# hagabbar/GenNet

Measured on AMD Instinct MI355X. Metric: waveforms/sec (CNN+GAN step, 2048-sample BBH), higher is better.
Workload: dtype f32

## Files before the change

gennet_amd/_lib.py:

```python
import ctypes as C
import os

_HERE = os.path.dirname(os.path.abspath(__file__))
LIB_PATH = os.path.join(_HERE, 'lib', 'libgennet_hip.so')

_lib = None

vp, i32, i64, f32, f64, u64, sz = C.c_void_p, C.c_int, C.c_longlong, C.c_float, C.c_double, C.c_uint64, C.c_size_t

_SIGS = {
    'gn_conv1d_fwd': [vp, vp, vp, vp, i32, i32, i32, i32, i32, i32, i32, i32, i32, f32, vp],
    'gn_conv1d_fwd_bf16x3': [vp, vp, vp, vp, vp, sz, i32, i32, i32, i32, i32, i32, i32, i32, i32, f32, i32, vp],
    'gn_conv1d_fwd_wino': [vp, vp, vp, vp, vp, sz, i32, i32, i32, i32, i32, i32, i32, i32, i32, f32, vp],
    'gn_conv1d_fwd_stats': [vp, vp, vp, vp, vp, vp, sz, i32, i32, i32, i32, i32, i32, i32, i32, vp],
    'gn_conv1d_fwd_dropout': [vp, vp, vp, vp, vp, i32, i32, i32, i32, i32, i32, i32, i32, i32, f32, f32, vp],
    'gn_conv1d_fwd_any': [vp, vp, vp, vp, i32, i32, i32, i32, i32, i32, i32, i32, i32, f32, vp],
    'gn_conv1d_dgrad_any': [vp, vp, vp, i32, i32, i32, i32, i32, i32, i32, i32, vp],
    'gn_conv1d_wgrad_any': [vp, vp, vp, vp, vp, sz, i32, i32, i32, i32, i32, i32, i32, i32, vp],
    'gn_conv1d_transpose_w': [vp, vp, i32, i32, i32, vp],
    'gn_conv1d_dgrad': [vp, vp, vp, i32, i32, i32, i32, i32, i32, i32, i32, vp],
    'gn_conv1d_dgrad_fused': [vp, vp, vp, i32, i32, i32, i32, i32, i32, i32, i32, vp, vp, i32, f32, f32, vp],
    'gn_dense_bwd_fused': [vp, vp, vp, vp, vp, vp, i32, i32, i32, vp, i32, f32, f32, vp],
    'gn_conv1d_wgrad': [vp, vp, vp, vp, vp, sz, i32, i32, i32, i32, i32, i32, i32, i32, vp],
    'gn_conv2d_w2_fold': [vp, vp, vp, vp, i32, i32, i32, vp],
    'gn_conv2d_w2_unfold_grad': [vp, vp, vp, vp, i32, i32, i32, vp],
    'gn_conv1d_tapfold_x': [vp, vp, i32, i32, i32, i32, i32, vp],
    'gn_conv1d_tapunfold_dx': [vp, vp, i32, i32, i32, i32, i32, vp],
    'gn_conv1d_tapfold_w': [vp, vp, i32, i32, i32, vp],
    'gn_conv1d_tapunfold_dw': [vp, vp, i32, i32, i32, vp],
    'gn_conv1d_tap_groups': [i32, vp, vp],
    'gn_conv1d_up2_fold': [vp, vp, vp, vp, i32, i32, i32, vp],
    'gn_conv1d_up2_unfold_grad': [vp, vp, vp, vp, i32, i32, i32, vp],
    'gn_dense_fwd': [vp, vp, vp, vp, i32, i32, i32, i32, f32, vp],
    'gn_dense_bwd': [vp, vp, vp, vp, vp, vp, vp, sz, i32, i32, i32, vp],
    'gn_act_fwd': [vp, vp, sz, i32, f32, vp],
    'gn_act_bwd': [vp, vp, vp, sz, i32, f32, vp],
    'gn_act_dropout_bwd': [vp, vp, vp, vp, sz, i32, f32, f32, vp],
    'gn_set_conv_math': [i32, vp, sz],
    'gn_conv_fold_bn': [vp, vp, vp, vp, vp, vp, sz, i32, vp],
    'gn_bn_apply_dropgen': [vp, vp, vp, vp, vp, sz, i32, i32, f32, f32, u64, u64, vp],
    'gn_bias_act_dropout': [vp, vp, vp, sz, i32, i32, f32, f32, i32, u64, u64, vp],
    'gn_bias_grad': [vp, vp, vp, sz, sz, i32, vp],
    'gn_prelu_fwd': [vp, vp, vp, i32, sz, vp],
    'gn_prelu_bwd': [vp, vp, vp, vp, vp, i32, sz, vp],
    'gn_dropout_mask': [vp, sz, f32, u64, u64, vp],
    'gn_dropout_apply': [vp, vp, vp, sz, f32, vp],
    'gn_upsample2_fwd': [vp, vp, i32, i32, i32, vp],
    'gn_upsample2_bwd': [vp, vp, i32, i32, i32, vp],
    'gn_maxpool_h2_fwd': [vp, vp, i32, i32, i32, vp],
    'gn_maxpool_h2_bwd': [vp, vp, vp, i32, i32, i32, vp],
    'gn_subtract_stack_fwd': [vp, vp, vp, i32, i32, vp],
    'gn_subtract_stack_bwd': [vp, vp, i32, i32, vp],
    'gn_affine_stack_fwd': [vp, vp, vp, f32, f32, vp, i32, i32, vp],
    'gn_affine_stack_bwd': [vp, f32, f32, vp, i32, i32, vp],
    'gn_assemble_d_batch': [vp, vp, vp, vp, vp, i32, i32, vp],
    'gn_fill_uniform': [vp, sz, f32, f32, u64, u64, vp],
    'gn_fill_normal': [vp, sz, f32, f32, u64, u64, vp],
    'gn_gather_rows': [vp, vp, vp, i32, i32, vp],
    'gn_axpy': [vp, vp, f32, sz, vp],
    'gn_bn_stats': [vp, sz, i32, vp, vp, sz, vp],
    'gn_bn_finalize': [vp, f64, vp, vp, f32, f32, vp, vp, vp, vp, vp, vp, i32, vp],
    'gn_bn_finalize_zero_debias': [vp, f64, vp, vp, f32, f32, vp, vp, vp, vp, i32, vp, vp, vp, vp, i32, vp],
    'gn_bn_infer_coeffs': [vp, vp, vp, vp, f32, vp, vp, i32, vp],
    'gn_bn_apply': [vp, vp, vp, vp, vp, sz, i32, i32, f32, f32, vp],
    'gn_bn_bwd_stats': [vp, vp, vp, vp, vp, vp, vp, vp, sz, sz, i32, i32, f32, f32, vp, vp, vp],
    'gn_bn_bwd_apply': [vp, vp, vp, vp, vp, vp, vp, vp, f64, vp, vp, vp, vp, sz, i32, i32, f32, f32, vp, vp, vp],
    'gn_bn_bwd_stats_conv1': [vp, vp, i32, i32, i32, i32, vp, vp, vp, vp, vp, vp, sz, sz, i32, i32, f32, f32, vp, vp, vp],
    'gn_bn_bwd_apply_conv1': [vp, vp, i32, i32, i32, i32, vp, vp, vp, vp, vp, vp, f64, vp, vp, vp, vp, sz, i32, i32, f32, f32, vp, vp, vp],
    'gn_bce_loss': [vp, vp, vp, vp, i32, i32, vp],
    'gn_mse_loss': [vp, vp, vp, vp, i32, i32, vp],
    'gn_loss_pass': [i32, vp, vp, vp, vp, i64, i32, f64, vp, sz, vp],
    'gn_weight_count': [vp, i64, vp, vp, sz, vp],
    'gn_loss_pass_weighted': [i32, vp, vp, vp, vp, vp, vp, i64, i32, vp, sz, vp],
    'gn_adam_step': [vp, vp, vp, vp, sz, f32, f32, f32, f32, vp],
    'gn_set_rng_base': [vp],
    'gn_adam_step_dyn': [vp, vp, vp, vp, sz, vp, f32, f32, f32, vp],
    'gn_optim_step': [i32, vp, vp, vp, vp, vp, sz, f32, vp, f32, f32, f32, i32, vp, f32, vp],
    'gn_optim_sumsq': [vp, sz, vp, vp],
    'gn_optim_clip_factor': [vp, sz, f32, vp, vp],
    'gn_fill_normal_dyn': [vp, sz, f32, vp, u64, u64, vp],
    'gn_gaussian_noise_fwd': [vp, vp, sz, f32, u64, u64, vp],
    'gn_gaussian_dropout_apply': [vp, vp, sz, f32, u64, u64, vp],
    'gn_alpha_dropout_fwd': [vp, vp, sz, f32, f32, f32, f32, u64, u64, vp],
    'gn_alpha_dropout_bwd': [vp, vp, sz, f32, f32, u64, u64, vp],
    'gn_bn_finalize_zero_debias_dyn': [vp, f64, vp, vp, f32, f32, vp, vp, vp, vp, vp, vp, vp, vp, vp, i32, vp],
    'gn_prof_enable': [i32],
    'gn_prof_reset': [],
    'gn_prof_collect': [i32, vp],
    'gn_chirp_fd_whitened': [vp, vp, vp, vp, vp, i32, i32, f64, f64, f64, f64, f64, vp],
    'gn_irfft_f64': [vp, vp, vp, i32, i32, vp],
    'gn_rfft_f64': [vp, vp, vp, i32, i32, vp],
    'gn_mul_f64': [vp, vp, sz, sz, i32, vp],
    'gn_align_crop': [vp, vp, vp, vp, vp, i32, i32, i32, i32, i32, i32, f64, f64, f64, vp],
    'gn_noise_fd': [vp, vp, i32, i32, u64, u64, vp],
    'gn_synth_templates': [vp, vp, vp, vp, vp, vp, vp, vp, i32, i32, i32, i32, i32, i32, f64, f64, f64, f64, f64, f64, f64, f64, vp],
    'gn_synth_templates_prior': [vp, vp, vp, vp, vp, vp, vp, vp, i32, i32, i32, i32, i32, i32, f64, f64, f64, f64, f64, f64, f64, f64, u64, u64, i32, i32,
                                 f64, f64, vp],
    'gn_noise_whitened': [vp, vp, vp, vp, vp, vp, vp, vp, vp, i32, i32, i32, i32, f64, u64, u64, vp],
    'gn_synth_templates_noise': [vp, vp, vp, vp, vp, vp, vp, vp, vp, vp, vp, vp, vp, i32, i32, i32, i32, i32, i32, f64, f64, f64, f64, f64, f64, f64, f64,
                                 u64, u64, i32, i32, f64, f64, u64, u64, vp, vp],
    'gn_kde2d_pdf': [vp, i32, vp, i32, f64, f64, f64, f64, vp, vp],
    'gn_scale_f64': [vp, f64, sz, vp],
    'gn_f64_to_f32': [vp, vp, f64, sz, vp],
}
_SIZE_FNS = {
    'gn_conv1d_bf16x3_workspace': [i32, i32, i32, i32, i32],
    'gn_conv1d_wino_workspace': [i32, i32],
    'gn_conv1d_wgrad_workspace': [i32, i32, i32, i32, i32, i32, i32],
    'gn_dense_bwd_workspace': [i32, i32, i32],
    'gn_bn_stats_workspace': [sz, i32],
    'gn_bias_grad_workspace': [sz, i32],
    'gn_conv1d_fwd_stats_workspace': [i32, i32, i32],
    'gn_optim_sumsq_slots': [sz],
    'gn_loss_pass_workspace': [i64, i32],
    'gn_weight_count_workspace': [i64],
    'gn_loss_pass_weighted_workspace': [i64, i32],
}


_PREDICATES = {
    'gn_conv1d_needs_any': [i32, i32],
}


class GennetHipError(RuntimeError):
    pass


def lib():
    global _lib
    if _lib is None:
        if not os.path.exists(LIB_PATH):
            try:
                from . import build as _build
                _build.build(verbose=False)
            except Exception as e:
                raise GennetHipError('%s not found and building it failed (%s): run `python -m gennet_amd.build` '
                                     '(hipcc --offload-arch=gfx950); gennet_amd has no CPU fallback' % (LIB_PATH, e))
        import torch
        L = C.CDLL(LIB_PATH)
        for table, restype in ((_SIGS, i32), (_SIZE_FNS, sz), (_PREDICATES, i32)):
            for name, args in table.items():
                try:
                    fn = getattr(L, name)
                except AttributeError:
                    continue
                fn.argtypes = args
                fn.restype = restype
        L.gn_last_error.restype = C.c_char_p
        L.gn_version.restype = i32
        _lib = L
    return _lib


def exported_symbols():
    return sorted(list(_SIGS) + list(_SIZE_FNS) + list(_PREDICATES) + ['gn_last_error', 'gn_version'])


def call(name, *args):
    L = lib()
    try:
        fn = getattr(L, name)
    except AttributeError:
        raise GennetHipError('%s is not exported by %s (stale build?)' % (name, LIB_PATH))
    rc = fn(*args)
    if rc != 0:
        raise GennetHipError('%s failed (%d): %s' % (name, rc, L.gn_last_error().decode()))


def size(name, *args):
    return int(getattr(lib(), name)(*args))


def predicate(name, *args):
    L = lib()
    try:
        fn = getattr(L, name)
    except AttributeError:
        raise GennetHipError('%s is not exported by %s (stale build?)' % (name, LIB_PATH))
    return bool(fn(*args))
```

gennet_amd/csrc/capi.hip:

```cpp
#include <stdarg.h>
#include <algorithm>
#include <mutex>
#include <vector>
#include <stdlib.h>
#include "common.h"

namespace gn {

static thread_local char g_err[512] = "";

void set_error(const char* fmt, ...) {
  va_list ap;
  va_start(ap, fmt);
  vsnprintf(g_err, sizeof(g_err), fmt, ap);
  va_end(ap);
}

int check_launch(const char* what) {
  hipError_t e = hipGetLastError();
  if (e != hipSuccess) {
    set_error("%s: %s", what, hipGetErrorString(e));
    return GN_ELAUNCH;
  }
  return GN_OK;
}

struct ProfRec {
  hipEvent_t a, b;
  double flop;
  int kind;
  double bytes;
};
static bool g_prof_on = false;
static std::vector<ProfRec> g_prof;
static std::vector<hipEvent_t> g_pool;
static hipEvent_t g_cur;
static std::mutex g_prof_mu;

static hipEvent_t get_event() {
  if (!g_pool.empty()) {
    hipEvent_t e = g_pool.back();
    g_pool.pop_back();
    return e;
  }
  hipEvent_t e;
  (void)hipEventCreate(&e);
  return e;
}

static thread_local const uint64_t* g_rng_base = nullptr;
const uint64_t* rng_base() { return g_rng_base; }

void prof_begin(hipStream_t s) {
  if (!g_prof_on) return;
  g_cur = get_event();
  (void)hipEventRecord(g_cur, s);
}

void prof_end(hipStream_t s, double flop, int kind, double bytes) {
  if (!g_prof_on) return;
  hipEvent_t b = get_event();
  (void)hipEventRecord(b, s);
  std::lock_guard<std::mutex> lk(g_prof_mu);
  g_prof.push_back({g_cur, b, flop, kind, bytes});
}

const Switches& switches() {
  static const Switches sw = [] {
    auto on = [](const char* name) { return getenv(name) != nullptr; };
    const char* gflop = getenv("GN_BF16X3_MIN_GFLOP");
    return Switches{on("GN_CONV_NOPIPE"),  on("GN_CONV_NODMA"),   on("GN_CONV_NOMERGE"),    on("GN_CONV_NONARROW"), on("GN_CONV_NOPATCH"),
                    on("GN_WGRAD_NOPIPE"), on("GN_BF16X3_NO_MERGE"), gflop ? atof(gflop) : 50.0};
  }();
  return sw;
}

static int g_conv_math = 0;
static void* g_conv_ws = nullptr;
static size_t g_conv_ws_bytes = 0;
constexpr size_t kWinoKernelBytes = 64ull << 20;

static bool split_worth_it(int B, int M, int ntaps, int Cin, int Cout) {
  constexpr int min_cin = 256, min_cout = 256;
  return Cin >= min_cin && Cout >= min_cout && 2.0 * B * (double)M * ntaps * Cin * Cout >= switches().bf16x3_min_gflop * 1e9;
}
static bool split_worth_it(const ConvArgs& a, int w_taps) {
  return w_taps > 0 ? split_worth_it(a.B, (a.Ly + 1) / 2, w_taps, a.Cin, a.Cout) : split_worth_it(a.B, a.M, a.t.ntaps, a.Cin, a.Cout);
}

static bool needs_any(int Cin, int Cout) {
  const bool strict = Cin <= 4 ? Cout % 4 == 0 : Cout <= 4 ? Cin % 4 == 0 : (Cin % 4 == 0 && Cout % 4 == 0);
  return !strict;
}

enum ConvFamily { CONV_SMALL, CONV_WINO, CONV_WINO_S2, CONV_BF16X3, CONV_DIRECT, CONV_ANYC };

static ConvFamily select_conv(const ConvArgs& a, int w_taps) {
  if (a.any_channels && needs_any(a.Cin, a.Cout)) return CONV_ANYC;
  if (a.Cin <= 4 || a.Cout <= 4) return CONV_SMALL;
  if (g_conv_math == 2 && a.Cin >= 32 && conv_wino_supported(a) && conv_wino_workspace_bytes(a.Cin, a.Cout) <= kWinoKernelBytes) return CONV_WINO;
  if (g_conv_math == 2 && conv_wino_s2_kind(a) == 1 && conv_wino_s2_workspace_bytes(a.Cin, a.Cout) <= kWinoKernelBytes) return CONV_WINO_S2;
  if (g_conv_math == 1 && split_worth_it(a, w_taps) && conv_bf16x3_supported(a)) return CONV_BF16X3;
  return CONV_DIRECT;
}

enum DgradFamily { DGRAD_WINO_S2, DGRAD_BF16X3_MERGED, DGRAD_MERGED, DGRAD_PHASES };

static DgradFamily select_dgrad(const ConvArgs& a) {
  if (a.any_channels && needs_any(a.Cin, a.Cout)) return DGRAD_PHASES;
  if (a.Ly < 2 || a.Cin <= 4 || a.Cout <= 4) return DGRAD_PHASES;
  if (g_conv_math == 2 && conv_wino_s2_kind(a) == 2 && conv_wino_s2_workspace_bytes(a.Cin, a.Cout) <= kWinoKernelBytes) return DGRAD_WINO_S2;
  const Switches& sw = switches();
  const bool split = g_conv_math == 1 && split_worth_it(a, 5);
  if (split) return !sw.bf16x3_no_merge && conv_bf16x3_merged_kind(a) ? DGRAD_BF16X3_MERGED : DGRAD_PHASES;
  if (!sw.conv_nomerge && !sw.conv_nopipe && !sw.conv_nodma && conv_pipe_merged_supported(a)) return DGRAD_MERGED;
  return DGRAD_PHASES;
}

enum WgradFamily { WGRAD_SMALL, WGRAD_WINO, WGRAD_WINO_S2, WGRAD_BF16X3, WGRAD_DIRECT, WGRAD_ANYC };

static WgradFamily select_wgrad(const WgradArgs& a) {
  if (a.any_channels && needs_any(a.Cin, a.Cout)) return WGRAD_ANYC;
  if (a.Cin <= 4 || a.Cout <= 4) return WGRAD_SMALL;
  if (g_conv_math == 2 && wgrad_wino_supported(a) && conv_wino_workspace_bytes(a.Cin, a.Cout) <= kWinoKernelBytes) return WGRAD_WINO;
  if (g_conv_math == 2 && wgrad_wino_s2_supported(a) && conv_wino_s2_workspace_bytes(a.Cin, a.Cout) <= kWinoKernelBytes) return WGRAD_WINO_S2;
  if (g_conv_math == 1 && split_worth_it(a.B, a.M, a.ntaps, a.Cin, a.Cout) && wgrad_bf16x3_supported(a)) return WGRAD_BF16X3;
  return WGRAD_DIRECT;
}

static size_t wgrad_ws_need(WgradFamily f, const WgradArgs& a) {
  switch (f) {
    case WGRAD_SMALL: return needs_any(a.Cin, a.Cout) ? 0 : wgrad_small_workspace_bytes(a.B, a.M, a.Cin, a.Cout, a.ntaps);
    case WGRAD_WINO: return wgrad_wino_workspace_bytes(a.B, a.M, a.Cin, a.Cout);
    case WGRAD_WINO_S2: return wgrad_wino_s2_workspace_bytes(a.B, a.M, a.Cin, a.Cout);
    case WGRAD_ANYC: return wgrad_anyc_workspace_bytes(a.B, a.M, a.Cin, a.Cout, a.ntaps);
    default: return wgrad_workspace_bytes(a.B, a.M, a.Cin, a.Cout, a.ntaps);
  }
}

static int ws_check(const char* what, size_t need, size_t have) {
  if (need <= have) return GN_OK;
  set_error("%s workspace: the selected kernel needs %zu bytes, the workspace has %zu", what, need, have);
  return GN_EWORKSPACE;
}

struct Phases { int w_taps; bool have_split; };

static int conv_run(const ConvArgs& a, hipStream_t s, Phases* ph = nullptr) {
  const ConvFamily f = select_conv(a, ph ? ph->w_taps : 0);
  int w_taps = ph ? ph->w_taps : 0;
  for (int j = 0; !ph && j < a.t.ntaps; ++j) w_taps = std::max(w_taps, a.t.widx[j] + 1);
  const size_t need = f == CONV_WINO ? conv_wino_workspace_bytes(a.Cin, a.Cout) : f == CONV_WINO_S2 ? conv_wino_s2_workspace_bytes(a.Cin, a.Cout)
                      : f == CONV_BF16X3 ? conv_bf16x3_workspace_bytes(a.B, a.Lin, a.Cin, a.Cout, w_taps) : 0;
  if (int rc = ws_check("conv-math", need, g_conv_ws_bytes)) return rc;
  switch (f) {
    case CONV_SMALL: return a.Cin <= 4 ? conv_smallcin_dispatch(a, s) : conv_smallcout_dispatch(a, s);
    case CONV_WINO: return conv_wino_run(a, g_conv_ws, g_conv_ws_bytes, s);
    case CONV_WINO_S2: return conv_wino_s2_run(a, g_conv_ws, g_conv_ws_bytes, s);
    case CONV_BF16X3:
      if (!(ph && ph->have_split)) {
        int rc = conv_bf16x3_split(a, w_taps, g_conv_ws, g_conv_ws_bytes, true, true, s);
        if (rc) return rc;
        if (ph) ph->have_split = true;
      }
      return conv_bf16x3_run(a, w_taps, g_conv_ws, s);
    case CONV_ANYC: return conv_anyc_dispatch(a, s);
    default: return conv_mfma_dispatch(a, s);
  }
}

static ConvArgs fwd_args(const float* x, const float* w, const float* bias, float* y, int B, int L, int Cin, int Cout, int k, int stride, int pad_left,
                         int Lout, int act, float act_param) {
  ConvArgs a = {};
  a.x = x; a.w = w; a.bias = bias; a.y = y;
  a.B = B; a.Lin = L; a.Cin = Cin; a.Cout = Cout; a.M = Lout; a.Ly = Lout;
  a.t.ntaps = k; a.t.in_stride = stride; a.t.out_stride = 1;
  for (int j = 0; j < k; ++j) { a.t.off[j] = j - pad_left; a.t.widx[j] = j; }
  a.act = act; a.act_param = act_param;
  return a;
}

static int set_conv_math_impl(int mode, void* workspace, size_t workspace_bytes) {
  GN_REQUIRE(mode >= 0 && mode <= 2, "set_conv_math: mode %d (0 = direct fp32, 1 = bf16x3, 2 = transform-domain fp32)", mode);
  GN_REQUIRE(mode == 0 || workspace, "set_conv_math: modes 1 and 2 need a device workspace");
  if (mode == 2 && workspace_bytes < kWinoKernelBytes) {
    set_error("set_conv_math: the transform-domain math needs a workspace of %zu bytes, got %zu", kWinoKernelBytes, workspace_bytes);
    return GN_EWORKSPACE;
  }
  g_conv_math = mode;
  g_conv_ws = mode ? workspace : nullptr;
  g_conv_ws_bytes = mode ? workspace_bytes : 0;
  return GN_OK;
}

__global__ void colsum_anyc_kernel(const float* __restrict__ x, double* __restrict__ acc, size_t n, int C) {
  double s[4] = {0, 0, 0, 0};
  const size_t stride = (size_t)gridDim.x * blockDim.x;
  for (size_t i = (size_t)blockIdx.x * blockDim.x + threadIdx.x; i < n; i += stride) {
    const int c = (int)(i % C);
    const double v = (double)x[i];
    s[0] += c == 0 ? v : 0.0; s[1] += c == 1 ? v : 0.0; s[2] += c == 2 ? v : 0.0; s[3] += c == 3 ? v : 0.0;
  }
  __shared__ double red[4][256];
  for (int c = 0; c < 4; ++c) red[c][threadIdx.x] = s[c];
  __syncthreads();
  for (int sft = 128; sft >= 1; sft >>= 1) {
    if (threadIdx.x < sft)
      for (int c = 0; c < 4; ++c) red[c][threadIdx.x] += red[c][threadIdx.x + sft];
    __syncthreads();
  }
  if (threadIdx.x < C) atomicAdd(&acc[threadIdx.x], red[threadIdx.x][0]);
}
__global__ void f64_to_f32_small_kernel(const double* __restrict__ a, float* __restrict__ o, int n) {
  if ((int)threadIdx.x < n) o[threadIdx.x] = (float)a[threadIdx.x];
}

static int bias_grad(const float* dy, float* db, size_t rows, int C, void* ws, size_t ws_bytes, hipStream_t s) {
  if (C % 4 == 0 || C > 4) {
    ColRedArgs r = {};
    r.a = dy; r.rows = rows; r.C = C;
    return colred_run(0, r, ws, ws_bytes, nullptr, db, s);
  }
  if (ws_bytes < 32) { set_error("bias_grad: workspace too small"); return GN_EWORKSPACE; }
  (void)hipMemsetAsync(ws, 0, 32, s);
  size_t g = (rows * C + 255) / 256;
  if (g > 1024) g = 1024;
  hipLaunchKernelGGL(colsum_anyc_kernel, dim3((unsigned)g), dim3(256), 0, s, dy, (double*)ws, rows * C, C);
  hipLaunchKernelGGL(f64_to_f32_small_kernel, dim3(1), dim3(64), 0, s, (const double*)ws, db, C);
  return check_launch("bias_grad");
}

static size_t bias_grad_ws(size_t rows, int C) { return C % 4 == 0 || C > 4 ? colred_workspace_bytes(rows, C) : 32; }

__global__ __launch_bounds__(256) void dense_any_kernel(const float* __restrict__ A, const float* __restrict__ Bm, const float* __restrict__ bias,
                                                        float* __restrict__ C, int M, int N, int K, size_t sam, size_t sak, size_t sbk, size_t sbn, int act,
                                                        float p) {
  __shared__ float As[16][17], Bs[16][17];
  const int tx = threadIdx.x % 16, ty = threadIdx.x / 16;
  const int m = blockIdx.y * 16 + ty, n = blockIdx.x * 16 + tx;
  float acc = 0.f;
  for (int k0 = 0; k0 < K; k0 += 16) {
    const int ka = k0 + tx, kb = k0 + ty;
    As[ty][tx] = (m < M && ka < K) ? A[(size_t)m * sam + (size_t)ka * sak] : 0.f;
    Bs[ty][tx] = (kb < K && n < N) ? Bm[(size_t)kb * sbk + (size_t)n * sbn] : 0.f;
    __syncthreads();
#pragma unroll
    for (int kk = 0; kk < 16; ++kk) acc = fmaf(As[ty][kk], Bs[kk][tx], acc);
    __syncthreads();
  }
  if (m < M && n < N) C[(size_t)m * N + n] = act_apply(bias ? acc + bias[n] : acc, act, p);
}
static int dense_any_gemm(const float* A, const float* Bm, const float* bias, float* C, int M, int N, int K, size_t sam, size_t sak, size_t sbk, size_t sbn,
                          int act, float p, hipStream_t s) {
  if (M <= 0 || N <= 0) return GN_OK;
  if ((M + 15) / 16 > 65535) { set_error("dense: %d rows exceed the grid", M); return GN_EINVAL; }
  hipLaunchKernelGGL(dense_any_kernel, dim3(cdiv(N, 16), cdiv(M, 16)), dim3(256), 0, s, A, Bm, bias, C, M, N, K, sam, sak, sbk, sbn, act, p);
  return check_launch("dense_any");
}
static bool dense_any_shape(int in, int out) { return (in % 4 || out % 4) && !(out <= 4 && in % 4 == 0); }

}

using namespace gn;

extern "C" {

const char* gn_last_error(void) { return g_err; }
int gn_version(void) { return 100; }

int gn_prof_enable(int on) {
  g_prof_on = on != 0;
  return GN_OK;
}
int gn_prof_reset(void) {
  std::lock_guard<std::mutex> lk(g_prof_mu);
  for (auto& r : g_prof) {
    g_pool.push_back(r.a);
    g_pool.push_back(r.b);
  }
  g_prof.clear();
  return GN_OK;
}
int gn_prof_collect(int kind, double* out) {
  std::lock_guard<std::mutex> lk(g_prof_mu);
  double ms = 0, flop = 0, cnt = 0, bytes = 0;
  for (auto& r : g_prof) {
    if (kind >= 0 && r.kind != kind) continue;
    cnt += 1;
    if (hipEventSynchronize(r.b) != hipSuccess) { set_error("prof: event sync failed"); return GN_ELAUNCH; }
    float t = 0;
    if (hipEventElapsedTime(&t, r.a, r.b) != hipSuccess) { set_error("prof: elapsed failed"); return GN_ELAUNCH; }
    ms += t;
    flop += r.flop;
    bytes += r.bytes;
  }
  out[0] = cnt;
  out[1] = ms;
  out[2] = flop;
  out[3] = bytes;
  return GN_OK;
}

static int fwd_impl(const float* x, const float* w, const float* bias, float* y, int B, int L, int Cin, int Cout, int k, int stride, int pad_left, int Lout,
                    int act, float act_param, bool any_channels, void* stream) {
  GN_REQUIRE(x && w && y, "conv1d_fwd: null pointer");
  GN_REQUIRE(B >= 0 && L > 0 && Cin > 0 && Cout > 0 && k >= 1 && k <= 8 && stride >= 1 && Lout > 0, "conv1d_fwd: bad shape");
  GN_REQUIRE(pad_left >= 0 && stride * (Lout - 1) + k - pad_left <= L + k, "conv1d_fwd: Lout %d inconsistent with L %d k %d stride %d", Lout, L, k, stride);
  if (B == 0) return GN_OK;
  ConvArgs a = fwd_args(x, w, bias, y, B, L, Cin, Cout, k, stride, pad_left, Lout, act, act_param);
  a.any_channels = any_channels;
  return conv_run(a, (hipStream_t)stream);
}

int gn_conv1d_fwd(const float* x, const float* w, const float* bias, float* y, int B, int L, int Cin, int Cout, int k, int stride, int pad_left, int Lout,
                  int act, float act_param, void* stream) {
  return fwd_impl(x, w, bias, y, B, L, Cin, Cout, k, stride, pad_left, Lout, act, act_param, false, stream);
}
int gn_conv1d_fwd_any(const float* x, const float* w, const float* bias, float* y, int B, int L, int Cin, int Cout, int k, int stride, int pad_left, int Lout,
                      int act, float act_param, void* stream) {
  return fwd_impl(x, w, bias, y, B, L, Cin, Cout, k, stride, pad_left, Lout, act, act_param, true, stream);
}
int gn_conv1d_needs_any(int Cin, int Cout) { return needs_any(Cin, Cout) ? 1 : 0; }

int gn_set_conv_math(int mode, void* workspace, size_t workspace_bytes) { return set_conv_math_impl(mode, workspace, workspace_bytes); }

size_t gn_conv1d_bf16x3_workspace(int B, int L, int Cin, int Cout, int k) { return conv_bf16x3_workspace_bytes(B, L, Cin, Cout, k); }

size_t gn_conv1d_fwd_stats_workspace(int B, int Lout, int Cout) {
  const size_t fused = (size_t)B * (size_t)((Lout + 63) / 64) * 2 * (size_t)Cout * sizeof(double);
  const size_t plain = colred_workspace_bytes((size_t)B * Lout, Cout);
  return (fused > plain ? fused : plain) + 256;
}

int gn_conv1d_fwd_stats(const float* x, const float* w, const float* bias, float* y, double* sums, void* ws, size_t ws_bytes, int B, int L, int Cin, int Cout, int k,
                        int stride, int pad_left, int Lout, void* stream) {
  hipStream_t s = (hipStream_t)stream;
  GN_REQUIRE(x && w && y && sums && ws, "conv1d_fwd_stats: null pointer");
  GN_REQUIRE(B > 0 && L > 0 && Cin > 0 && Cout > 0 && Cout % 4 == 0 && k >= 1 && k <= 8 && stride >= 1 && Lout > 0, "conv1d_fwd_stats: bad shape");
  GN_REQUIRE(pad_left >= 0 && stride * (Lout - 1) + k - pad_left <= L + k, "conv1d_fwd_stats: Lout %d inconsistent with L %d k %d stride %d", Lout, L, k, stride);
  GN_REQUIRE(ws_bytes >= gn_conv1d_fwd_stats_workspace(B, Lout, Cout), "conv1d_fwd_stats: workspace too small");
  ConvArgs a = fwd_args(x, w, bias, y, B, L, Cin, Cout, k, stride, pad_left, Lout, GN_ACT_LINEAR, 0.f);
  int done = 0;
  a.stat_part = (double*)ws; a.stat_sums = sums; a.stat_done = &done;
  int rc = conv_run(a, s);
  if (rc || done) return rc;
  ColRedArgs r = {};
  r.a = y; r.rows = (size_t)B * Lout; r.C = Cout;
  return colred_run(1, r, ws, ws_bytes, sums, nullptr, s);
}

int gn_conv1d_fwd_bf16x3(const float* x, const float* w, const float* bias, float* y, void* ws, size_t ws_bytes, int B, int L, int Cin, int Cout, int k, int stride,
                         int pad_left, int Lout, int act, float act_param, int resplit, void* stream) {
  GN_REQUIRE(x && w && y && ws, "conv1d_fwd_bf16x3: null pointer");
  GN_REQUIRE(B >= 0 && L > 0 && Cin > 0 && Cout > 0 && k >= 1 && k <= 5 && stride >= 1 && Lout > 0 && pad_left >= 0, "conv1d_fwd_bf16x3: bad shape");
  if (B == 0) return GN_OK;
  ConvArgs a = fwd_args(x, w, bias, y, B, L, Cin, Cout, k, stride, pad_left, Lout, act, act_param);
  GN_REQUIRE(conv_bf16x3_supported(a), "conv1d_fwd_bf16x3: needs Cin %% 16 == 0, Cout %% 64 == 0, k <= 5, stride 1");
  if (resplit) {
    int rc = conv_bf16x3_split(a, k, ws, ws_bytes, true, true, (hipStream_t)stream);
    if (rc) return rc;
  }
  return conv_bf16x3_run(a, k, ws, (hipStream_t)stream);
}

size_t gn_conv1d_wino_workspace(int Cin, int Cout) { return conv_wino_workspace_bytes(Cin, Cout); }

int gn_conv1d_fwd_wino(const float* x, const float* w, const float* bias, float* y, void* ws, size_t ws_bytes, int B, int L, int Cin, int Cout, int k, int stride,
                       int pad_left, int Lout, int act, float act_param, void* stream) {
  GN_REQUIRE(x && w && y && ws, "conv1d_fwd_wino: null pointer");
  GN_REQUIRE(B >= 0 && L > 0 && Cin > 0 && Cout > 0 && k == 5 && stride == 1 && Lout > 0 && pad_left >= 0, "conv1d_fwd_wino: 5 taps, unit stride");
  if (B == 0) return GN_OK;
  ConvArgs a = fwd_args(x, w, bias, y, B, L, Cin, Cout, k, stride, pad_left, Lout, act, act_param);
  return conv_wino_run(a, ws, ws_bytes, (hipStream_t)stream);
}

int gn_conv1d_fwd_dropout(const float* x, const float* w, const float* bias, const uint8_t* mask, float* y, int B, int L, int Cin, int Cout, int k, int stride,
                          int pad_left, int Lout, int act, float act_param, float rate, void* stream) {
  GN_REQUIRE(x && w && y && mask, "conv1d_fwd_dropout: null pointer");
  GN_REQUIRE(B >= 0 && L > 0 && Cin > 0 && Cout > 4 && Cout % 4 == 0 && k >= 1 && k <= 5 && stride >= 1 && Lout > 0 && pad_left >= 0, "conv1d_fwd_dropout: bad shape");
  GN_REQUIRE(rate >= 0.f && rate < 1.f, "conv1d_fwd_dropout: bad rate %f", rate);
  if (B == 0) return GN_OK;
  ConvArgs a = fwd_args(x, w, bias, y, B, L, Cin, Cout, k, stride, pad_left, Lout, act, act_param);
  a.mask = mask; a.keep_scale = 1.0f / (1.0f - rate);
  return conv_run(a, (hipStream_t)stream);
}

int gn_conv1d_transpose_w(const float* w, float* wt, int k, int Cin, int Cout, void* stream) {
  GN_REQUIRE(w && wt && k >= 1 && Cin > 0 && Cout > 0, "transpose_w: bad arguments");
  return transpose_w(w, wt, k, Cin, Cout, (hipStream_t)stream);
}

static int dgrad_impl(const float* dy, const float* wt, float* dx, int B, int L, int Cin, int Cout, int k, int stride, int pad_left, int Lout, const float* gy,
                      const uint8_t* gmask, int gact, float gparam, float grate, void* stream, bool any_channels = false) {
  GN_REQUIRE(dy && wt && dx, "conv1d_dgrad: null pointer");
  GN_REQUIRE(B >= 0 && L > 0 && Cin > 0 && Cout > 0 && k >= 1 && k <= 8 && stride >= 1 && Lout > 0 && pad_left >= 0, "conv1d_dgrad: bad shape");
  if (B == 0) return GN_OK;
  auto phase_args = [&](int p) {
    ConvArgs a = {};
    a.x = dy; a.w = wt; a.bias = nullptr; a.y = dx;
    a.B = B; a.Lin = Lout; a.Cin = Cout; a.Cout = Cin; a.Ly = L;
    a.t.in_stride = 1; a.t.out_stride = stride;
    a.act = GN_ACT_LINEAR;
    a.any_channels = any_channels;
    a.gy = gy; a.gmask = gmask; a.gact = gact; a.gparam = gparam; a.gscale = 1.0f / (1.0f - grate);
    a.M = (L - std::max(p, 0) + stride - 1) / stride;
    a.t.out_off = p < 0 ? pad_left & 1 : p;
    if (p < 0) a.t.out_off_odd = 1 - (pad_left & 1);
    for (int kk = 0; kk < k; ++kk) {
      const int d = (p < 0 ? (kk + pad_left) & 1 : p) + pad_left - kk;
      if (((d % stride) + stride) % stride) continue;
      a.t.off[a.t.ntaps] = (d >= 0) ? d / stride : -((-d) / stride);
      a.t.widx[a.t.ntaps++] = kk;
    }
    return a;
  };
  hipStream_t s = (hipStream_t)stream;
  if (stride == 2 && k == 5) {
    const ConvArgs a = phase_args(-1);
    const DgradFamily f = select_dgrad(a);
    const size_t need = f == DGRAD_WINO_S2 ? conv_wino_s2_workspace_bytes(a.Cin, a.Cout)
                        : f == DGRAD_BF16X3_MERGED ? conv_bf16x3_workspace_bytes(a.B, a.Lin, a.Cin, a.Cout, 5) : 0;
    if (int rc = ws_check("conv-math", need, g_conv_ws_bytes)) return rc;
    if (f == DGRAD_WINO_S2) return conv_wino_s2_run(a, g_conv_ws, g_conv_ws_bytes, s);
    if (f == DGRAD_MERGED) return conv_pipe_run_merged(a, s);
    if (f == DGRAD_BF16X3_MERGED) {
      int rc = conv_bf16x3_split(a, 5, g_conv_ws, g_conv_ws_bytes, true, true, s);
      return rc ? rc : conv_bf16x3_run_merged(a, g_conv_ws, s);
    }
  }
  Phases ph = {stride > 1 ? k : 0, false};
  for (int p = 0; p < stride && p < L; ++p) {
    const ConvArgs a = phase_args(p);
    GN_REQUIRE(a.t.ntaps > 0, "conv1d_dgrad: phase %d has no taps (k %d < stride %d)", p, k, stride);
    int rc = conv_run(a, s, stride > 1 ? &ph : nullptr);
    if (rc) return rc;
  }
  return GN_OK;
}

int gn_conv1d_dgrad(const float* dy, const float* wt, float* dx, int B, int L, int Cin, int Cout, int k, int stride, int pad_left, int Lout, void* stream) {
  return dgrad_impl(dy, wt, dx, B, L, Cin, Cout, k, stride, pad_left, Lout, nullptr, nullptr, GN_ACT_LINEAR, 0.f, 0.f, stream);
}

int gn_conv1d_dgrad_any(const float* dy, const float* wt, float* dx, int B, int L, int Cin, int Cout, int k, int stride, int pad_left, int Lout, void* stream) {
  return dgrad_impl(dy, wt, dx, B, L, Cin, Cout, k, stride, pad_left, Lout, nullptr, nullptr, GN_ACT_LINEAR, 0.f, 0.f, stream, true);
}

int gn_conv1d_dgrad_fused(const float* dy, const float* wt, float* dx, int B, int L, int Cin, int Cout, int k, int stride, int pad_left, int Lout,
                          const float* y_prev, const uint8_t* mask_prev, int act_prev, float act_param_prev, float rate_prev, void* stream) {
  GN_REQUIRE(y_prev, "conv1d_dgrad_fused: y_prev is NULL");
  GN_REQUIRE(Cin > 4 && Cout > 4, "conv1d_dgrad_fused: only the MFMA path fuses the producer's activation gradient (Cin %d, Cout %d)", Cin, Cout);
  GN_REQUIRE(rate_prev >= 0.f && rate_prev < 1.f, "conv1d_dgrad_fused: bad rate");
  return dgrad_impl(dy, wt, dx, B, L, Cin, Cout, k, stride, pad_left, Lout, y_prev, mask_prev, act_prev, act_param_prev, mask_prev ? rate_prev : 0.f, stream);
}

static WgradArgs wgrad_args(const float* x, const float* dy, void* ws, int B, int L, int Cin, int Cout, int k, int stride, int pad_left, int Lout) {
  WgradArgs a = {};
  a.x = x; a.dy = dy; a.part = (float*)ws;
  a.B = B; a.Lin = L; a.Cin = Cin; a.Cout = Cout; a.M = Lout; a.ntaps = k; a.in_stride = stride;
  for (int j = 0; j < k && j < 8; ++j) a.off[j] = j - pad_left;
  return a;
}

size_t gn_conv1d_wgrad_workspace(int B, int L, int Cin, int Cout, int k, int stride, int Lout) {
  WgradArgs a = wgrad_args(nullptr, nullptr, nullptr, B, L, Cin, Cout, k, stride, 0, Lout);
  a.any_channels = 1;
  return std::max(wgrad_ws_need(select_wgrad(a), a), bias_grad_ws((size_t)B * Lout, Cout)) + 256;
}

static int wgrad_impl(const float* x, const float* dy, float* dw, float* db, void* ws, size_t ws_bytes, int B, int L, int Cin, int Cout, int k, int stride,
                      int pad_left, int Lout, bool any_channels, void* stream) {
  GN_REQUIRE(x && dy && dw && ws, "conv1d_wgrad: null pointer");
  GN_REQUIRE(B > 0 && L > 0 && Cin > 0 && Cout > 0 && k >= 1 && k <= 5 && stride >= 1 && Lout > 0 && pad_left >= 0, "conv1d_wgrad: bad shape");
  hipStream_t s = (hipStream_t)stream;
  WgradArgs a = wgrad_args(x, dy, ws, B, L, Cin, Cout, k, stride, pad_left, Lout);
  a.db = db;
  a.any_channels = any_channels;
  const WgradFamily f = select_wgrad(a);
  int rc = ws_check("conv1d_wgrad", wgrad_ws_need(f, a), ws_bytes);
  if (rc) return rc;
  switch (f) {
    case WGRAD_SMALL: {
      WgradSmallArgs sa = {x, dy, (float*)ws, B, L, Cin, Cout, Lout, k, stride};
      std::copy(a.off, a.off + k, sa.off);
      rc = wgrad_small_dispatch(sa, dw, ws_bytes, s);
      break;
    }
    case WGRAD_WINO: rc = wgrad_wino_run(a, dw, s); break;
    case WGRAD_WINO_S2: rc = wgrad_wino_s2_run(a, dw, s); break;
    case WGRAD_ANYC: rc = wgrad_anyc_dispatch(a, dw, ws_bytes, s); break;
    case WGRAD_BF16X3:
      rc = ws_check("conv-math", wgrad_bf16x3_workspace_bytes(B, Lout, Cin, Cout, stride), g_conv_ws_bytes);
      if (!rc) rc = wgrad_bf16x3_dispatch(a, dw, g_conv_ws, g_conv_ws_bytes, s);
      break;
    default:
      rc = wgrad_mfma_dispatch(a, dw, ws_bytes, s);
      if (!rc && a.db_done) return GN_OK;
  }
  if (rc) return rc;
  return db ? bias_grad(dy, db, (size_t)B * Lout, Cout, ws, ws_bytes, s) : GN_OK;
}

int gn_conv1d_wgrad(const float* x, const float* dy, float* dw, float* db, void* ws, size_t ws_bytes, int B, int L, int Cin, int Cout, int k, int stride,
                    int pad_left, int Lout, void* stream) {
  return wgrad_impl(x, dy, dw, db, ws, ws_bytes, B, L, Cin, Cout, k, stride, pad_left, Lout, false, stream);
}
int gn_conv1d_wgrad_any(const float* x, const float* dy, float* dw, float* db, void* ws, size_t ws_bytes, int B, int L, int Cin, int Cout, int k, int stride,
                        int pad_left, int Lout, void* stream) {
  return wgrad_impl(x, dy, dw, db, ws, ws_bytes, B, L, Cin, Cout, k, stride, pad_left, Lout, true, stream);
}

int gn_conv2d_w2_fold(const float* w, const float* bias, float* wf, float* biasf, int kh, int Cin, int Cout, void* stream) {
  GN_REQUIRE(w && wf && kh >= 1 && Cin > 0 && Cout > 0, "conv2d_w2_fold: bad arguments");
  return conv2d_w2_fold(w, bias, wf, biasf, kh, Cin, Cout, (hipStream_t)stream);
}
int gn_conv2d_w2_unfold_grad(const float* dwf, const float* dbf, float* dw, float* db, int kh, int Cin, int Cout, void* stream) {
  GN_REQUIRE(dwf && dw && kh >= 1 && Cin > 0 && Cout > 0, "conv2d_w2_unfold_grad: bad arguments");
  return conv2d_w2_unfold(dwf, dbf, dw, db, kh, Cin, Cout, (hipStream_t)stream);
}
int gn_conv1d_up2_fold(const float* w, const float* bias, float* wf, float* biasf, int Cin, int Cout, int stride, void* stream) {
  GN_REQUIRE(w && wf && Cin > 0 && Cout > 0 && (stride == 1 || stride == 2), "conv1d_up2_fold: bad arguments (5-tap 'same' conv, stride 1 or 2)");
  return up2_fold(w, bias, wf, biasf, Cin, Cout, stride, (hipStream_t)stream);
}
int gn_conv1d_up2_unfold_grad(const float* dwf, const float* dbf, float* dw, float* db, int Cin, int Cout, int stride, void* stream) {
  GN_REQUIRE(dwf && dw && Cin > 0 && Cout > 0 && (stride == 1 || stride == 2) && (!db || dbf), "conv1d_up2_unfold_grad: bad arguments");
  return up2_unfold(dwf, dbf, dw, db, Cin, Cout, stride, (hipStream_t)stream);
}

size_t gn_bias_grad_workspace(size_t rows, int C) { return bias_grad_ws(rows, C) + 256; }

int gn_bias_grad(const float* dy, float* db, void* ws, size_t ws_bytes, size_t rows, int C, void* stream) {
  GN_REQUIRE(dy && db && ws && rows > 0 && C > 0, "bias_grad: bad arguments");
  return bias_grad(dy, db, rows, C, ws, ws_bytes, (hipStream_t)stream);
}

int gn_dense_fwd(const float* x, const float* w, const float* bias, float* y, int B, int in, int out, int act, float act_param, void* stream) {
  GN_REQUIRE(x && w && y && B >= 0 && in > 0 && out > 0, "dense_fwd: bad arguments");
  if (B == 0) return GN_OK;
  if (dense_any_shape(in, out))
    return dense_any_gemm(x, w, bias, y, B, out, in, (size_t)in, 1, (size_t)out, 1, act, act_param, (hipStream_t)stream);
  if (out <= 4) return dense_small_fwd(x, w, bias, y, B, in, out, act, act_param, (hipStream_t)stream);
  return conv_mfma_dispatch(fwd_args(x, w, bias, y, 1, B, in, out, 1, 1, 0, B, act, act_param), (hipStream_t)stream);
}

size_t gn_dense_bwd_workspace(int B, int in, int out) {
  if (out <= 4) return 256;
  if (dense_any_shape(in, out)) return bias_grad_ws((size_t)B, out) + 256;
  size_t w = wgrad_workspace_bytes(1, B, in, out, 1);
  size_t b = bias_grad_ws((size_t)B, out);
  return (w > b ? w : b) + (size_t)in * out * sizeof(float) + 256;
}

int gn_dense_bwd_fused(const float* x, const float* w, const float* dy, float* dx, float* dw, float* db, int B, int in, int out, const uint8_t* mask_prev,
                       int act_prev, float act_param_prev, float rate_prev, void* stream) {
  GN_REQUIRE(x && w && dy && dx && dw && B > 0 && in > 0 && out >= 1 && out <= 4, "dense_bwd_fused: bad arguments (small-output heads only)");
  GN_REQUIRE(rate_prev >= 0.f && rate_prev < 1.f, "dense_bwd_fused: bad rate");
  return dense_small_bwd(x, w, dy, dx, dw, db, B, in, out, (hipStream_t)stream, act_prev, act_param_prev, mask_prev, 1.0f / (1.0f - (mask_prev ? rate_prev : 0.f)));
}

int gn_dense_bwd(const float* x, const float* w, const float* dy, float* dx, float* dw, float* db, void* ws, size_t ws_bytes, int B, int in, int out, void* stream) {
  GN_REQUIRE(x && w && dy && dw && B > 0 && in > 0 && out > 0, "dense_bwd: bad arguments");
  hipStream_t s = (hipStream_t)stream;
  if (dense_any_shape(in, out)) {
    GN_REQUIRE(ws && ws_bytes >= bias_grad_ws((size_t)B, out), "dense_bwd: workspace too small");
    int rc = dx ? dense_any_gemm(dy, w, nullptr, dx, B, in, out, (size_t)out, 1, 1, (size_t)out, GN_ACT_LINEAR, 0.f, s) : GN_OK;
    if (!rc) rc = dense_any_gemm(x, dy, nullptr, dw, in, out, B, 1, (size_t)in, (size_t)out, 1, GN_ACT_LINEAR, 0.f, s);
    if (!rc && db) rc = bias_grad(dy, db, (size_t)B, out, ws, ws_bytes, s);
    return rc;
  }
  if (out <= 4) return dense_small_bwd(x, w, dy, dx, dw, db, B, in, out, s);
  GN_REQUIRE(ws && ws_bytes >= gn_dense_bwd_workspace(B, in, out), "dense_bwd: workspace too small");
// ... 243 lines not shown
```

gennet_amd/csrc/common.h:

```cpp
#pragma once
#include <hip/hip_runtime.h>
#include <stdint.h>
#include <stdio.h>
#include "../../include/gennet_hip.h"

#define GN_LDS_DMA_CLOBBER() asm volatile("" ::: "v0", "v1", "v2", "v3")
#define gn_buffer_load_lds(...) do { __builtin_amdgcn_raw_ptr_buffer_load_lds(__VA_ARGS__); GN_LDS_DMA_CLOBBER(); } while (0)
#define gn_global_load_lds(...) do { __builtin_amdgcn_global_load_lds(__VA_ARGS__); GN_LDS_DMA_CLOBBER(); } while (0)

namespace gn {

void set_error(const char* fmt, ...);
int check_launch(const char* what);

struct Switches {
  bool conv_nopipe, conv_nodma, conv_nomerge, conv_nonarrow, conv_nopatch;
  bool wgrad_nopipe, bf16x3_no_merge;
  double bf16x3_min_gflop;
};
const Switches& switches();

const uint64_t* rng_base();
void prof_begin(hipStream_t s);
void prof_end(hipStream_t s, double flop, int kind, double bytes = 0.0);


struct ConvTaps {
  int ntaps;
  int in_stride;
  int off[8];
  int widx[8];
  int out_stride, out_off;
  int out_off_odd;
};

struct ConvArgs {
  const float* x;
  const float* w;
  const float* bias;
  float* y;
  int B, Lin, Cin, Cout;
  int M;
  int Ly;
  ConvTaps t;
  int act;
  float act_param;
  int any_channels;
  const uint8_t* mask;
  float keep_scale;
  const float* gy;
  const uint8_t* gmask;
  int gact;
  float gparam, gscale;
  double* stat_part;
  double* stat_sums;
  int* stat_done;
};

struct WgradArgs {
  const float* x;
  const float* dy;
  float* part;
  int B, Lin, Cin, Cout, M;
  int ntaps, in_stride;
  int off[8];
  int chunks_per_split;
  double* db_part;
  float* db;
  int db_done;
  int any_channels;
};

struct WgradSmallArgs {
  const float* x;
  const float* dy;
  float* part;
  int B, Lin, Cin, Cout, M;
  int ntaps, in_stride;
  int off[8];
  int rows_per_chunk;
};

struct LazyDy {
  const float* g;
  const float* w;
  int L, Lout, k, pad_left;
};

struct ColRedArgs {
  const float* a;
  const float* y;
  const float* xpre;
  const uint8_t* mask;
  const float* mean;
  const float* invstd;
  const float* scale;
  const float* shift;
  double* part;
  size_t rows;
  int C;
  int rows_per_chunk;
  int act;
  float act_param;
  float keep_scale;
  LazyDy lz;
};

int conv_mfma_dispatch(const ConvArgs& a, hipStream_t s);
size_t wgrad_workspace_bytes(int B, int M, int Cin, int Cout, int ntaps);
int wgrad_mfma_dispatch(WgradArgs& a, float* dw, size_t ws_bytes, hipStream_t s);
int wgrad_bf16x3_dispatch(WgradArgs& a, float* dw, void* split_ws, size_t split_ws_bytes, hipStream_t s);
int conv_pipe_try(const ConvArgs& a, bool tall, hipStream_t s, bool* launched);
bool conv_pipe_merged_supported(const ConvArgs& a);
int conv_pipe_run_merged(const ConvArgs& a, hipStream_t s);
void wgrad_pipe_launch(const WgradArgs& a, dim3 grid, bool narrow, hipStream_t s);
size_t conv_bf16x3_workspace_bytes(int B, int Lin, int Cin, int Cout, int w_taps);
bool conv_bf16x3_supported(const ConvArgs& a);
int conv_bf16x3_split(const ConvArgs& a, int w_taps, void* ws, size_t ws_bytes, bool split_x, bool split_w, hipStream_t s);
int conv_bf16x3_run(const ConvArgs& a, int w_taps, void* ws, hipStream_t s);
int conv_bf16x3_merged_kind(const ConvArgs& a);
int conv_bf16x3_run_merged(const ConvArgs& a, void* ws, hipStream_t s);
size_t conv_wino_workspace_bytes(int Cin, int Cout);
bool conv_wino_supported(const ConvArgs& a);
int conv_wino_run(const ConvArgs& a, void* ws, size_t ws_bytes, hipStream_t s);
size_t conv_wino_s2_workspace_bytes(int Cin, int Cout);
int conv_wino_s2_kind(const ConvArgs& a);
int conv_wino_s2_run(const ConvArgs& a, void* ws, size_t ws_bytes, hipStream_t s);
void wgrad_split_plan(int B, int M, int Cin, int Cout, int TC, int TN, int* splits, int* chunks_per_split);
bool wgrad_wino_supported(const WgradArgs& a);
size_t wgrad_wino_workspace_bytes(int B, int M, int Cin, int Cout);
int wgrad_wino_run(WgradArgs& a, float* dw, hipStream_t s);
bool wgrad_wino_s2_supported(const WgradArgs& a);
size_t wgrad_wino_s2_workspace_bytes(int B, int M, int Cin, int Cout);
int wgrad_wino_s2_run(WgradArgs& a, float* dw, hipStream_t s);
size_t wgrad_bf16x3_workspace_bytes(int B, int M, int Cin, int Cout, int in_stride);
bool wgrad_bf16x3_supported(const WgradArgs& a);
int wgrad_bf16x3_run(const WgradArgs& a, int splits, void* ws, size_t ws_bytes, hipStream_t s);
int conv_anyc_dispatch(const ConvArgs& a, hipStream_t s);
size_t wgrad_anyc_workspace_bytes(int B, int M, int Cin, int Cout, int ntaps);
int wgrad_anyc_dispatch(WgradArgs& a, float* dw, size_t ws_bytes, hipStream_t s);
int conv_smallcin_dispatch(const ConvArgs& a, hipStream_t s);
int conv_smallcout_dispatch(const ConvArgs& a, hipStream_t s);
size_t wgrad_small_workspace_bytes(int B, int M, int Cin, int Cout, int ntaps);
int wgrad_small_dispatch(WgradSmallArgs a, float* dw, size_t ws_bytes, hipStream_t s);
int dense_small_fwd(const float* x, const float* w, const float* bias, float* y, int B, int in, int out, int act, float p, hipStream_t s);
int dense_small_bwd(const float* x, const float* w, const float* dy, float* dx, float* dw, float* db, int B, int in, int out, hipStream_t s,
                    int gact = 0, float gparam = 0.f, const uint8_t* gmask = nullptr, float gscale = 1.f);
int act_fwd(const float* x, float* y, size_t n, int act, float p, hipStream_t s);
int act_bwd(const float* dy, const float* y, float* dx, size_t n, int act, float p, hipStream_t s);
int act_dropout_bwd(const float* dy, const float* y, const uint8_t* mask, float* dx, size_t n, int act, float p, float rate, hipStream_t s);
int dropout_mask(uint8_t* mask, size_t n, float rate, uint64_t seed, uint64_t offset, hipStream_t s);
int dropout_apply(const float* x, const uint8_t* mask, float* y, size_t n, float rate, hipStream_t s);
int upsample2_fwd(const float* x, float* y, int B, int L, int C, hipStream_t s);
int upsample2_bwd(const float* dy, float* dx, int B, int L, int C, hipStream_t s);
int subtract_stack_fwd(const float* x, const float* ev, float* img, int B, int n, hipStream_t s);
int subtract_stack_bwd(const float* dimg, float* dx, int B, int n, hipStream_t s);
int affine_stack_fwd(const float* x, const float* b0, const float* b1, float a0, float a1, float* img, int B, int n, hipStream_t s);
int affine_stack_bwd(const float* dimg, float a0, float a1, float* dx, int B, int n, hipStream_t s);
int assemble_d_batch(const float* real, const float* noise, const float* fake, const float* ev, float* sX, int B, int n, hipStream_t s);
int gather_rows(const float* src, const int64_t* idx, float* out, int rows, int width, hipStream_t s);
int axpy(float* y, const float* x, float a, size_t n, hipStream_t s);
int fill_uniform(float* out, size_t n, float lo, float hi, uint64_t seed, uint64_t offset, hipStream_t s);
int fill_normal(float* out, size_t n, float mean, float sd, uint64_t seed, uint64_t offset, hipStream_t s, const float* sd_dev = nullptr);
int gaussian_noise_fwd(const float* x, float* y, size_t n, float stddev, uint64_t seed, uint64_t offset, hipStream_t s);
int gaussian_dropout_apply(const float* x, float* y, size_t n, float sd, uint64_t seed, uint64_t offset, hipStream_t s);
int alpha_dropout_fwd(const float* x, float* y, size_t n, float rate, float a, float b, float alpha_p, uint64_t seed, uint64_t offset, hipStream_t s);
int alpha_dropout_bwd(const float* dy, float* dx, size_t n, float rate, float a, uint64_t seed, uint64_t offset, hipStream_t s);
size_t colred_workspace_bytes(size_t rows, int C);
int colred_run(int mode, ColRedArgs a, void* ws, size_t ws_bytes, double* out_f64, float* out_f32, hipStream_t s);
int colred_finalize(const double* part, double* out_f64, size_t n, int chunks, hipStream_t s);
int colred_finalize_f32(const double* part, float* out_f32, size_t n, int chunks, hipStream_t s);
int bn_finalize(const double* sums, double count, const float* gamma, const float* beta, float eps, float momentum, float* mm, float* mv,
                float* bm, float* bv, float zd_step, float* scale, float* shift, float* smean, float* sinv, int C, hipStream_t s,
                const int32_t* zd_step_dev = nullptr);
int bn_infer_coeffs(const float* gamma, const float* beta, const float* mm, const float* mv, float eps, float* scale, float* shift, int C, hipStream_t s);
int bn_apply(const float* x, const float* scale, const float* shift, const uint8_t* mask, float* y, size_t rows, int C, int act, float p, float rate, hipStream_t s);
int bn_bwd_apply(const float* dy, const float* y, const float* x, const uint8_t* mask, const float* gamma, const float* mean, const float* invstd,
                 const double* dsums_global, double count, const double* dsums_local, float* dx, float* dgamma, float* dbeta, size_t rows, int C,
                 int act, float p, float rate, const float* scale, const float* shift, hipStream_t s, const LazyDy* lz = nullptr);
int loss_run(int kind, const float* p, const float* y, float* dp, float* out, int B, int Bglobal, hipStream_t s);
int adam_step(float* p, const float* g, float* m, float* v, size_t n, float lr_t, float b1, float b2, float eps, hipStream_t s, const float* lr_t_dev = nullptr);
struct OptArgs {
  float *p, *s0, *s1, *s2;
  const float* g;
  size_t n;
  float lr;
  const float* lr_dev;
  float h0, h1, eps;
  int nesterov;
  const float* clip_scale;
  float clipvalue;
};
int optim_step(int rule, const OptArgs& a, hipStream_t s);
size_t optim_sumsq_slots(size_t n);
int optim_sumsq(const float* g, size_t n, double* partials, hipStream_t s);
int optim_clip_factor(const double* partials, size_t count, float clipnorm, float* factor, hipStream_t s);
int transpose_w(const float* w, float* wt, int k, int Cin, int Cout, hipStream_t s);
int conv2d_w2_fold(const float* w, const float* bias, float* wf, float* bf, int kh, int Cin, int Cout, hipStream_t s);
int conv2d_w2_unfold(const float* dwf, const float* dbf, float* dw, float* db, int kh, int Cin, int Cout, hipStream_t s);
int up2_fold(const float* w, const float* bias, float* wf, float* bf, int Cin, int Cout, int stride, hipStream_t s);
int up2_unfold(const float* dwf, const float* dbf, float* dw, float* db, int Cin, int Cout, int stride, hipStream_t s);

static inline unsigned cdiv(size_t a, size_t b) { return (unsigned)((a + b - 1) / b); }
static inline unsigned stream_grid(size_t n_items, int block = 256) {
  size_t g = (n_items + block - 1) / block;
  if (g > 256 * 8) g = 256 * 8;
  if (g < 1) g = 1;
  return (unsigned)g;
}

static inline void allow_big_lds(const void* kernel, unsigned long long* done) {
  int dev = 0;
  (void)hipGetDevice(&dev);
  const unsigned long long bit = 1ull << (dev & 63);
  if (!(*done & bit)) {
    (void)hipFuncSetAttribute(kernel, hipFuncAttributeMaxDynamicSharedMemorySize, 160 * 1024);
    *done |= bit;
  }
}

#define GN_REQUIRE(cond, ...)            \
  do {                                   \
    if (!(cond)) {                       \
      gn::set_error(__VA_ARGS__);        \
      return GN_EINVAL;                  \
    }                                    \
  } while (0)

__device__ __forceinline__ float gn_tanhf(float x) {
  const float ax = fabsf(x);
  const float e = __builtin_amdgcn_exp2f(ax * 2.8853900817779268f);
  const float big = 1.f - 2.f * __builtin_amdgcn_rcpf(e + 1.f);
  const float x2 = ax * ax;
  float q = fmaf(x2, -1382.f / 155925.f, 62.f / 2835.f);
  q = fmaf(x2, q, -17.f / 315.f);
  q = fmaf(x2, q, 2.f / 15.f);
  q = fmaf(x2, q, -1.f / 3.f);
  const float small = fmaf(ax * x2, q, ax);
  return copysignf(ax < 0.35f ? small : big, x);
}

__device__ __forceinline__ float act_apply(float x, int act, float p) {
  switch (act) {
    case GN_ACT_RELU: return fmaxf(x, 0.f);
    case GN_ACT_RELU_MAX: return fminf(fmaxf(x, 0.f), p);
    case GN_ACT_LEAKY: return x > 0.f ? x : p * x;
    case GN_ACT_TANH: return gn_tanhf(x);
    case GN_ACT_SIGMOID: return 1.f / (1.f + expf(-x));
    default: return x;
  }
}

__device__ __forceinline__ float act_grad_from_y(float y, int act, float p) {
  switch (act) {
    case GN_ACT_RELU: return y > 0.f ? 1.f : 0.f;
    case GN_ACT_RELU_MAX: return (y > 0.f && y < p) ? 1.f : 0.f;
    case GN_ACT_LEAKY: return y > 0.f ? 1.f : p;
    case GN_ACT_TANH: return 1.f - y * y;
    case GN_ACT_SIGMOID: return y * (1.f - y);
    default: return 1.f;
  }
}

struct Philox4 {
  uint32_t v[4];
};

__host__ __device__ __forceinline__ uint32_t mulhi32(uint32_t a, uint32_t b) { return (uint32_t)(((uint64_t)a * b) >> 32); }

__host__ __device__ __forceinline__ Philox4 philox4x32_10(uint64_t counter, uint64_t seed) {
  uint32_t c0 = (uint32_t)counter, c1 = (uint32_t)(counter >> 32), c2 = 0, c3 = 0;
  uint32_t k0 = (uint32_t)seed, k1 = (uint32_t)(seed >> 32);
#pragma unroll
  for (int r = 0; r < 10; ++r) {
    const uint32_t M0 = 0xD2511F53u, M1 = 0xCD9E8D57u;
    uint32_t h0 = mulhi32(M0, c0), l0 = M0 * c0;
    uint32_t h1 = mulhi32(M1, c2), l1 = M1 * c2;
    uint32_t n0 = h1 ^ c1 ^ k0, n1 = l1, n2 = h0 ^ c3 ^ k1, n3 = l0;
    c0 = n0; c1 = n1; c2 = n2; c3 = n3;
    k0 += 0x9E3779B9u; k1 += 0xBB67AE85u;
  }
  Philox4 o;
  o.v[0] = c0; o.v[1] = c1; o.v[2] = c2; o.v[3] = c3;
  return o;
}

__host__ __device__ __forceinline__ float u01_24(uint32_t x) { return (float)(x >> 8) * (1.0f / 16777216.0f); }
__host__ __device__ __forceinline__ double u01_53(uint32_t hi, uint32_t lo) {
  uint64_t x = (((uint64_t)hi << 32) | lo) >> 11;
  return ((double)x + 0.5) * (1.0 / 9007199254740992.0);
}

}
```

gennet_amd/csrc/conv_wino.hip:

```cpp
#include <stdlib.h>
#include <algorithm>
#include <type_traits>
#include "common.h"
#include "conv_epilogue.h"
#include "wino_common.h"

namespace gn {

struct WinoTaps {
  int wq[5];
};

__global__ void wino_u_kernel(const float* __restrict__ w, float* __restrict__ U, int Cin, int Cout, WinoTaps t) {
  const size_t i = (size_t)blockIdx.x * blockDim.x + threadIdx.x;
  const size_t cc = (size_t)Cin * Cout;
  if (i >= cc) return;
  const int ci = (int)(i / Cout), co = (int)(i % Cout);
  double g[5];
#pragma unroll
  for (int q = 0; q < 5; ++q) g[q] = (double)w[(size_t)t.wq[q] * cc + i];
  float u[6];
  u[0] = (float)g[0];
  u[1] = (float)((g[0] + g[1] + g[2] + g[3] + g[4]) * (1.0 / 3.0));
  u[2] = (float)((g[0] - g[1] + g[2] - g[3] + g[4]) * (1.0 / 3.0));
  u[3] = (float)((16.0 * g[0] + 8.0 * g[1] + 4.0 * g[2] + 2.0 * g[3] + g[4]) * (1.0 / 15.0));
  u[4] = (float)((g[0] - 2.0 * g[1] + 4.0 * g[2] - 8.0 * g[3] + 16.0 * g[4]) * (1.0 / 30.0));
  u[5] = (float)g[4];
  const int chunk = ci >> 3, c = ci & 7, kq = c >> 1, s = c & 1;
  const int tile = co >> 6, nn = co & 63, ct = nn >> 4, n16 = nn & 15, cth = ct >> 1, ctl = ct & 1;
  const size_t base = ((size_t)chunk * (Cout >> 6) + tile) * 3072 + ((cth * 4 + kq) * 16 + n16) * 4 + ctl * 2 + s;
#pragma unroll
  for (int p = 0; p < 6; ++p) U[base + p * 512] = u[p];
}

template <int O, int OP1>
__device__ __forceinline__ void wino_slot_rba(f32x4& c, float a, float b, f32x4& nb0, f32x4& nb1, unsigned addr_b, f32x2 (&d)[6], unsigned addr_a) {
  asm volatile(
      "ds_read_b128 %1, %11 offset:%13\n\t"
      "ds_read_b128 %2, %11 offset:%14\n\t"
      "ds_read_b64 %3, %12\n\t"
      "ds_read_b64 %4, %12 offset:%15\n\t"
      "ds_read_b64 %5, %12 offset:32\n\t"
      "ds_read_b64 %6, %12 offset:%16\n\t"
      "ds_read_b64 %7, %12 offset:64\n\t"
      "ds_read_b64 %8, %12 offset:%17\n\t"
      "s_waitcnt lgkmcnt(8)\n\t"
      "v_mfma_f32_16x16x4_f32 %0, %9, %10, %0"
      : "+v"(c), "=&v"(nb0), "=&v"(nb1), "=&v"(d[0]), "=&v"(d[1]), "=&v"(d[2]), "=&v"(d[3]), "=&v"(d[4]), "=&v"(d[5])
      : "v"(a), "v"(b), "v"(addr_b), "v"(addr_a), "i"(O), "i"(O + 1024), "i"(OP1), "i"(OP1 + 32), "i"(OP1 + 64)
      : "memory");
}
template <int O>
__device__ __forceinline__ void wino_slot_rbw(f32x4& c, float a, float b, f32x4& nb0, f32x4& nb1, unsigned addr_b, f32x2 (&d)[6]) {
  asm volatile(
      "ds_read_b128 %1, %11 offset:%12\n\t"
      "ds_read_b128 %2, %11 offset:%13\n\t"
      "s_waitcnt lgkmcnt(2)\n\t"
      "v_mfma_f32_16x16x4_f32 %0, %9, %10, %0"
      : "+v"(c), "=&v"(nb0), "=&v"(nb1), "+v"(d[0]), "+v"(d[1]), "+v"(d[2]), "+v"(d[3]), "+v"(d[4]), "+v"(d[5])
      : "v"(a), "v"(b), "v"(addr_b), "i"(O), "i"(O + 1024)
      : "memory");
}

template <int RPER, int ABL = 0>
struct WinoChunk {
  template <int NPIECES, int I = 0, class D>
  static __device__ __forceinline__ void run(f32x4 (&acc)[6][4], const f32x2 (&v)[6], f32x2 (&vn)[6], f32x2 (&d)[6], WinoT& t, f32x4 (&B)[2][2], unsigned addr_b,
                                             unsigned addr_b_next, unsigned addr_a, unsigned long long k15, unsigned long long km15, D& dma) {
    if constexpr (I < 48) {
      constexpr int P = I / 8, S = (I / 4) % 2, CT = I % 4;
      f32x4(&bc)[2] = B[P & 1];
      f32x4(&bn)[2] = B[(P + 1) & 1];
      const float bv = bc[CT >> 1][2 * (CT & 1) + S];
      const float av = v[P][S];
      if constexpr ((ABL & 8) != 0) wino_slot(acc[P][CT], av, bv);
      else if constexpr (I == 0) wino_slot_rba<2048, RPER * 32>(acc[0][0], av, bv, bn[0], bn[1], addr_b, d, addr_a);
      else if constexpr (I == 8) wino_slot_rbw<2 * 2048>(acc[1][0], av, bv, bn[0], bn[1], addr_b, d);
      else if constexpr (I == 40) wino_slot_rb<0, 2>(acc[5][0], av, bv, bn[0], bn[1], addr_b_next);
      else if constexpr (I % 8 == 0) wino_slot_rb<(P + 1) * 2048, 2>(acc[P][0], av, bv, bn[0], bn[1], addr_b);
      else wino_slot(acc[P][CT], av, bv);
      if constexpr ((I & 1) && (I >> 1) < NPIECES) dma(std::integral_constant<int, (I >> 1)>{});
      if constexpr (!(ABL & 2)) {
        if constexpr (I == 12) wino_run<0, 5>(d, vn, t, k15, km15);
        if constexpr (I == 24) wino_run<5, 10>(d, vn, t, k15, km15);
        if constexpr (I == 36) wino_run<10, kWinoPieces>(d, vn, t, k15, km15);
      }
      run<NPIECES, I + 1>(acc, v, vn, d, t, B, addr_b, addr_b_next, addr_a, k15, km15, dma);
    }
  }
};

template <int WAVES_M, int ABL = 0>
__global__ __launch_bounds__(64 * WAVES_M, (WAVES_M > 4 ? 1 : 2)) void conv_wino_kernel(ConvArgs a, const float* __restrict__ U, int off0, int m_tiles, int n_tiles,
                                                                                        int patch) {
#if defined(__HIP_DEVICE_COMPILE__)
  constexpr int KC = 8, NP = 6;
  constexpr int TT = WAVES_M * 16;
  constexpr int TN = 64;
  constexpr int NT = 64 * WAVES_M;
  constexpr int RPER = TT + 2;
  constexpr int SLAB = 2 * RPER * KC;
  constexpr int UT = NP * KC * TN;
  constexpr int BUF = SLAB + UT;
  constexpr int STAGE_BYTES = BUF * 4;
  extern __shared__ __attribute__((aligned(16))) float smem[];
  typedef __attribute__((address_space(3))) void* lptr_t;

  const int tid = threadIdx.x, lane = tid & 63, wave = tid >> 6;
  const int n16 = lane & 15, kq = lane >> 4;
  const BlockTile bt = xcd_block_tile(patch, m_tiles, n_tiles);
  const int n_tile = bt.n_tile, m_tile = bt.m_tile, b = bt.b;
  const int t0 = m_tile * TT, n0 = n_tile * TN;

  f32x4 acc[NP][4];
#pragma unroll
  for (int p = 0; p < NP; ++p)
#pragma unroll
    for (int ct = 0; ct < 4; ++ct)
#pragma unroll
      for (int r = 0; r < 4; ++r) acc[p][ct][r] = 0.f;

  const int t_base = 2 * t0 + off0;
  const uintptr_t xbp = (uintptr_t)(a.x + (size_t)b * a.Lin * a.Cin);
  const unsigned xb_lo = __builtin_amdgcn_readfirstlane((unsigned)xbp), xb_hi = __builtin_amdgcn_readfirstlane((unsigned)(xbp >> 32));
  const int xbytes = __builtin_amdgcn_readfirstlane(a.Lin * a.Cin * 4);
  const __amdgpu_buffer_rsrc_t xsrd = __builtin_amdgcn_make_buffer_rsrc((void*)(((uintptr_t)xb_hi << 32) | xb_lo), 0, xbytes, 0x00020000);

  constexpr int S_COUNT = SLAB / 4;
  constexpr int S_ITEMS = (S_COUNT + NT - 1) / NT;
  constexpr int W_TOTAL = UT / 4;
  constexpr int W_ITEMS = (W_TOTAL + NT - 1) / NT;
  int soff[S_ITEMS];
#pragma unroll
  for (int it = 0; it < S_ITEMS; ++it) {
    const int id = tid + it * NT;
    const int lr = id >> 1, c4 = id & 1;
    const int r = lr < RPER ? 2 * lr : 2 * (lr - RPER) + 1;
    soff[it] = (id < S_COUNT) ? ((t_base + r) * a.Cin + 4 * c4) * 4 : 0x40000000;
  }
  const uintptr_t wbp = (uintptr_t)U;
  const unsigned wb_lo = __builtin_amdgcn_readfirstlane((unsigned)wbp), wb_hi = __builtin_amdgcn_readfirstlane((unsigned)(wbp >> 32));
  const int wbytes = __builtin_amdgcn_readfirstlane(NP * a.Cin * a.Cout * 4);
  const __amdgpu_buffer_rsrc_t wsrd = __builtin_amdgcn_make_buffer_rsrc((void*)(((uintptr_t)wb_hi << 32) | wb_lo), 0, wbytes, 0x00020000);
  const int w_chunk_bytes = n_tiles * UT * 4;
  int c_next = 0, st_next = 0;
  bool in_loop = false;
  const int wv64 = __builtin_amdgcn_readfirstlane(tid & ~63);
  auto dma_piece = [&](auto kc) {
    constexpr int k = decltype(kc)::value;
    if ((ABL & 1) && in_loop) return;
    float* stg = smem + st_next * BUF;
    if constexpr (k < S_ITEMS) {
      if ((k + 1) * NT <= S_COUNT || tid + k * NT < S_COUNT)
        gn_buffer_load_lds(xsrd, (lptr_t)(stg + (k * NT + wv64) * 4), 16, soff[k], c_next * KC * 4, 0, 0);
    } else {
      constexpr int it = k - S_ITEMS;
      if ((it + 1) * NT <= W_TOTAL || wv64 + it * NT < W_TOTAL)
        gn_buffer_load_lds(wsrd, (lptr_t)(stg + SLAB + (it * NT + wv64) * 4), 16, (n_tile * UT + (tid + it * NT) * 4) * 4,
                                                 c_next * w_chunk_bytes, 0, 0);
    }
  };
  constexpr int NPIECES = S_ITEMS + W_ITEMS;
  static_assert(NPIECES <= 6, "staging pieces");
  auto dma_all = [&]() {
    dma_piece(std::integral_constant<int, 0>{});
    if constexpr (NPIECES > 1) dma_piece(std::integral_constant<int, 1>{});
    if constexpr (NPIECES > 2) dma_piece(std::integral_constant<int, 2>{});
    if constexpr (NPIECES > 3) dma_piece(std::integral_constant<int, 3>{});
    if constexpr (NPIECES > 4) dma_piece(std::integral_constant<int, 4>{});
    if constexpr (NPIECES > 5) dma_piece(std::integral_constant<int, 5>{});
  };

  const unsigned lds0 = (unsigned)(uintptr_t)smem;
  const unsigned base_a = lds0 + (wave * 16 + n16) * 32 + kq * 8;
  const unsigned base_b = lds0 + SLAB * 4 + (kq * 16 + n16) * 16;
  const unsigned long long k15 = 0x3fc000003fc00000ull, km15 = 0xbfc00000bfc00000ull;

  const int n_chunks = a.Cin / KC;
  c_next = 0; st_next = 0; dma_all();
  c_next = min(1, n_chunks - 1); st_next = 1; dma_all();
  __syncthreads();

  f32x2 V0[6], V1[6], d[6];
  f32x4 Bq[2][2];
  WinoT tt;
  {
    const char* sb = reinterpret_cast<const char*>(smem);
#pragma unroll
    for (int j = 0; j < 6; ++j) d[j] = *reinterpret_cast<const f32x2*>(sb + (base_a - lds0) + (j & 1) * RPER * 32 + (j >> 1) * 32);
    wino_run<0, kWinoPieces>(d, V0, tt, k15, km15);
    Bq[0][0] = *reinterpret_cast<const f32x4*>(sb + (base_b - lds0));
    Bq[0][1] = *reinterpret_cast<const f32x4*>(sb + (base_b - lds0) + 1024);
  }
  int st = 0;
  in_loop = true;
  for (int ch = 0; ch < n_chunks; ch += 2) {
#pragma unroll
    for (int half = 0; half < 2; ++half) {
      if (half == 1 && ch + 1 >= n_chunks) break;
      const int st1 = st == 2 ? 0 : st + 1, st2 = st1 == 2 ? 0 : st1 + 1;
      c_next = min(ch + half + 2, n_chunks - 1);
      st_next = st2;
      const unsigned addr_a = base_a + st1 * STAGE_BYTES;
      const unsigned addr_b = base_b + st * STAGE_BYTES, addr_b_next = base_b + st1 * STAGE_BYTES;
      if (half == 0) WinoChunk<RPER, ABL>::template run<NPIECES>(acc, V0, V1, d, tt, Bq, addr_b, addr_b_next, addr_a, k15, km15, dma_piece);
      else WinoChunk<RPER, ABL>::template run<NPIECES>(acc, V1, V0, d, tt, Bq, addr_b, addr_b_next, addr_a, k15, km15, dma_piece);
      if constexpr (!(ABL & 4)) __syncthreads();
      st = st1;
    }
  }
  asm volatile("s_nop 15\n\ts_nop 7" : "+v"(acc[5][0]), "+v"(acc[5][1]), "+v"(acc[5][2]), "+v"(acc[5][3]));

  f32x4 out[2][4];
#pragma unroll
  for (int ct = 0; ct < 4; ++ct)
#pragma unroll
    for (int r = 0; r < 4; ++r) {
      out[0][ct][r] = (((acc[0][ct][r] + acc[1][ct][r]) + acc[2][ct][r]) + acc[3][ct][r]) + acc[4][ct][r];
      out[1][ct][r] = __builtin_fmaf(-2.f, acc[4][ct][r], __builtin_fmaf(0.5f, acc[3][ct][r], acc[1][ct][r] - acc[2][ct][r])) + acc[5][ct][r];
    }
  const int m_base = t0 + __builtin_amdgcn_readfirstlane(wave) * 16;
  const int mode = a.gy ? (a.gmask ? 3 : 2) : (a.mask ? 1 : 0);
  ConvArgs a2 = a;
  a2.t.out_stride = 2;
  tile16_epilogue_dispatch<4>(a2, out[0], b, m_base, n0, n16, kq, a.t.out_off, mode);
  tile16_epilogue_dispatch<4>(a2, out[1], b, m_base, n0, n16, kq, a.t.out_off + 1, mode);

  if (a.stat_part) {
    double* red = reinterpret_cast<double*>(smem);
#pragma unroll
    for (int ct = 0; ct < 4; ++ct) {
      const float bias = a.bias ? a.bias[n0 + ct * 16 + n16] : 0.f;
      double s1 = 0.0, s2 = 0.0;
#pragma unroll
      for (int ph = 0; ph < 2; ++ph)
#pragma unroll
        for (int r = 0; r < 4; ++r) {
          const int row = 2 * (m_base + 4 * kq + r) + ph;
          if (row < a.M) {
            const double v = (double)(out[ph][ct][r] + bias);
            s1 += v; s2 += v * v;
          }
        }
      s1 += __shfl_xor(s1, 16, 64); s2 += __shfl_xor(s2, 16, 64);
      s1 += __shfl_xor(s1, 32, 64); s2 += __shfl_xor(s2, 32, 64);
      if (kq == 0) {
        const int slot = (wave * TN + ct * 16 + n16) * 2;
        red[slot] = s1; red[slot + 1] = s2;
      }
    }
    __syncthreads();
    if (tid < TN) {
      double t1 = 0.0, t2 = 0.0;
#pragma unroll
      for (int w = 0; w < WAVES_M; ++w) { t1 += red[(w * TN + tid) * 2]; t2 += red[(w * TN + tid) * 2 + 1]; }
      double* dst = a.stat_part + (size_t)(b * m_tiles + m_tile) * 2 * a.Cout;
      dst[n0 + tid] = t1;
      dst[a.Cout + n0 + tid] = t2;
    }
  }
#endif
}

template <int WAVES_M, int ABL = 0>
static int launch_conv_wino(const ConvArgs& a, const float* U, int off0, hipStream_t s) {
  constexpr int TT = WAVES_M * 16, TN = 64;
  constexpr size_t lds = 3 * sizeof(float) * ((size_t)2 * (TT + 2) * 8 + (size_t)6 * 8 * TN);
  static_assert(lds <= 160 * 1024, "stages too large");
  if (lds > 64 * 1024) {
    static unsigned long long lds_done = 0;
    allow_big_lds((const void*)conv_wino_kernel<WAVES_M, ABL>, &lds_done);
  }
  const int tiles = (a.M + 1) / 2;
  const int m_tiles = (tiles + TT - 1) / TT, n_tiles = a.Cout / TN;
  const size_t blocks = (size_t)m_tiles * n_tiles * a.B;
  if (blocks == 0 || blocks > 0x7fffffffull) {
    set_error("conv_wino: bad grid %zu", blocks);
    return GN_EINVAL;
  }
  const int patch = xcd_patch(n_tiles);
  prof_begin(s);
  hipLaunchKernelGGL((conv_wino_kernel<WAVES_M, ABL>), dim3((unsigned)blocks), dim3(64 * WAVES_M), lds, s, a, U, off0, m_tiles, n_tiles, patch);
  prof_end(s, 0.6 * 2.0 * a.B * (double)a.M * 5 * a.Cin * a.Cout, 5, 4.0 * ((double)a.B * a.Lin * a.Cin + 5.0 * a.Cin * a.Cout + (double)a.B * a.M * a.Cout));
  int rc = check_launch("conv_wino");
  if (rc || !a.stat_part) return rc;
  *a.stat_done = 1;
  return colred_finalize(a.stat_part, a.stat_sums, (size_t)2 * a.Cout, a.B * m_tiles, s);
}

size_t conv_wino_workspace_bytes(int Cin, int Cout) { return (size_t)6 * Cin * Cout * sizeof(float); }

bool conv_wino_supported(const ConvArgs& a) {
  if (a.t.ntaps != 5 || a.t.in_stride != 1 || a.t.out_stride != 1 || a.t.out_off != 0) return false;
  if (a.Cin % 8 || a.Cout % 64 || a.Cin < 8) return false;
  if ((size_t)a.Ly * a.Cout * 4 >= 0x40000000ull || (size_t)a.Lin * a.Cin * 4 >= 0x40000000ull || (size_t)6 * a.Cin * a.Cout * 4 >= 0x40000000ull) return false;
  bool seen[5] = {false, false, false, false, false};
  int minoff = a.t.off[0];
  for (int j = 1; j < 5; ++j) minoff = std::min(minoff, a.t.off[j]);
  for (int j = 0; j < 5; ++j) {
    const int q = a.t.off[j] - minoff;
    if (q < 0 || q > 4 || seen[q]) return false;
    seen[q] = true;
  }
  if (a.stat_part && (a.act != GN_ACT_LINEAR || a.mask || a.gy)) return false;
  return true;
}

int conv_wino_run(const ConvArgs& a, void* ws, size_t ws_bytes, hipStream_t s) {
  if (!conv_wino_supported(a)) {
    set_error("conv_wino: unsupported shape (5 consecutive taps, unit strides, Cin %% 8 == 0, Cout %% 64 == 0)");
    return GN_EINVAL;
  }
  if (!ws || ws_bytes < conv_wino_workspace_bytes(a.Cin, a.Cout)) {
    set_error("conv_wino: workspace too small (%zu < %zu)", ws_bytes, conv_wino_workspace_bytes(a.Cin, a.Cout));
    return GN_EWORKSPACE;
  }
  int minoff = a.t.off[0];
  for (int j = 1; j < 5; ++j) minoff = std::min(minoff, a.t.off[j]);
  WinoTaps t;
  for (int j = 0; j < 5; ++j) t.wq[a.t.off[j] - minoff] = a.t.widx[j];
  const size_t cc = (size_t)a.Cin * a.Cout;
  hipLaunchKernelGGL(wino_u_kernel, dim3(cdiv(cc, 256)), dim3(256), 0, s, a.w, (float*)ws, a.Cin, a.Cout, t);
  int rc = check_launch("wino_u");
  if (rc) return rc;
  const float* Up = (const float*)ws;
#ifdef GN_ABLATION
  {
    static const int abl = getenv("GN_WINO_ABL") ? atoi(getenv("GN_WINO_ABL")) : 0;
    switch (abl) {
      case 1: return launch_conv_wino<4, 1>(a, Up, minoff, s);
      case 2: return launch_conv_wino<4, 2>(a, Up, minoff, s);
      case 3: return launch_conv_wino<4, 3>(a, Up, minoff, s);
      case 4: return launch_conv_wino<4, 4>(a, Up, minoff, s);
      case 8: return launch_conv_wino<4, 8>(a, Up, minoff, s);
      case 15: return launch_conv_wino<4, 15>(a, Up, minoff, s);
      default: break;
    }
  }
#endif
  return launch_conv_wino<4>(a, Up, minoff, s);
}

}
```

gennet_amd/csrc/conv_wino_s2.hip:

```cpp
#include <stdlib.h>
#include <algorithm>
#include <type_traits>
#include "common.h"
#include "conv_epilogue.h"
#include "wino_common.h"

namespace gn {

struct WinoS2Taps {
  int wq[5];
};

__global__ void wino_s2_u_kernel(const float* __restrict__ w, float* __restrict__ U, int Cin, int Cout, WinoS2Taps t) {
  const size_t i = (size_t)blockIdx.x * blockDim.x + threadIdx.x;
  const size_t cc = (size_t)Cin * Cout;
  if (i >= cc) return;
  const int ci = (int)(i / Cout), co = (int)(i % Cout);
  double g[5];
#pragma unroll
  for (int q = 0; q < 5; ++q) g[q] = (double)w[(size_t)t.wq[q] * cc + i];
  float u[7];
  u[0] = (float)g[0];
  u[1] = (float)(0.5 * (g[0] + g[2] + g[4]));
  u[2] = (float)(0.5 * (g[0] - g[2] + g[4]));
  u[3] = (float)g[4];
  u[4] = (float)g[1];
  u[5] = (float)(g[1] + g[3]);
  u[6] = (float)g[3];
  const int chunk = ci >> 3, c = ci & 7, kq = c >> 1, s = c & 1;
  const int tile = co >> 6, nn = co & 63, ct = nn >> 4, n16 = nn & 15, cth = ct >> 1, ctl = ct & 1;
  const size_t base = ((size_t)chunk * (Cout >> 6) + tile) * 3584 + ((cth * 4 + kq) * 16 + n16) * 4 + ctl * 2 + s;
#pragma unroll
  for (int p = 0; p < 7; ++p) U[base + p * 512] = u[p];
}

template <int O, int PB>
__device__ __forceinline__ void s2_slot_rba7(f32x4& c, float a, float b, f32x4& nb0, f32x4& nb1, unsigned addr_b, f32x2 (&d)[7], unsigned addr_a) {
  asm volatile(
      "ds_read_b128 %1, %12 offset:%14\n\t"
      "ds_read_b128 %2, %12 offset:%15\n\t"
      "ds_read_b64 %3, %13\n\t"
      "ds_read_b64 %4, %13 offset:%16\n\t"
      "ds_read_b64 %5, %13 offset:%17\n\t"
      "ds_read_b64 %6, %13 offset:%18\n\t"
      "ds_read_b64 %7, %13 offset:32\n\t"
      "ds_read_b64 %8, %13 offset:%19\n\t"
      "ds_read_b64 %9, %13 offset:%20\n\t"
      "s_waitcnt lgkmcnt(9)\n\t"
      "v_mfma_f32_16x16x4_f32 %0, %10, %11, %0"
      : "+v"(c), "=&v"(nb0), "=&v"(nb1), "=&v"(d[0]), "=&v"(d[1]), "=&v"(d[2]), "=&v"(d[3]), "=&v"(d[4]), "=&v"(d[5]), "=&v"(d[6])
      : "v"(a), "v"(b), "v"(addr_b), "v"(addr_a), "i"(O), "i"(O + 1024), "i"(PB), "i"(2 * PB), "i"(3 * PB), "i"(PB + 32), "i"(2 * PB + 32)
      : "memory");
}
template <int O, int PB>
__device__ __forceinline__ void s2_slot_rba4(f32x4& c, float a, float b, f32x4& nb0, f32x4& nb1, unsigned addr_b, f32x2 (&d)[4], unsigned addr_a) {
  asm volatile(
      "ds_read_b128 %1, %9 offset:%11\n\t"
      "ds_read_b128 %2, %9 offset:%12\n\t"
      "ds_read_b64 %3, %10\n\t"
      "ds_read_b64 %4, %10 offset:%13\n\t"
      "ds_read_b64 %5, %10 offset:32\n\t"
      "ds_read_b64 %6, %10 offset:%14\n\t"
      "s_waitcnt lgkmcnt(6)\n\t"
      "v_mfma_f32_16x16x4_f32 %0, %7, %8, %0"
      : "+v"(c), "=&v"(nb0), "=&v"(nb1), "=&v"(d[0]), "=&v"(d[1]), "=&v"(d[2]), "=&v"(d[3])
      : "v"(a), "v"(b), "v"(addr_b), "v"(addr_a), "i"(O), "i"(O + 1024), "i"(PB), "i"(PB + 32)
      : "memory");
}
template <int O>
__device__ __forceinline__ void s2_slot_rbw7(f32x4& c, float a, float b, f32x4& nb0, f32x4& nb1, unsigned addr_b, f32x2 (&d)[7]) {
  asm volatile(
      "ds_read_b128 %1, %12 offset:%13\n\t"
      "ds_read_b128 %2, %12 offset:%14\n\t"
      "s_waitcnt lgkmcnt(2)\n\t"
      "v_mfma_f32_16x16x4_f32 %0, %10, %11, %0"
      : "+v"(c), "=&v"(nb0), "=&v"(nb1), "+v"(d[0]), "+v"(d[1]), "+v"(d[2]), "+v"(d[3]), "+v"(d[4]), "+v"(d[5]), "+v"(d[6])
      : "v"(a), "v"(b), "v"(addr_b), "i"(O), "i"(O + 1024)
      : "memory");
}
template <int O>
__device__ __forceinline__ void s2_slot_rbw4(f32x4& c, float a, float b, f32x4& nb0, f32x4& nb1, unsigned addr_b, f32x2 (&d)[4]) {
  asm volatile(
      "ds_read_b128 %1, %9 offset:%10\n\t"
      "ds_read_b128 %2, %9 offset:%11\n\t"
      "s_waitcnt lgkmcnt(2)\n\t"
      "v_mfma_f32_16x16x4_f32 %0, %7, %8, %0"
      : "+v"(c), "=&v"(nb0), "=&v"(nb1), "+v"(d[0]), "+v"(d[1]), "+v"(d[2]), "+v"(d[3])
      : "v"(a), "v"(b), "v"(addr_b), "i"(O), "i"(O + 1024)
      : "memory");
}

template <int KIND, int SB, int RPER, int NR, int PAR>
struct S2Chunk {
  template <int NPIECES, int I = 0, class D>
  static __device__ __forceinline__ void run(f32x4 (&acc)[7][4], const f32x2 (&v)[7], f32x2 (&vn)[7], f32x2 (&d)[NR], f32x4 (&B)[2][2], unsigned addr_b,
                                             unsigned addr_b_next, unsigned addr_a, D& dma) {
    if constexpr (I < 56) {
      constexpr int P = I / 8, S = (I / 4) % 2, CT = I % 4;
      f32x4(&bc)[2] = B[(P + PAR) & 1];
      f32x4(&bn)[2] = B[(P + PAR + 1) & 1];
      const float bv = bc[CT >> 1][2 * (CT & 1) + S];
      const float av = v[P][S];
      if constexpr (I == 0) {
        if constexpr (NR == 7) s2_slot_rba7<2048, RPER * 32>(acc[0][0], av, bv, bn[0], bn[1], addr_b, d, addr_a);
        else s2_slot_rba4<2048, RPER * 32>(acc[0][0], av, bv, bn[0], bn[1], addr_b, d, addr_a);
      } else if constexpr (I == 8) {
        if constexpr (NR == 7) s2_slot_rbw7<2 * 2048>(acc[1][0], av, bv, bn[0], bn[1], addr_b, d);
        else s2_slot_rbw4<2 * 2048>(acc[1][0], av, bv, bn[0], bn[1], addr_b, d);
      } else if constexpr (I == 48) wino_slot_rb<0, 2>(acc[6][0], av, bv, bn[0], bn[1], addr_b_next);
      else if constexpr (I % 8 == 0) wino_slot_rb<(P + 1) * 2048, 2>(acc[P][0], av, bv, bn[0], bn[1], addr_b);
      else wino_slot(acc[P][CT], av, bv);
      if constexpr ((I & 1) && (I >> 1) < NPIECES) dma(std::integral_constant<int, (I >> 1)>{});
      if constexpr (I == 20) s2_run<KIND, SB, NR, 0, 4>(d, vn);
      if constexpr (I == 36) s2_run<KIND, SB, NR, 4, 7>(d, vn);
      run<NPIECES, I + 1>(acc, v, vn, d, B, addr_b, addr_b_next, addr_a, dma);
    }
  }
};

template <int KIND, int SB>
__global__ __launch_bounds__(256, 2) void conv_wino_s2_kernel(ConvArgs a, const float* __restrict__ U, int off0, int m_tiles, int n_tiles, int patch, int offA,
                                                              int offB) {
#if defined(__HIP_DEVICE_COMPILE__)
  constexpr int KC = 8, NP = 7, WAVES_M = 4;
  constexpr int TT = WAVES_M * 16, TN = 64, NT = 64 * WAVES_M;
  constexpr int NR = KIND == 1 ? 7 : 4;
  constexpr int TS = KIND == 1 ? 4 : 2;
  constexpr int RPER = TT + 1;
  constexpr int SLAB = TS * RPER * KC;
  constexpr int UT = NP * KC * TN;
  constexpr int BUF = SLAB + UT;
  constexpr int STAGE_BYTES = BUF * 4;
  extern __shared__ __attribute__((aligned(16))) float smem[];
  typedef __attribute__((address_space(3))) void* lptr_t;

  const int tid = threadIdx.x, lane = tid & 63, wave = tid >> 6;
  const int n16 = lane & 15, kq = lane >> 4;
  const BlockTile bt = xcd_block_tile(patch, m_tiles, n_tiles);
  const int n_tile = bt.n_tile, m_tile = bt.m_tile, b = bt.b;
  const int t0 = m_tile * TT, n0 = n_tile * TN;

  f32x4 acc[NP][4];
#pragma unroll
  for (int p = 0; p < NP; ++p)
#pragma unroll
    for (int ct = 0; ct < 4; ++ct)
#pragma unroll
      for (int r = 0; r < 4; ++r) acc[p][ct][r] = 0.f;

  const int t_base = TS * t0 + off0;
  const uintptr_t xbp = (uintptr_t)(a.x + (size_t)b * a.Lin * a.Cin);
  const unsigned xb_lo = __builtin_amdgcn_readfirstlane((unsigned)xbp), xb_hi = __builtin_amdgcn_readfirstlane((unsigned)(xbp >> 32));
  const int xbytes = __builtin_amdgcn_readfirstlane(a.Lin * a.Cin * 4);
  const __amdgpu_buffer_rsrc_t xsrd = __builtin_amdgcn_make_buffer_rsrc((void*)(((uintptr_t)xb_hi << 32) | xb_lo), 0, xbytes, 0x00020000);

  constexpr int S_COUNT = SLAB / 4;
  constexpr int S_ITEMS = (S_COUNT + NT - 1) / NT;
  constexpr int W_TOTAL = UT / 4;
  constexpr int W_ITEMS = (W_TOTAL + NT - 1) / NT;
  int soff[S_ITEMS];
#pragma unroll
  for (int it = 0; it < S_ITEMS; ++it) {
    const int id = tid + it * NT;
    const int lr = id >> 1, c4 = id & 1;
    const int r = TS * (lr % RPER) + lr / RPER;
    soff[it] = (id < S_COUNT) ? ((t_base + r) * a.Cin + 4 * c4) * 4 : 0x40000000;
  }
  const uintptr_t wbp = (uintptr_t)U;
  const unsigned wb_lo = __builtin_amdgcn_readfirstlane((unsigned)wbp), wb_hi = __builtin_amdgcn_readfirstlane((unsigned)(wbp >> 32));
  const int wbytes = __builtin_amdgcn_readfirstlane(NP * a.Cin * a.Cout * 4);
  const __amdgpu_buffer_rsrc_t wsrd = __builtin_amdgcn_make_buffer_rsrc((void*)(((uintptr_t)wb_hi << 32) | wb_lo), 0, wbytes, 0x00020000);
  const int w_chunk_bytes = n_tiles * UT * 4;
  int c_next = 0, st_next = 0;
  const int wv64 = __builtin_amdgcn_readfirstlane(tid & ~63);
  auto dma_piece = [&](auto kc) {
    constexpr int k = decltype(kc)::value;
    float* stg = smem + st_next * BUF;
    if constexpr (k < S_ITEMS) {
      if ((k + 1) * NT <= S_COUNT || tid + k * NT < S_COUNT)
        gn_buffer_load_lds(xsrd, (lptr_t)(stg + (k * NT + wv64) * 4), 16, soff[k], c_next * KC * 4, 0, 0);
    } else {
      constexpr int it = k - S_ITEMS;
      if ((it + 1) * NT <= W_TOTAL || wv64 + it * NT < W_TOTAL)
        gn_buffer_load_lds(wsrd, (lptr_t)(stg + SLAB + (it * NT + wv64) * 4), 16, (n_tile * UT + (tid + it * NT) * 4) * 4,
                                                 c_next * w_chunk_bytes, 0, 0);
    }
  };
  constexpr int NPIECES = S_ITEMS + W_ITEMS;
  static_assert(NPIECES <= 8, "staging pieces");
  auto dma_all = [&]() {
    dma_piece(std::integral_constant<int, 0>{});
    dma_piece(std::integral_constant<int, 1>{});
    if constexpr (NPIECES > 2) dma_piece(std::integral_constant<int, 2>{});
    if constexpr (NPIECES > 3) dma_piece(std::integral_constant<int, 3>{});
    if constexpr (NPIECES > 4) dma_piece(std::integral_constant<int, 4>{});
    if constexpr (NPIECES > 5) dma_piece(std::integral_constant<int, 5>{});
    if constexpr (NPIECES > 6) dma_piece(std::integral_constant<int, 6>{});
    if constexpr (NPIECES > 7) dma_piece(std::integral_constant<int, 7>{});
  };

  const unsigned lds0 = (unsigned)(uintptr_t)smem;
  const unsigned base_a = lds0 + (wave * 16 + n16) * 32 + kq * 8;
  const unsigned base_b = lds0 + SLAB * 4 + (kq * 16 + n16) * 16;

  const int n_chunks = a.Cin / KC;
  c_next = 0; st_next = 0; dma_all();
  c_next = min(1, n_chunks - 1); st_next = 1; dma_all();
  __syncthreads();

  f32x2 V0[7], V1[7], d[NR];
  f32x4 Bq[2][2];
  {
    const char* sb = reinterpret_cast<const char*>(smem);
#pragma unroll
    for (int j = 0; j < NR; ++j) d[j] = *reinterpret_cast<const f32x2*>(sb + (base_a - lds0) + (j % TS) * RPER * 32 + (j / TS) * 32);
    s2_run<KIND, SB, NR, 0, 7>(d, V0);
    Bq[0][0] = *reinterpret_cast<const f32x4*>(sb + (base_b - lds0));
    Bq[0][1] = *reinterpret_cast<const f32x4*>(sb + (base_b - lds0) + 1024);
  }
  int st = 0;
  for (int ch = 0; ch < n_chunks; ch += 2) {
#pragma unroll
    for (int half = 0; half < 2; ++half) {
      if (half == 1 && ch + 1 >= n_chunks) break;
      const int st1 = st == 2 ? 0 : st + 1, st2 = st1 == 2 ? 0 : st1 + 1;
      c_next = min(ch + half + 2, n_chunks - 1);
      st_next = st2;
      const unsigned addr_a = base_a + st1 * STAGE_BYTES;
      const unsigned addr_b = base_b + st * STAGE_BYTES, addr_b_next = base_b + st1 * STAGE_BYTES;
      if (half == 0) S2Chunk<KIND, SB, RPER, NR, 0>::template run<NPIECES>(acc, V0, V1, d, Bq, addr_b, addr_b_next, addr_a, dma_piece);
      else S2Chunk<KIND, SB, RPER, NR, 1>::template run<NPIECES>(acc, V1, V0, d, Bq, addr_b, addr_b_next, addr_a, dma_piece);
      __syncthreads();
      st = st1;
    }
  }
  asm volatile("s_nop 15\n\ts_nop 7" : "+v"(acc[6][0]), "+v"(acc[6][1]), "+v"(acc[6][2]), "+v"(acc[6][3]));

  const int m_base = t0 + __builtin_amdgcn_readfirstlane(wave) * 16;
  const int mode = a.gy ? (a.gmask ? 3 : 2) : (a.mask ? 1 : 0);
  ConvArgs a2 = a;
  if constexpr (KIND == 1) {
    f32x4 out[2][4];
#pragma unroll
    for (int ct = 0; ct < 4; ++ct)
#pragma unroll
      for (int r = 0; r < 4; ++r) {
        out[0][ct][r] = ((acc[0][ct][r] + acc[1][ct][r]) + acc[2][ct][r]) + (acc[4][ct][r] + acc[5][ct][r]);
        out[1][ct][r] = ((acc[1][ct][r] - acc[2][ct][r]) - acc[3][ct][r]) + (acc[5][ct][r] + acc[6][ct][r]);
      }
    a2.t.out_stride = 2;
    tile16_epilogue_dispatch<4>(a2, out[0], b, m_base, n0, n16, kq, a.t.out_off, mode);
    tile16_epilogue_dispatch<4>(a2, out[1], b, m_base, n0, n16, kq, a.t.out_off + 1, mode);
    if (a.stat_part) {
      double* red = reinterpret_cast<double*>(smem);
#pragma unroll
      for (int ct = 0; ct < 4; ++ct) {
        const float bias = a.bias ? a.bias[n0 + ct * 16 + n16] : 0.f;
        double s1 = 0.0, s2 = 0.0;
#pragma unroll
        for (int ph = 0; ph < 2; ++ph)
#pragma unroll
          for (int r = 0; r < 4; ++r) {
            const int row = 2 * (m_base + 4 * kq + r) + ph;
            if (row < a.M) {
              const double v = (double)(out[ph][ct][r] + bias);
              s1 += v; s2 += v * v;
            }
          }
        s1 += __shfl_xor(s1, 16, 64); s2 += __shfl_xor(s2, 16, 64);
        s1 += __shfl_xor(s1, 32, 64); s2 += __shfl_xor(s2, 32, 64);
        if (kq == 0) {
          const int slot = (wave * TN + ct * 16 + n16) * 2;
          red[slot] = s1; red[slot + 1] = s2;
        }
      }
      __syncthreads();
      if (tid < TN) {
        double t1 = 0.0, t2 = 0.0;
#pragma unroll
        for (int w = 0; w < WAVES_M; ++w) { t1 += red[(w * TN + tid) * 2]; t2 += red[(w * TN + tid) * 2 + 1]; }
        double* dst = a.stat_part + (size_t)(b * m_tiles + m_tile) * 2 * a.Cout;
        dst[n0 + tid] = t1;
        dst[a.Cout + n0 + tid] = t2;
      }
    }
  } else {
    f32x4 out[4][4];
#pragma unroll
    for (int ct = 0; ct < 4; ++ct)
#pragma unroll
      for (int r = 0; r < 4; ++r) {
        out[0][ct][r] = (acc[0][ct][r] + acc[1][ct][r]) + acc[2][ct][r];
        out[1][ct][r] = (acc[1][ct][r] - acc[2][ct][r]) - acc[3][ct][r];
        out[2][ct][r] = acc[4][ct][r] + acc[5][ct][r];
        out[3][ct][r] = acc[5][ct][r] + acc[6][ct][r];
      }
    a2.t.out_stride = 4;
    tile16_epilogue_dispatch<4>(a2, out[0], b, m_base, n0, n16, kq, offA, mode);
    tile16_epilogue_dispatch<4>(a2, out[1], b, m_base, n0, n16, kq, offA + 2, mode);
    tile16_epilogue_dispatch<4>(a2, out[2], b, m_base, n0, n16, kq, offB, mode);
    tile16_epilogue_dispatch<4>(a2, out[3], b, m_base, n0, n16, kq, offB + 2, mode);
  }
#endif
}

template <int KIND, int SB>
static int launch_s2(const ConvArgs& a, const float* U, int off0, int offA, int offB, hipStream_t s) {
  constexpr int TT = 64, TN = 64, TS = KIND == 1 ? 4 : 2;
  constexpr size_t lds = 3 * sizeof(float) * ((size_t)TS * (TT + 1) * 8 + (size_t)7 * 8 * TN);
  static_assert(lds <= 160 * 1024, "stages too large");
  if (lds > 64 * 1024) {
    static unsigned long long lds_done = 0;
    allow_big_lds((const void*)conv_wino_s2_kernel<KIND, SB>, &lds_done);
  }
  const int tiles = (a.M + 1) / 2;
  const int m_tiles = (tiles + TT - 1) / TT, n_tiles = a.Cout / TN;
  const size_t blocks = (size_t)m_tiles * n_tiles * a.B;
  if (blocks == 0 || blocks > 0x7fffffffull) {
    set_error("conv_wino_s2: bad grid %zu", blocks);
    return GN_EINVAL;
  }
  const int patch = xcd_patch(n_tiles);
  prof_begin(s);
  hipLaunchKernelGGL((conv_wino_s2_kernel<KIND, SB>), dim3((unsigned)blocks), dim3(256), lds, s, a, U, off0, m_tiles, n_tiles, patch, offA, offB);
  prof_end(s, 0.7 * 2.0 * a.B * (double)a.M * 5 * a.Cin * a.Cout, 7, 4.0 * ((double)a.B * a.Lin * a.Cin + 5.0 * a.Cin * a.Cout + (double)a.B * a.M * a.Cout));
  int rc = check_launch("conv_wino_s2");
  if (rc || !a.stat_part) return rc;
  *a.stat_done = 1;
  return colred_finalize(a.stat_part, a.stat_sums, (size_t)2 * a.Cout, a.B * m_tiles, s);
}

size_t conv_wino_s2_workspace_bytes(int Cin, int Cout) { return (size_t)7 * Cin * Cout * sizeof(float); }

int conv_wino_s2_kind(const ConvArgs& a) {
  if (a.t.ntaps != 5 || a.Cin % 8 || a.Cout % 64 || a.Cin < 32) return 0;
  if ((size_t)a.Ly * a.Cout * 4 >= 0x40000000ull || (size_t)a.Lin * a.Cin * 4 >= 0x40000000ull || (size_t)7 * a.Cin * a.Cout * 4 >= 0x40000000ull) return 0;
  if (a.t.in_stride == 2 && a.t.out_stride == 1 && a.t.out_off == 0) {
    for (int j = 0; j < 5; ++j)
      if (a.t.off[j] != a.t.off[0] + j) return 0;
    if (a.stat_part && (a.act != GN_ACT_LINEAR || a.mask || a.gy)) return 0;
    return 1;
  }
  if (a.t.in_stride == 1 && a.t.out_stride == 2 && !a.stat_part && !a.mask && !a.bias) {
    if (a.t.off[0] != a.t.off[2] + 1 || a.t.off[2] != a.t.off[4] + 1 || a.t.off[1] != a.t.off[3] + 1) return 0;
    const int sb = a.t.off[3] - a.t.off[4];
    if (sb != 0 && sb != 1) return 0;
    return 2;
  }
  return 0;
}

int conv_wino_s2_run(const ConvArgs& a, void* ws, size_t ws_bytes, hipStream_t s) {
  const int kind = conv_wino_s2_kind(a);
  if (!kind) {
    set_error("conv_wino_s2: unsupported shape");
    return GN_EINVAL;
  }
  if (!ws || ws_bytes < conv_wino_s2_workspace_bytes(a.Cin, a.Cout)) {
    set_error("conv_wino_s2: workspace too small (%zu < %zu)", ws_bytes, conv_wino_s2_workspace_bytes(a.Cin, a.Cout));
    return GN_EWORKSPACE;
  }
  WinoS2Taps t;
  int off0, offA = 0, offB = 0, sb = 0;
  if (kind == 1) {
    for (int j = 0; j < 5; ++j) t.wq[j] = a.t.widx[j];
    off0 = a.t.off[0];
  } else {
    t.wq[0] = a.t.widx[4]; t.wq[2] = a.t.widx[2]; t.wq[4] = a.t.widx[0];
    t.wq[1] = a.t.widx[3]; t.wq[3] = a.t.widx[1];
    off0 = a.t.off[4];
    sb = a.t.off[3] - a.t.off[4];
    offA = a.t.out_off; offB = a.t.out_off_odd;
  }
  const size_t cc = (size_t)a.Cin * a.Cout;
  hipLaunchKernelGGL(wino_s2_u_kernel, dim3(cdiv(cc, 256)), dim3(256), 0, s, a.w, (float*)ws, a.Cin, a.Cout, t);
  int rc = check_launch("wino_s2_u");
  if (rc) return rc;
  const float* Up = (const float*)ws;
  if (kind == 1) return launch_s2<1, 0>(a, Up, off0, 0, 0, s);
  return sb ? launch_s2<2, 1>(a, Up, off0, offA, offB, s) : launch_s2<2, 0>(a, Up, off0, offA, offB, s);
}

}
```

gennet_amd/csrc/wgrad_wino.hip:

```cpp
#include <stdlib.h>
#include <algorithm>
#include <type_traits>
#include "common.h"
#include "wino_common.h"

namespace gn {

template <int O>
__device__ __forceinline__ void wg_slot_e(f32x4& c, float a, float b, f32x2& e0, f32x2& e1, unsigned addr_b) {
  asm volatile(
      "ds_read2st64_b32 %1, %5 offset0:%6 offset1:%7\n\t"
      "ds_read2st64_b32 %2, %5 offset0:%8 offset1:%9\n\t"
      "v_mfma_f32_16x16x4_f32 %0, %3, %4, %0"
      : "+v"(c), "=&v"(e0), "=&v"(e1)
      : "v"(a), "v"(b), "v"(addr_b), "i"(O), "i"(O + 1), "i"(O + 4), "i"(O + 5)
      : "memory");
}
template <int O, int OA>
__device__ __forceinline__ void wg_slot_ea(f32x4& c, float a, float b, f32x2& e0, f32x2& e1, unsigned addr_b, f32x2 (&d)[6], const unsigned (&addr_a)[3]) {
  asm volatile(
      "ds_read2st64_b32 %1, %11 offset0:%15 offset1:%16\n\t"
      "ds_read2st64_b32 %2, %11 offset0:%17 offset1:%18\n\t"
      "ds_read2st64_b32 %3, %12 offset0:%19 offset1:%20\n\t"
      "ds_read2st64_b32 %4, %12 offset0:%21 offset1:%22\n\t"
      "ds_read2st64_b32 %5, %13 offset0:%19 offset1:%20\n\t"
      "ds_read2st64_b32 %6, %13 offset0:%21 offset1:%22\n\t"
      "ds_read2st64_b32 %7, %14 offset0:%19 offset1:%20\n\t"
      "ds_read2st64_b32 %8, %14 offset0:%21 offset1:%22\n\t"
      "v_mfma_f32_16x16x4_f32 %0, %9, %10, %0"
      : "+v"(c), "=&v"(e0), "=&v"(e1), "=&v"(d[0]), "=&v"(d[1]), "=&v"(d[2]), "=&v"(d[3]), "=&v"(d[4]), "=&v"(d[5])
      : "v"(a), "v"(b), "v"(addr_b), "v"(addr_a[0]), "v"(addr_a[1]), "v"(addr_a[2]), "i"(O), "i"(O + 1), "i"(O + 4), "i"(O + 5), "i"(OA), "i"(OA + 1), "i"(OA + 5),
        "i"(OA + 6)
      : "memory");
}
template <int O>
__device__ __forceinline__ void wg_slot_e_wd(f32x4& c, float a, float b, f32x2& e0, f32x2& e1, unsigned addr_b, f32x2 (&d)[6]) {
  asm volatile(
      "ds_read2st64_b32 %1, %11 offset0:%12 offset1:%13\n\t"
      "ds_read2st64_b32 %2, %11 offset0:%14 offset1:%15\n\t"
      "s_waitcnt lgkmcnt(2)\n\t"
      "v_mfma_f32_16x16x4_f32 %0, %9, %10, %0"
      : "+v"(c), "=&v"(e0), "=&v"(e1), "+v"(d[0]), "+v"(d[1]), "+v"(d[2]), "+v"(d[3]), "+v"(d[4]), "+v"(d[5])
      : "v"(a), "v"(b), "v"(addr_b), "i"(O), "i"(O + 1), "i"(O + 4), "i"(O + 5)
      : "memory");
}

template <int H, int ABL = 0>
struct WgPair {
  template <int NP0, int NP1, int I = 0, class DMA>
  static __device__ __forceinline__ void run(f32x4 (&acc)[6][4], const f32x2 (&v)[6], f32x2 (&vn)[6], f32x2 (&d)[6], WinoT& t, f32x2 (&D)[2][6], unsigned addr_b,
                                             unsigned addr_b_next, const unsigned (&addr_a)[3], const unsigned (&addr_a_next)[3], unsigned long long k15,
                                             unsigned long long km15, DMA& dma) {
    if constexpr (I < 48) {
      constexpr int CT = I / 12, G = I % 12, S = G / 6, P = G % 6;
      f32x2(&dc)[6] = D[CT & 1];
      f32x2(&dn)[6] = D[(CT + 1) & 1];
      const float av = v[P][S], bv = dc[P][S];
      constexpr int OE = (CT < 3) ? (CT + 1) * 8 + 2 * H : (H == 0 ? 2 : 0);
      if constexpr ((ABL & 8) != 0) wino_slot(acc[P][CT], av, bv);
      else if constexpr (I == 0) {
        if constexpr (H == 0) wg_slot_ea<OE, 2>(acc[P][CT], av, bv, dn[0], dn[5], addr_b, d, addr_a);
        else wg_slot_ea<OE, 0>(acc[P][CT], av, bv, dn[0], dn[5], addr_b, d, addr_a_next);
      } else if constexpr (I == 12) wg_slot_e_wd<OE>(acc[P][CT], av, bv, dn[0], dn[5], addr_b, d);
      else if constexpr (G == 0) {
        if constexpr (CT == 3 && H == 1) wg_slot_e<OE>(acc[P][CT], av, bv, dn[0], dn[5], addr_b_next);
        else wg_slot_e<OE>(acc[P][CT], av, bv, dn[0], dn[5], addr_b);
      } else if constexpr (G == 4) wino_slot_w<(I == 4 ? 6 : 0)>(acc[P][CT], av, bv, dn[0], dn[5]);
      else wino_slot(acc[P][CT], av, bv);
      if constexpr (G == 4) {
        constexpr int K = (H == 0 ? 0 : NP0) + CT;
        if constexpr (CT < (H == 0 ? NP0 : NP1)) dma(std::integral_constant<int, K>{});
      }
      if constexpr (!(ABL & 2)) {
        if constexpr (G == 5) {
          wino_a_piece<0>(dn[0], dn[5], dn[1], dn[2], dn[3], dn[4]); wino_a_piece<1>(dn[0], dn[5], dn[1], dn[2], dn[3], dn[4]);
          wino_a_piece<2>(dn[0], dn[5], dn[1], dn[2], dn[3], dn[4]); wino_a_piece<3>(dn[0], dn[5], dn[1], dn[2], dn[3], dn[4]);
        }
        if constexpr (CT == 1 && G == 9) wino_run<0, 5>(d, vn, t, k15, km15);
        if constexpr (CT == 2 && G == 9) wino_run<5, 10>(d, vn, t, k15, km15);
        if constexpr (CT == 3 && G == 9) wino_run<10, kWinoPieces>(d, vn, t, k15, km15);
      }
      run<NP0, NP1, I + 1>(acc, v, vn, d, t, D, addr_b, addr_b_next, addr_a, addr_a_next, k15, km15, dma);
    }
  }
};

template <int ABL = 0>
__global__ __launch_bounds__(256, 2) void wgrad_wino_kernel(WgradArgs a, int off0, int cpb) {
#if defined(__HIP_DEVICE_COMPILE__)
  constexpr int NT = 256;
  constexpr int XS = 4 * 2 * 20 * 16;
  constexpr int YS = 4 * 2 * 16 * 16;
  constexpr int BUF = XS + YS;
  constexpr int STAGE_BYTES = BUF * 4;
  extern __shared__ __attribute__((aligned(16))) float smem[];
  typedef __attribute__((address_space(3))) void* lptr_t;

  const int tid = threadIdx.x, lane = tid & 63, wave = tid >> 6;
  const int n16 = lane & 15, kq = lane >> 4;
  const int ci0 = blockIdx.x * 64, co0 = blockIdx.y * 64, split = blockIdx.z;
  const int total = a.B * cpb;
  const int q_begin = split * a.chunks_per_split, q_end = min(q_begin + a.chunks_per_split, total);

  f32x4 acc[6][4];
#pragma unroll
  for (int p = 0; p < 6; ++p)
#pragma unroll
    for (int ct = 0; ct < 4; ++ct)
#pragma unroll
      for (int r = 0; r < 4; ++r) acc[p][ct][r] = 0.f;

  constexpr int X_ITEMS = 3, Y_ITEMS = 2;
  int xoff[X_ITEMS], yoff[Y_ITEMS];
#pragma unroll
  for (int it = 0; it < X_ITEMS; ++it) {
    const int g = tid + it * NT;
    const int sub = g / 160, rem = g % 160, plane = rem / 80, prow = (rem % 80) >> 2, c4 = rem & 3;
    xoff[it] = ((2 * prow + plane + off0) * a.Cin + ci0 + sub * 16 + 4 * c4) * 4;
  }
#pragma unroll
  for (int it = 0; it < Y_ITEMS; ++it) {
    const int g = tid + it * NT;
    const int ct = g >> 7, rem = g & 127, plane = rem >> 6, tile = (rem & 63) >> 2, c4 = rem & 3;
    yoff[it] = ((2 * tile + plane) * a.Cout + co0 + ct * 16 + 4 * c4) * 4;
  }
  const int xbytes = __builtin_amdgcn_readfirstlane(a.Lin * a.Cin * 4), ybytes = __builtin_amdgcn_readfirstlane(a.M * a.Cout * 4);
  int q_next = 0, st_next = 0;
  bool in_loop = false;
  const int wv64 = __builtin_amdgcn_readfirstlane(tid & ~63);
  auto dma_piece = [&](auto kc) {
    constexpr int k = decltype(kc)::value;
    if ((ABL & 1) && in_loop) return;
    const int b = __builtin_amdgcn_readfirstlane(q_next / cpb), cb = __builtin_amdgcn_readfirstlane(q_next % cpb);
    float* stg = smem + st_next * BUF;
    if constexpr (k < X_ITEMS) {
      if (k < 2 || wv64 < 128) {
        const uintptr_t p = (uintptr_t)(a.x + (size_t)b * a.Lin * a.Cin);
        const __amdgpu_buffer_rsrc_t srd = __builtin_amdgcn_make_buffer_rsrc((void*)p, 0, xbytes, 0x00020000);
        gn_buffer_load_lds(srd, (lptr_t)(stg + (k * NT + wv64) * 4), 16, xoff[k] + cb * 32 * a.Cin * 4, 0, 0, 0);
      }
    } else {
      constexpr int it = k - X_ITEMS;
      const int cbo = cb * 32 * a.Cout * 4;
      const uintptr_t p = (uintptr_t)(a.dy + (size_t)b * a.M * a.Cout) + (uintptr_t)(unsigned)cbo;
      const __amdgpu_buffer_rsrc_t srd = __builtin_amdgcn_make_buffer_rsrc((void*)p, 0, ybytes - cbo, 0x00020000);
      gn_buffer_load_lds(srd, (lptr_t)(stg + XS + (it * NT + wv64) * 4), 16, yoff[it], 0, 0, 0);
    }
  };
  auto dma_all = [&]() {
    dma_piece(std::integral_constant<int, 0>{}); dma_piece(std::integral_constant<int, 1>{}); dma_piece(std::integral_constant<int, 2>{});
    dma_piece(std::integral_constant<int, 3>{}); dma_piece(std::integral_constant<int, 4>{});
  };

  const unsigned lds0 = (unsigned)(uintptr_t)smem;
  unsigned base_a[3];
#pragma unroll
  for (int j2 = 0; j2 < 3; ++j2) base_a[j2] = lds0 + wave * 2560 + ((kq + j2) * 16 + n16) * 4;
  const unsigned base_b = lds0 + XS * 4 + (kq * 16 + n16) * 4;
  const unsigned long long k15 = 0x3fc000003fc00000ull, km15 = 0xbfc00000bfc00000ull;

  if (q_begin < q_end) {
    q_next = q_begin; st_next = 0; dma_all();
    q_next = min(q_begin + 1, q_end - 1); st_next = 1; dma_all();
    __syncthreads();

    f32x2 V0[6], V1[6], d[6], D[2][6];
    WinoT tt;
    {
      const char* sb = reinterpret_cast<const char*>(smem);
#pragma unroll
      for (int j = 0; j < 6; ++j) {
        const float* pp = reinterpret_cast<const float*>(sb + (base_a[j >> 1] - lds0) + (j & 1) * 1280);
        d[j][0] = pp[0]; d[j][1] = pp[64];
      }
      wino_run<0, kWinoPieces>(d, V0, tt, k15, km15);
      const float* pb = reinterpret_cast<const float*>(sb + (base_b - lds0));
      D[0][0][0] = pb[0]; D[0][0][1] = pb[64]; D[0][5][0] = pb[256]; D[0][5][1] = pb[320];
      wino_a_piece<0>(D[0][0], D[0][5], D[0][1], D[0][2], D[0][3], D[0][4]); wino_a_piece<1>(D[0][0], D[0][5], D[0][1], D[0][2], D[0][3], D[0][4]);
      wino_a_piece<2>(D[0][0], D[0][5], D[0][1], D[0][2], D[0][3], D[0][4]); wino_a_piece<3>(D[0][0], D[0][5], D[0][1], D[0][2], D[0][3], D[0][4]);
    }
    int st = 0;
    in_loop = true;
    for (int q = q_begin; q < q_end; ++q) {
      const int st1 = st == 2 ? 0 : st + 1, st2 = st1 == 2 ? 0 : st1 + 1;
      q_next = min(q + 2, q_end - 1);
      st_next = st2;
      unsigned addr_a[3], addr_a_next[3];
#pragma unroll
      for (int j2 = 0; j2 < 3; ++j2) { addr_a[j2] = base_a[j2] + st * STAGE_BYTES; addr_a_next[j2] = base_a[j2] + st1 * STAGE_BYTES; }
      const unsigned addr_b = base_b + st * STAGE_BYTES, addr_b_next = base_b + st1 * STAGE_BYTES;
      WgPair<0, ABL>::template run<3, 2>(acc, V0, V1, d, tt, D, addr_b, addr_b_next, addr_a, addr_a_next, k15, km15, dma_piece);
      WgPair<1, ABL>::template run<3, 2>(acc, V1, V0, d, tt, D, addr_b, addr_b_next, addr_a, addr_a_next, k15, km15, dma_piece);
      if constexpr (!(ABL & 4)) __syncthreads();
      st = st1;
    }
    asm volatile("s_nop 15\n\ts_nop 7" : "+v"(acc[5][0]), "+v"(acc[5][1]), "+v"(acc[5][2]), "+v"(acc[5][3]));
  }

  const size_t cc = (size_t)a.Cin * a.Cout;
#pragma unroll
  for (int p = 0; p < 6; ++p) {
    float* dst = a.part + ((size_t)split * 6 + p) * cc + (size_t)(ci0 + wave * 16 + 4 * kq) * a.Cout + co0 + n16;
#pragma unroll
    for (int ct = 0; ct < 4; ++ct)
#pragma unroll
      for (int r = 0; r < 4; ++r) dst[(size_t)r * a.Cout + ct * 16] = acc[p][ct][r];
  }
#endif
}

__global__ void wgrad_wino_reduce_kernel(const float* __restrict__ part, float* __restrict__ dw, size_t cc, int splits) {
  const size_t i = (size_t)blockIdx.x * blockDim.x + threadIdx.x;
  if (i >= cc) return;
  double Q[6] = {0, 0, 0, 0, 0, 0};
#pragma unroll 4
  for (int s = 0; s < splits; ++s)
#pragma unroll
    for (int p = 0; p < 6; ++p) Q[p] += (double)part[((size_t)s * 6 + p) * cc + i];
  const double e = (Q[1] + Q[2]) * (1.0 / 3.0), o = (Q[1] - Q[2]) * (1.0 / 3.0);
  dw[i] = (float)(Q[0] + e + Q[3] * (16.0 / 15.0) + Q[4] * (1.0 / 30.0));
  dw[cc + i] = (float)(o + Q[3] * (8.0 / 15.0) - Q[4] * (2.0 / 30.0));
  dw[2 * cc + i] = (float)(e + Q[3] * (4.0 / 15.0) + Q[4] * (4.0 / 30.0));
  dw[3 * cc + i] = (float)(o + Q[3] * (2.0 / 15.0) - Q[4] * (8.0 / 30.0));
  dw[4 * cc + i] = (float)(e + Q[3] * (1.0 / 15.0) + Q[4] * (16.0 / 30.0) + Q[5]);
}

bool wgrad_wino_supported(const WgradArgs& a) {
  if (a.ntaps != 5 || a.in_stride != 1 || a.Cin % 64 || a.Cout % 64) return false;
  for (int j = 0; j < 5; ++j)
    if (a.off[j] != a.off[0] + j) return false;
  return (size_t)a.Lin * a.Cin * 4 < 0x40000000ull && (size_t)a.M * a.Cout * 4 < 0x40000000ull;
}

size_t wgrad_wino_workspace_bytes(int B, int M, int Cin, int Cout) {
  int s, cps;
  wgrad_split_plan(B, M, Cin, Cout, 64, 64, &s, &cps);
  return (size_t)s * 6 * Cin * Cout * sizeof(float);
}

int wgrad_wino_run(WgradArgs& a, float* dw, hipStream_t s) {
  if (!wgrad_wino_supported(a)) {
    set_error("wgrad_wino: unsupported shape");
    return GN_EINVAL;
  }
  int splits;
  wgrad_split_plan(a.B, a.M, a.Cin, a.Cout, 64, 64, &splits, &a.chunks_per_split);
  const int cpb = (a.M + 31) / 32;
  constexpr size_t lds = 3 * sizeof(float) * (4 * 2 * 20 * 16 + 4 * 2 * 16 * 16);
  dim3 grid(a.Cin / 64, a.Cout / 64, splits);
  prof_begin(s);
#ifdef GN_ABLATION
  static const int abl = getenv("GN_WGWINO_ABL") ? atoi(getenv("GN_WGWINO_ABL")) : 0;
  if (abl == 1) hipLaunchKernelGGL(wgrad_wino_kernel<1>, grid, dim3(256), lds, s, a, a.off[0], cpb);
  else if (abl == 2) hipLaunchKernelGGL(wgrad_wino_kernel<2>, grid, dim3(256), lds, s, a, a.off[0], cpb);
  else if (abl == 8) hipLaunchKernelGGL(wgrad_wino_kernel<8>, grid, dim3(256), lds, s, a, a.off[0], cpb);
  else if (abl == 15) hipLaunchKernelGGL(wgrad_wino_kernel<15>, grid, dim3(256), lds, s, a, a.off[0], cpb);
  else
#endif
  hipLaunchKernelGGL(wgrad_wino_kernel<0>, grid, dim3(256), lds, s, a, a.off[0], cpb);
  prof_end(s, 0.6 * 2.0 * a.B * (double)a.M * 5 * a.Cin * a.Cout, 6, 4.0 * ((double)a.B * a.Lin * a.Cin + (double)a.B * a.M * a.Cout + 5.0 * a.Cin * a.Cout));
  int rc = check_launch("wgrad_wino");
  if (rc) return rc;
  const size_t cc = (size_t)a.Cin * a.Cout;
  hipLaunchKernelGGL(wgrad_wino_reduce_kernel, dim3(cdiv(cc, 256)), dim3(256), 0, s, a.part, dw, cc, splits);
  return check_launch("wgrad_wino_reduce");
}

}
```

gennet_amd/csrc/wgrad_wino_s2.hip:

```cpp
#include <stdlib.h>
#include <algorithm>
#include <type_traits>
#include "common.h"
#include "wino_common.h"

namespace gn {

template <int O>
__device__ __forceinline__ void wg2_slot_e(f32x4& c, float a, float b, f32x2& e0, f32x2& e1, unsigned addr_b) {
  asm volatile(
      "ds_read2st64_b32 %1, %5 offset0:%6 offset1:%7\n\t"
      "ds_read2st64_b32 %2, %5 offset0:%8 offset1:%9\n\t"
      "v_mfma_f32_16x16x4_f32 %0, %3, %4, %0"
      : "+v"(c), "=&v"(e0), "=&v"(e1)
      : "v"(a), "v"(b), "v"(addr_b), "i"(O), "i"(O + 1), "i"(O + 2), "i"(O + 3)
      : "memory");
}
template <int O>
__device__ __forceinline__ void wg2_slot_ea(f32x4& c, float a, float b, f32x2& e0, f32x2& e1, unsigned addr_b, f32x2 (&d)[7], const unsigned (&addr_a)[2]) {
  asm volatile(
      "ds_read2st64_b32 %1, %12 offset0:%15 offset1:%16\n\t"
      "ds_read2st64_b32 %2, %12 offset0:%17 offset1:%18\n\t"
      "ds_read2st64_b32 %3, %13 offset0:0 offset1:1\n\t"
      "ds_read2st64_b32 %4, %13 offset0:3 offset1:4\n\t"
      "ds_read2st64_b32 %5, %13 offset0:6 offset1:7\n\t"
      "ds_read2st64_b32 %6, %13 offset0:9 offset1:10\n\t"
      "ds_read2st64_b32 %7, %14 offset0:0 offset1:1\n\t"
      "ds_read2st64_b32 %8, %14 offset0:3 offset1:4\n\t"
      "ds_read2st64_b32 %9, %14 offset0:6 offset1:7\n\t"
      "v_mfma_f32_16x16x4_f32 %0, %10, %11, %0"
      : "+v"(c), "=&v"(e0), "=&v"(e1), "=&v"(d[0]), "=&v"(d[1]), "=&v"(d[2]), "=&v"(d[3]), "=&v"(d[4]), "=&v"(d[5]), "=&v"(d[6])
      : "v"(a), "v"(b), "v"(addr_b), "v"(addr_a[0]), "v"(addr_a[1]), "i"(O), "i"(O + 1), "i"(O + 2), "i"(O + 3)
      : "memory");
}
template <int O>
__device__ __forceinline__ void wg2_slot_e_wd(f32x4& c, float a, float b, f32x2& e0, f32x2& e1, unsigned addr_b, f32x2 (&d)[7]) {
  asm volatile(
      "ds_read2st64_b32 %1, %12 offset0:%13 offset1:%14\n\t"
      "ds_read2st64_b32 %2, %12 offset0:%15 offset1:%16\n\t"
      "s_waitcnt lgkmcnt(2)\n\t"
      "v_mfma_f32_16x16x4_f32 %0, %10, %11, %0"
      : "+v"(c), "=&v"(e0), "=&v"(e1), "+v"(d[0]), "+v"(d[1]), "+v"(d[2]), "+v"(d[3]), "+v"(d[4]), "+v"(d[5]), "+v"(d[6])
      : "v"(a), "v"(b), "v"(addr_b), "i"(O), "i"(O + 1), "i"(O + 2), "i"(O + 3)
      : "memory");
}

struct Wg2Chunk {
  template <int NPIECES, int I = 0, class DMA>
  static __device__ __forceinline__ void run(f32x4 (&acc)[7][4], const f32x2 (&v)[7], f32x2 (&vn)[7], f32x2 (&d)[7], f32x2 (&D)[2][4], unsigned addr_b,
                                             unsigned addr_b_next, const unsigned (&addr_a_next)[2], DMA& dma) {
    if constexpr (I < 56) {
      constexpr int CT = I / 14, G = I % 14, S = G / 7, P = G % 7;
      constexpr int BI = (P == 0 || P == 4) ? 0 : ((P == 1 || P == 5) ? 2 : (P == 2 ? 3 : 1));
      f32x2(&dc)[4] = D[CT & 1];
      f32x2(&dn)[4] = D[(CT + 1) & 1];
      const float av = v[P][S], bv = dc[BI][S];
      constexpr int OE = (CT < 3) ? (CT + 1) * 4 : 0;
      if constexpr (I == 0) wg2_slot_ea<OE>(acc[P][CT], av, bv, dn[0], dn[1], addr_b, d, addr_a_next);
      else if constexpr (I == 14) wg2_slot_e_wd<OE>(acc[P][CT], av, bv, dn[0], dn[1], addr_b, d);
      else if constexpr (G == 0) {
        if constexpr (CT == 3) wg2_slot_e<OE>(acc[P][CT], av, bv, dn[0], dn[1], addr_b_next);
        else wg2_slot_e<OE>(acc[P][CT], av, bv, dn[0], dn[1], addr_b);
      } else if constexpr (G == 4) wino_slot_w<(I == 4 ? 7 : 0)>(acc[P][CT], av, bv, dn[0], dn[1]);
      else wino_slot(acc[P][CT], av, bv);
      if constexpr (G == 4 && CT < NPIECES) dma(std::integral_constant<int, CT>{});
      if constexpr (G == 5) {
        GN_PK_ADD(dn[2], dn[0], dn[1]);
        GN_PK_SUB(dn[3], dn[0], dn[1]);
      }
      if constexpr (CT == 1 && G == 9) s2_run<1, 0, 7, 0, 4>(d, vn);
      if constexpr (CT == 2 && G == 9) s2_run<1, 0, 7, 4, 7>(d, vn);
      run<NPIECES, I + 1>(acc, v, vn, d, D, addr_b, addr_b_next, addr_a_next, dma);
    }
  }
};

__global__ __launch_bounds__(256, 2) void wgrad_wino_s2_kernel(WgradArgs a, int off0, int cpb) {
#if defined(__HIP_DEVICE_COMPILE__)
  constexpr int NT = 256;
  constexpr int XS = 4 * 4 * 12 * 16;
  constexpr int YS = 4 * 2 * 8 * 16;
  constexpr int BUF = XS + YS;
  constexpr int STAGE_BYTES = BUF * 4;
  extern __shared__ __attribute__((aligned(16))) float smem[];
  typedef __attribute__((address_space(3))) void* lptr_t;

  const int tid = threadIdx.x, lane = tid & 63, wave = tid >> 6;
  const int n16 = lane & 15, kq = lane >> 4;
  const int ci0 = blockIdx.x * 64, co0 = blockIdx.y * 64, split = blockIdx.z;
  const int total = a.B * cpb;
  const int q_begin = split * a.chunks_per_split, q_end = min(q_begin + a.chunks_per_split, total);

  f32x4 acc[7][4];
#pragma unroll
  for (int p = 0; p < 7; ++p)
#pragma unroll
    for (int ct = 0; ct < 4; ++ct)
#pragma unroll
      for (int r = 0; r < 4; ++r) acc[p][ct][r] = 0.f;

  constexpr int X_ITEMS = 3;
  int xoff[X_ITEMS], yoff;
#pragma unroll
  for (int it = 0; it < X_ITEMS; ++it) {
    const int g = tid + it * NT;
    const int sub = g / 192, rem = g % 192, plane = rem / 48, prow = (rem % 48) >> 2, c4 = rem & 3;
    xoff[it] = ((4 * prow + plane + off0) * a.Cin + ci0 + sub * 16 + 4 * c4) * 4;
  }
  {
    const int g = tid;
    const int ct = g >> 6, rem = g & 63, plane = rem >> 5, tile = (rem & 31) >> 2, c4 = rem & 3;
    yoff = ((2 * tile + plane) * a.Cout + co0 + ct * 16 + 4 * c4) * 4;
  }
  const int xbytes = __builtin_amdgcn_readfirstlane(a.Lin * a.Cin * 4), ybytes = __builtin_amdgcn_readfirstlane(a.M * a.Cout * 4);
  int q_next = 0, st_next = 0;
  const int wv64 = __builtin_amdgcn_readfirstlane(tid & ~63);
  auto dma_piece = [&](auto kc) {
    constexpr int k = decltype(kc)::value;
    const int b = __builtin_amdgcn_readfirstlane(q_next / cpb), cb = __builtin_amdgcn_readfirstlane(q_next % cpb);
    float* stg = smem + st_next * BUF;
    if constexpr (k < X_ITEMS) {
      const uintptr_t p = (uintptr_t)(a.x + (size_t)b * a.Lin * a.Cin);
      const __amdgpu_buffer_rsrc_t srd = __builtin_amdgcn_make_buffer_rsrc((void*)p, 0, xbytes, 0x00020000);
      gn_buffer_load_lds(srd, (lptr_t)(stg + (k * NT + wv64) * 4), 16, xoff[k] + cb * 32 * a.Cin * 4, 0, 0, 0);
    } else {
      const int cbo = cb * 16 * a.Cout * 4;
      const uintptr_t p = (uintptr_t)(a.dy + (size_t)b * a.M * a.Cout) + (uintptr_t)(unsigned)cbo;
      const __amdgpu_buffer_rsrc_t srd = __builtin_amdgcn_make_buffer_rsrc((void*)p, 0, ybytes - cbo, 0x00020000);
      gn_buffer_load_lds(srd, (lptr_t)(stg + XS + wv64 * 4), 16, yoff, 0, 0, 0);
    }
  };
  auto dma_all = [&]() {
    dma_piece(std::integral_constant<int, 0>{}); dma_piece(std::integral_constant<int, 1>{}); dma_piece(std::integral_constant<int, 2>{});
    dma_piece(std::integral_constant<int, 3>{});
  };

  const unsigned lds0 = (unsigned)(uintptr_t)smem;
  unsigned base_a[2];
#pragma unroll
  for (int j4 = 0; j4 < 2; ++j4) base_a[j4] = lds0 + wave * 3072 + ((kq + j4) * 16 + n16) * 4;
  const unsigned base_b = lds0 + XS * 4 + (kq * 16 + n16) * 4;

  if (q_begin < q_end) {
    q_next = q_begin; st_next = 0; dma_all();
    q_next = min(q_begin + 1, q_end - 1); st_next = 1; dma_all();
    __syncthreads();

    f32x2 V0[7], V1[7], d[7], D[2][4];
    {
      const char* sb = reinterpret_cast<const char*>(smem);
#pragma unroll
      for (int j = 0; j < 7; ++j) {
        const float* pp = reinterpret_cast<const float*>(sb + (base_a[j >> 2] - lds0) + (j & 3) * 768);
        d[j][0] = pp[0]; d[j][1] = pp[64];
      }
      s2_run<1, 0, 7, 0, 7>(d, V0);
      const float* pb = reinterpret_cast<const float*>(sb + (base_b - lds0));
      D[0][0][0] = pb[0]; D[0][0][1] = pb[64]; D[0][1][0] = pb[128]; D[0][1][1] = pb[192];
      GN_PK_ADD(D[0][2], D[0][0], D[0][1]);
      GN_PK_SUB(D[0][3], D[0][0], D[0][1]);
    }
    int st = 0;
    for (int q = q_begin; q < q_end; q += 2) {
#pragma unroll
      for (int half = 0; half < 2; ++half) {
        if (half == 1 && q + 1 >= q_end) break;
        const int st1 = st == 2 ? 0 : st + 1, st2 = st1 == 2 ? 0 : st1 + 1;
        q_next = min(q + half + 2, q_end - 1);
        st_next = st2;
        unsigned addr_a_next[2];
#pragma unroll
        for (int j4 = 0; j4 < 2; ++j4) addr_a_next[j4] = base_a[j4] + st1 * STAGE_BYTES;
        const unsigned addr_b = base_b + st * STAGE_BYTES, addr_b_next = base_b + st1 * STAGE_BYTES;
        if (half == 0) Wg2Chunk::run<4>(acc, V0, V1, d, D, addr_b, addr_b_next, addr_a_next, dma_piece);
        else Wg2Chunk::run<4>(acc, V1, V0, d, D, addr_b, addr_b_next, addr_a_next, dma_piece);
        __syncthreads();
        st = st1;
      }
    }
    asm volatile("s_nop 15\n\ts_nop 7" : "+v"(acc[6][0]), "+v"(acc[6][1]), "+v"(acc[6][2]), "+v"(acc[6][3]));
  }

  const size_t cc = (size_t)a.Cin * a.Cout;
#pragma unroll
  for (int p = 0; p < 7; ++p) {
    float* dst = a.part + ((size_t)split * 7 + p) * cc + (size_t)(ci0 + wave * 16 + 4 * kq) * a.Cout + co0 + n16;
#pragma unroll
    for (int ct = 0; ct < 4; ++ct)
#pragma unroll
      for (int r = 0; r < 4; ++r) dst[(size_t)r * a.Cout + ct * 16] = acc[p][ct][r];
  }
#endif
}

__global__ void wgrad_wino_s2_reduce_kernel(const float* __restrict__ part, float* __restrict__ dw, size_t cc, int splits) {
  const size_t i = (size_t)blockIdx.x * blockDim.x + threadIdx.x;
  if (i >= cc) return;
  double Q[7] = {0, 0, 0, 0, 0, 0, 0};
#pragma unroll 4
  for (int s = 0; s < splits; ++s)
#pragma unroll
    for (int p = 0; p < 7; ++p) Q[p] += (double)part[((size_t)s * 7 + p) * cc + i];
  dw[i] = (float)(Q[0] + 0.5 * (Q[1] + Q[2]));
  dw[cc + i] = (float)(Q[4] + Q[5]);
  dw[2 * cc + i] = (float)(0.5 * (Q[1] - Q[2]));
  dw[3 * cc + i] = (float)(Q[5] + Q[6]);
  dw[4 * cc + i] = (float)(0.5 * (Q[1] + Q[2]) - Q[3]);
}

static void s2_plan(int B, int M, int Cin, int Cout, int* splits, int* cps16, int* cpb16) {
  int s, cps32;
  wgrad_split_plan(B, M, Cin, Cout, 64, 64, &s, &cps32);
  *cpb16 = (M + 15) / 16;
  const int cpb32 = (M + 31) / 32;
  if (cps32 % cpb32 == 0) *cps16 = (cps32 / cpb32) * *cpb16;
  else *cps16 = 2 * cps32;
  const long total = (long)B * *cpb16;
  *splits = (int)((total + *cps16 - 1) / *cps16);
}

bool wgrad_wino_s2_supported(const WgradArgs& a) {
  if (a.ntaps != 5 || a.in_stride != 2 || a.Cin % 64 || a.Cout % 64) return false;
  for (int j = 0; j < 5; ++j)
    if (a.off[j] != a.off[0] + j) return false;
  return (size_t)a.Lin * a.Cin * 4 < 0x40000000ull && (size_t)a.M * a.Cout * 4 < 0x40000000ull;
}

size_t wgrad_wino_s2_workspace_bytes(int B, int M, int Cin, int Cout) {
  int s, cps, cpb;
  s2_plan(B, M, Cin, Cout, &s, &cps, &cpb);
  return (size_t)s * 7 * Cin * Cout * sizeof(float);
}

int wgrad_wino_s2_run(WgradArgs& a, float* dw, hipStream_t s) {
  if (!wgrad_wino_s2_supported(a)) {
    set_error("wgrad_wino_s2: unsupported shape");
    return GN_EINVAL;
  }
  int splits, cpb;
  s2_plan(a.B, a.M, a.Cin, a.Cout, &splits, &a.chunks_per_split, &cpb);
  constexpr size_t lds = 3 * sizeof(float) * (4 * 4 * 12 * 16 + 4 * 2 * 8 * 16);
  dim3 grid(a.Cin / 64, a.Cout / 64, splits);
  prof_begin(s);
  hipLaunchKernelGGL(wgrad_wino_s2_kernel, grid, dim3(256), lds, s, a, a.off[0], cpb);
  prof_end(s, 0.7 * 2.0 * a.B * (double)a.M * 5 * a.Cin * a.Cout, 8, 4.0 * ((double)a.B * a.Lin * a.Cin + (double)a.B * a.M * a.Cout + 5.0 * a.Cin * a.Cout));
  int rc = check_launch("wgrad_wino_s2");
  if (rc) return rc;
  const size_t cc = (size_t)a.Cin * a.Cout;
  hipLaunchKernelGGL(wgrad_wino_s2_reduce_kernel, dim3(cdiv(cc, 256)), dim3(256), 0, s, a.part, dw, cc, splits);
  return check_launch("wgrad_wino_s2_reduce");
}

}
```

gennet_amd/ops.py:

```python
import torch

from . import _lib

ACT = {'linear': 0, None: 0, 'relu': 1, 'relu_max': 2, 'leaky': 3, 'tanh': 4, 'sigmoid': 5}

_ws = {}


def _stream():
    return torch.cuda.current_stream().cuda_stream


def _p(t):
    return None if t is None else t.data_ptr()


def _chk(*ts):
    for t in ts:
        if t is None:
            continue
        if not t.is_cuda:
            raise _lib.GennetHipError('gennet_amd ops need CUDA (HIP) tensors; got a %s tensor -- there is no CPU path' % t.device)
        if not t.is_contiguous():
            raise ValueError('non-contiguous tensor passed to a gennet_amd op')
# ... 445 lines not shown
    _lib.call('gn_subtract_stack_bwd', _p(dimg), _p(dx), B, n, _stream())
    return dx


def affine_stack_fwd(x, a0, b0, a1, b1):
    _chk(x)
    B, n = x.shape[0], x.shape[1]
    img = torch.empty((B, n, 2, 1), dtype=torch.float32, device=x.device)
    _lib.call('gn_affine_stack_fwd', _p(x), _p(b0), _p(b1), float(a0), float(a1), _p(img), B, n, _stream())
    return img


def affine_stack_bwd(dimg, a0, a1):
    _chk(dimg)
    B, n = dimg.shape[0], dimg.shape[1]
    dx = torch.empty((B, n, 1), dtype=torch.float32, device=dimg.device)
    _lib.call('gn_affine_stack_bwd', _p(dimg), float(a0), float(a1), _p(dx), B, n, _stream())
    return dx


def assemble_d_batch(real, noise, fake, event):
    _chk(real, noise, fake, event)
    B, n = real.shape[0], real.shape[1]
    sX = torch.empty((2 * B, n, 2, 1), dtype=torch.float32, device=real.device)
    _lib.call('gn_assemble_d_batch', _p(real), _p(noise), _p(fake), _p(event), _p(sX), B, n, _stream())
    return sX


def fill_uniform(shape, lo, hi, seed, offset, device):
    t = torch.empty(shape, dtype=torch.float32, device=device)
    _lib.call('gn_fill_uniform', _p(t), t.numel(), float(lo), float(hi), int(seed), int(offset), _stream())
    return t


def fill_normal(shape, mean, std, seed, offset, device):
    t = torch.empty(shape, dtype=torch.float32, device=device)
    if isinstance(std, DevScalar):
        _lib.call('gn_fill_normal_dyn', _p(t), t.numel(), float(mean), std.ptr, int(seed), int(offset), _stream())
    else:
        _lib.call('gn_fill_normal', _p(t), t.numel(), float(mean), float(std), int(seed), int(offset), _stream())
    return t


def _noise_out(x, out):
    _chk(x, out)
    return torch.empty_like(x) if out is None else out


def gaussian_noise(x, stddev, seed, offset, out=None):
    y = _noise_out(x, out)
    _lib.call('gn_gaussian_noise_fwd', _p(x), _p(y), x.numel(), float(stddev), int(seed), int(offset), _stream())
    return y


def gaussian_dropout(x, sd, seed, offset, out=None):
    y = _noise_out(x, out)
    _lib.call('gn_gaussian_dropout_apply', _p(x), _p(y), x.numel(), float(sd), int(seed), int(offset), _stream())
    return y


def alpha_dropout_fwd(x, rate, a, b, alpha_p, seed, offset, out=None):
    y = _noise_out(x, out)
    _lib.call('gn_alpha_dropout_fwd', _p(x), _p(y), x.numel(), float(rate), float(a), float(b), float(alpha_p), int(seed), int(offset), _stream())
    return y


def alpha_dropout_bwd(dy, rate, a, seed, offset, out=None):
    dx = _noise_out(dy, out)
    _lib.call('gn_alpha_dropout_bwd', _p(dy), _p(dx), dy.numel(), float(rate), float(a), int(seed), int(offset), _stream())
    return dx


def gather_rows(src, idx):
    _chk(src, idx)
    rows, width = idx.numel(), src.shape[1]
    out = torch.empty((rows, width), dtype=torch.float32, device=src.device)
    _lib.call('gn_gather_rows', _p(src), _p(idx), _p(out), rows, width, _stream())
    return out


def axpy(y, x, a):
    _chk(y, x)
    _lib.call('gn_axpy', _p(y), _p(x), float(a), y.numel(), _stream())
    return y


def bn_stats(x2d):
    _chk(x2d)
    rows, Cc = x2d.shape
    sums = torch.empty((2 * Cc,), dtype=torch.float64, device=x2d.device)
    nb = _lib.size('gn_bn_stats_workspace', rows, Cc)
    ws = workspace(nb, x2d.device)
    _lib.call('gn_bn_stats', _p(x2d), rows, Cc, _p(sums), _p(ws), ws.numel(), _stream())
    return sums


def bn_finalize(sums, count, gamma, beta, eps, momentum, moving_mean, moving_var, zero_debias=None):
    Cc = gamma.numel()
    dev = gamma.device
    scale, shift, smean, sinv = (torch.empty((Cc,), dtype=torch.float32, device=dev) for _ in range(4))
    if zero_debias is not None:
        bm, bv, step = zero_debias
        if isinstance(step, DevScalar):
            _lib.call('gn_bn_finalize_zero_debias_dyn', _p(sums), float(count), _p(gamma), _p(beta), float(eps), float(momentum), _p(moving_mean), _p(moving_var),
                      _p(bm), _p(bv), step.ptr, _p(scale), _p(shift), _p(smean), _p(sinv), Cc, _stream())
        else:
            _lib.call('gn_bn_finalize_zero_debias', _p(sums), float(count), _p(gamma), _p(beta), float(eps), float(momentum), _p(moving_mean), _p(moving_var),
                      _p(bm), _p(bv), int(step), _p(scale), _p(shift), _p(smean), _p(sinv), Cc, _stream())
    else:
        _lib.call('gn_bn_finalize', _p(sums), float(count), _p(gamma), _p(beta), float(eps), float(momentum), _p(moving_mean), _p(moving_var),
                  _p(scale), _p(shift), _p(smean), _p(sinv), Cc, _stream())
    return scale, shift, smean, sinv


def bn_infer_coeffs(gamma, beta, moving_mean, moving_var, eps):
    Cc = gamma.numel()
    scale, shift = (torch.empty((Cc,), dtype=torch.float32, device=gamma.device) for _ in range(2))
    _lib.call('gn_bn_infer_coeffs', _p(gamma), _p(beta), _p(moving_mean), _p(moving_var), float(eps), _p(scale), _p(shift), Cc, _stream())
    return scale, shift


def bn_apply(x2d, scale, shift, mask=None, act='linear', act_param=0.0, rate=0.0):
    _chk(x2d, mask)
    rows, Cc = x2d.shape
    y = torch.empty_like(x2d)
    _lib.call('gn_bn_apply', _p(x2d), _p(scale), _p(shift), _p(mask), _p(y), rows, Cc, ACT[act], float(act_param), float(rate), _stream())
    return y


def bn_apply_dropgen(x2d, scale, shift, act, act_param, rate, seed, offset):
    _chk(x2d)
    rows, Cc = x2d.shape
    y = torch.empty_like(x2d)
    mask = torch.empty((rows, Cc), dtype=torch.uint8, device=x2d.device)
    _lib.call('gn_bn_apply_dropgen', _p(x2d), _p(scale), _p(shift), _p(mask), _p(y), rows, Cc, ACT[act], float(act_param), float(rate), int(seed), int(offset),
              _stream())
    return y, mask


def bn_bwd_stats(dy2d, y2d, x2d, mask, smean, sinv, act='linear', act_param=0.0, rate=0.0, scale=None, shift=None):
    _chk(dy2d, y2d, x2d, mask)
    rows, Cc = x2d.shape
    dsums = torch.empty((2 * Cc,), dtype=torch.float64, device=x2d.device)
    nb = _lib.size('gn_bn_stats_workspace', rows, Cc)
    ws = workspace(nb, x2d.device)
    _lib.call('gn_bn_bwd_stats', _p(dy2d), _p(y2d), _p(x2d), _p(mask), _p(smean), _p(sinv), _p(dsums), _p(ws), ws.numel(), rows, Cc,
              ACT[act], float(act_param), float(rate), _p(scale), _p(shift), _stream())
    return dsums


def bn_bwd_apply(dy2d, y2d, x2d, mask, gamma, smean, sinv, dsums_global, count, dsums_local, dgamma, dbeta, act='linear', act_param=0.0, rate=0.0,
                 scale=None, shift=None):
    rows, Cc = x2d.shape
    dx = torch.empty_like(x2d)
    _lib.call('gn_bn_bwd_apply', _p(dy2d), _p(y2d), _p(x2d), _p(mask), _p(gamma), _p(smean), _p(sinv), _p(dsums_global), float(count),
              _p(dsums_local), _p(dx), _p(dgamma), _p(dbeta), rows, Cc, ACT[act], float(act_param), float(rate), _p(scale), _p(shift), _stream())
    return dx


class ConvGrad1(object):

    def __init__(self, g, w, L, pad_left):
        _chk(g, w)
        self.g, self.w, self.L, self.pad_left = g, w, int(L), int(pad_left)
        self.B, self.Lout = int(g.shape[0]), int(g.shape[1])
        self.k, self.C = int(w.shape[0]), int(w.shape[1])
        self.shape = (self.B, self.L, self.C)


def bn_bwd_stats_conv1(cg, x2d, mask, smean, sinv, act, act_param, rate, scale, shift):
    _chk(x2d, mask)
    rows, Cc = x2d.shape
    assert rows == cg.B * cg.L and Cc == cg.C
    dsums = torch.empty((2 * Cc,), dtype=torch.float64, device=x2d.device)
    ws = workspace(_lib.size('gn_bn_stats_workspace', rows, Cc), x2d.device)
    _lib.call('gn_bn_bwd_stats_conv1', _p(cg.g), _p(cg.w), cg.L, cg.Lout, cg.k, cg.pad_left, _p(x2d), _p(mask), _p(smean), _p(sinv), _p(dsums), _p(ws),
              ws.numel(), rows, Cc, ACT[act], float(act_param), float(rate), _p(scale), _p(shift), _stream())
    return dsums


def bn_bwd_apply_conv1(cg, x2d, mask, gamma, smean, sinv, dsums_global, count, dsums_local, dgamma, dbeta, act, act_param, rate, scale, shift):
    rows, Cc = x2d.shape
    dx = torch.empty_like(x2d)
    _lib.call('gn_bn_bwd_apply_conv1', _p(cg.g), _p(cg.w), cg.L, cg.Lout, cg.k, cg.pad_left, _p(x2d), _p(mask), _p(gamma), _p(smean), _p(sinv),
              _p(dsums_global), float(count), _p(dsums_local), _p(dx), _p(dgamma), _p(dbeta), rows, Cc, ACT[act], float(act_param), float(rate),
              _p(scale), _p(shift), _stream())
    return dx


def loss(kind, p, y, Bglobal=None):
    _chk(p, y)
    B = p.shape[0]
    dp = torch.empty_like(p)
    out = torch.empty((2,), dtype=torch.float32, device=p.device)
    fn = {'binary_crossentropy': 'gn_bce_loss', 'mean_squared_error': 'gn_mse_loss'}[kind]
    _lib.call(fn, _p(p), _p(y), _p(dp), _p(out), B, int(Bglobal or B), _stream())
    return dp, out


LOSS_KINDS = {'binary_crossentropy': 0, 'mean_squared_error': 1, 'mean_absolute_error': 2, 'mean_absolute_percentage_error': 3,
              'mean_squared_logarithmic_error': 4, 'hinge': 5, 'squared_hinge': 6, 'logcosh': 7, 'poisson': 8, 'kullback_leibler_divergence': 9,
              'categorical_crossentropy': 10, 'cosine_proximity': 11, 'categorical_accuracy': 12}
LOSS_ALIASES = {'mse': 'mean_squared_error', 'mae': 'mean_absolute_error', 'mape': 'mean_absolute_percentage_error',
                'msle': 'mean_squared_logarithmic_error', 'kld': 'kullback_leibler_divergence', 'cosine': 'cosine_proximity'}
LOSS_PASS_MIN_ELEMENTS = 131072


def loss_pass(kind, p, y, denom=None, grad=True, dp=None):
    _chk(p, y, dp)
    rows, cols = p.shape
    if grad and dp is None:
        dp = torch.empty_like(p)
    out = torch.empty((2,), dtype=torch.float32, device=p.device)
    ws = workspace(_lib.size('gn_loss_pass_workspace', rows, cols), p.device)
    _lib.call('gn_loss_pass', LOSS_KINDS.get(kind, kind), _p(p), _p(y), _p(dp) if grad else None, _p(out), rows, cols, float(rows if denom is None else denom),
              _p(ws), ws.numel(), _stream())
    return (dp if grad else None), out


def weight_count(w, count=None):
    _chk(w, count)
    if count is None:
        count = torch.empty((1,), dtype=torch.float64, device=w.device)
    ws = workspace(_lib.size('gn_weight_count_workspace', w.numel()), w.device)
    _lib.call('gn_weight_count', _p(w), w.numel(), _p(count), _p(ws), ws.numel(), _stream())
    return count


def loss_pass_weighted(kind, p, y, w, count, grad=True, dp=None):
    _chk(p, y, w, count, dp)
    rows, cols = p.shape
    if w.numel() != rows or w.dtype != torch.float32:
        raise ValueError('loss_pass_weighted: %d float32 weights expected, got %s %s' % (rows, tuple(w.shape), w.dtype))
    if count.numel() != 1 or count.dtype != torch.float64:
        raise ValueError('loss_pass_weighted: count is one float64 value on the device')
    if grad and dp is None:
        dp = torch.empty_like(p)
    out = torch.empty((3,), dtype=torch.float32, device=p.device)
    ws = workspace(_lib.size('gn_loss_pass_weighted_workspace', rows, cols), p.device)
    _lib.call('gn_loss_pass_weighted', LOSS_KINDS.get(kind, kind), _p(p), _p(y), _p(w), _p(count), _p(dp) if grad else None, _p(out), rows, cols,
              _p(ws), ws.numel(), _stream())
    return (dp if grad else None), out


def adam_step(p, g, m, v, lr_t, b1, b2, eps):
    _chk(p, g, m, v)
    if isinstance(lr_t, DevScalar):
        _lib.call('gn_adam_step_dyn', _p(p), _p(g), _p(m), _p(v), p.numel(), lr_t.ptr, float(b1), float(b2), float(eps), _stream())
    else:
        _lib.call('gn_adam_step', _p(p), _p(g), _p(m), _p(v), p.numel(), float(lr_t), float(b1), float(b2), float(eps), _stream())


OPT_RULES = {'sgd': 0, 'rmsprop': 1, 'adagrad': 2, 'adadelta': 3, 'adamax': 4, 'adam': 5, 'amsgrad': 6}


def optim_step(rule, p, g, states, lr, h0=0.0, h1=0.0, eps=0.0, nesterov=False, clip_scale=None, clipvalue=0.0):
    _chk(p, g, *states)
    st = [_p(s) for s in states] + [None] * (3 - len(states))
    dyn = isinstance(lr, DevScalar)
    _lib.call('gn_optim_step', OPT_RULES[rule], _p(p), _p(g), st[0], st[1], st[2], p.numel(), 0.0 if dyn else float(lr), lr.ptr if dyn else None,
              float(h0), float(h1), float(eps), 1 if nesterov else 0, None if clip_scale is None else _p(clip_scale), float(clipvalue), _stream())


def optim_sumsq_slots(n):
    return _lib.size('gn_optim_sumsq_slots', int(n))


def optim_sumsq(g, partials):
    _chk(g)
    _lib.call('gn_optim_sumsq', _p(g), g.numel(), _p(partials), _stream())


def optim_clip_factor(partials, clipnorm, factor):
    _lib.call('gn_optim_clip_factor', _p(partials), partials.numel(), float(clipnorm), _p(factor), _stream())


class DevScalar(object):

    def __init__(self, ptr):
        self.ptr = int(ptr)


def set_rng_base(ptr):
    _lib.call('gn_set_rng_base', None if ptr is None else int(ptr))


_PROF_ON = False


def prof_enable(on=True):
    global _PROF_ON
    _PROF_ON = bool(on)
    _lib.call('gn_prof_enable', 1 if on else 0)


def prof_enabled():
    return _PROF_ON


def prof_reset():
    _lib.call('gn_prof_reset')


def prof_collect(kind=-1):
    import ctypes
    out = (ctypes.c_double * 4)()
    _lib.call('gn_prof_collect', int(kind), ctypes.cast(out, ctypes.c_void_p))
    return {'launches': int(out[0]), 'ms': out[1], 'flop': out[2], 'bytes': out[3]}
```

include/gennet_hip.h:

```cpp
#ifndef GENNET_HIP_H
#define GENNET_HIP_H

#include <stddef.h>
#include <stdint.h>

#ifdef __cplusplus
extern "C" {
#endif

#define GN_OK 0
#define GN_EINVAL (-1)
#define GN_ELAUNCH (-2)
#define GN_EWORKSPACE (-3)

enum gn_act { GN_ACT_LINEAR = 0, GN_ACT_RELU = 1, GN_ACT_RELU_MAX = 2, GN_ACT_LEAKY = 3, GN_ACT_TANH = 4, GN_ACT_SIGMOID = 5 };

const char* gn_last_error(void);
int gn_version(void);

int gn_conv1d_fwd(const float* x, const float* w, const float* bias, float* y,
                  int B, int L, int Cin, int Cout, int k, int stride, int pad_left, int Lout,
                  int act, float act_param, void* stream);

size_t gn_conv1d_bf16x3_workspace(int B, int L, int Cin, int Cout, int k);
int gn_conv1d_fwd_bf16x3(const float* x, const float* w, const float* bias, float* y, void* ws, size_t ws_bytes,
                         int B, int L, int Cin, int Cout, int k, int stride, int pad_left, int Lout,
                         int act, float act_param, int resplit, void* stream);
size_t gn_conv1d_wino_workspace(int Cin, int Cout);
int gn_conv1d_fwd_wino(const float* x, const float* w, const float* bias, float* y, void* ws, size_t ws_bytes,
                       int B, int L, int Cin, int Cout, int k, int stride, int pad_left, int Lout,
                       int act, float act_param, void* stream);
int gn_set_conv_math(int mode, void* workspace, size_t workspace_bytes);

int gn_conv1d_fwd_dropout(const float* x, const float* w, const float* bias, const uint8_t* mask, float* y,
                          int B, int L, int Cin, int Cout, int k, int stride, int pad_left, int Lout,
                          int act, float act_param, float rate, void* stream);
size_t gn_conv1d_fwd_stats_workspace(int B, int Lout, int Cout);
int gn_conv1d_fwd_stats(const float* x, const float* w, const float* bias, float* y, double* sums, void* ws, size_t ws_bytes,
                        int B, int L, int Cin, int Cout, int k, int stride, int pad_left, int Lout, void* stream);

int gn_conv1d_transpose_w(const float* w, float* wt, int k, int Cin, int Cout, void* stream);

int gn_conv1d_dgrad(const float* dy, const float* wt, float* dx,
                    int B, int L, int Cin, int Cout, int k, int stride, int pad_left, int Lout, void* stream);

int gn_conv1d_dgrad_fused(const float* dy, const float* wt, float* dx,
                          int B, int L, int Cin, int Cout, int k, int stride, int pad_left, int Lout,
                          const float* y_prev, const uint8_t* mask_prev, int act_prev, float act_param_prev, float rate_prev, void* stream);

size_t gn_conv1d_wgrad_workspace(int B, int L, int Cin, int Cout, int k, int stride, int Lout);
int gn_conv1d_wgrad(const float* x, const float* dy, float* dw, float* db, void* ws, size_t ws_bytes,
                    int B, int L, int Cin, int Cout, int k, int stride, int pad_left, int Lout, void* stream);

int gn_conv1d_needs_any(int Cin, int Cout);
int gn_conv1d_fwd_any(const float* x, const float* w, const float* bias, float* y,
                      int B, int L, int Cin, int Cout, int k, int stride, int pad_left, int Lout,
                      int act, float act_param, void* stream);
int gn_conv1d_dgrad_any(const float* dy, const float* wt, float* dx,
                        int B, int L, int Cin, int Cout, int k, int stride, int pad_left, int Lout, void* stream);
int gn_conv1d_wgrad_any(const float* x, const float* dy, float* dw, float* db, void* ws, size_t ws_bytes,
                        int B, int L, int Cin, int Cout, int k, int stride, int pad_left, int Lout, void* stream);

int gn_conv2d_w2_fold(const float* w, const float* bias, float* wf, float* biasf, int kh, int Cin, int Cout, void* stream);
int gn_conv2d_w2_unfold_grad(const float* dwf, const float* dbf, float* dw, float* db, int kh, int Cin, int Cout, void* stream);
int gn_conv1d_tap_groups(int k, int* groups, int* taps);
int gn_conv1d_tapfold_x(const float* x, float* x2, int B, int L, int Cin, int k, int pad_left, void* stream);
int gn_conv1d_tapunfold_dx(const float* dx2, float* dx, int B, int L, int Cin, int k, int pad_left, void* stream);
int gn_conv1d_tapfold_w(const float* w, float* w2, int k, int Cin, int Cout, void* stream);
int gn_conv1d_tapunfold_dw(const float* dw2, float* dw, int k, int Cin, int Cout, void* stream);

int gn_conv1d_up2_fold(const float* w, const float* bias, float* wf, float* biasf, int Cin, int Cout, int stride, void* stream);
int gn_conv1d_up2_unfold_grad(const float* dwf, const float* dbf, float* dw, float* db, int Cin, int Cout, int stride, void* stream);

int gn_dense_fwd(const float* x, const float* w, const float* bias, float* y, int B, int in, int out,
                 int act, float act_param, void* stream);
size_t gn_dense_bwd_workspace(int B, int in, int out);
int gn_dense_bwd(const float* x, const float* w, const float* dy, float* dx, float* dw, float* db,
                 void* ws, size_t ws_bytes, int B, int in, int out, void* stream);

int gn_dense_bwd_fused(const float* x, const float* w, const float* dy, float* dx, float* dw, float* db, int B, int in, int out,
                       const uint8_t* mask_prev, int act_prev, float act_param_prev, float rate_prev, void* stream);

int gn_act_fwd(const float* x, float* y, size_t n, int act, float act_param, void* stream);
int gn_act_bwd(const float* dy, const float* y, float* dx, size_t n, int act, float act_param, void* stream);
int gn_act_dropout_bwd(const float* dy, const float* y, const uint8_t* mask, float* dx, size_t n, int act, float act_param, float rate, void* stream);
int gn_bn_apply_dropgen(const float* x, const float* scale, const float* shift, uint8_t* mask_out, float* y, size_t rows, int C,
                        int act, float act_param, float rate, uint64_t seed, uint64_t offset, void* stream);
int gn_bias_act_dropout(float* y, const float* bias, uint8_t* mask, size_t rows, int C, int act, float act_param, float rate, int gen,
                        uint64_t seed, uint64_t offset, void* stream);
size_t gn_bias_grad_workspace(size_t rows, int C);
int gn_bias_grad(const float* dy, float* db, void* ws, size_t ws_bytes, size_t rows, int C, void* stream);
int gn_conv_fold_bn(const float* w, const float* bias, const float* scale, const float* shift, float* w_out, float* bias_out,
                    size_t rows, int Cout, void* stream);
int gn_prelu_fwd(const float* x, const float* alpha, float* y, int B, size_t F, void* stream);
int gn_prelu_bwd(const float* dy, const float* x, const float* alpha, float* dx, float* dalpha, int B, size_t F, void* stream);
int gn_dropout_mask(uint8_t* mask, size_t n, float rate, uint64_t seed, uint64_t offset, void* stream);
int gn_dropout_apply(const float* x, const uint8_t* mask, float* y, size_t n, float rate, void* stream);
int gn_upsample2_fwd(const float* x, float* y, int B, int L, int C, void* stream);
int gn_upsample2_bwd(const float* dy, float* dx, int B, int L, int C, void* stream);
int gn_maxpool_h2_fwd(const float* x, float* y, int B, int H, int R, void* stream);
int gn_maxpool_h2_bwd(const float* dy, const float* x, float* dx, int B, int H, int R, void* stream);
int gn_subtract_stack_fwd(const float* x, const float* event, float* img, int B, int n, void* stream);
int gn_subtract_stack_bwd(const float* dimg, float* dx, int B, int n, void* stream);
int gn_affine_stack_fwd(const float* x, const float* b0, const float* b1, float a0, float a1, float* img, int B, int n, void* stream);
int gn_affine_stack_bwd(const float* dimg, float a0, float a1, float* dx, int B, int n, void* stream);
int gn_assemble_d_batch(const float* real, const float* noise, const float* fake, const float* event, float* sX, int B, int n, void* stream);
int gn_fill_uniform(float* out, size_t n, float lo, float hi, uint64_t seed, uint64_t offset, void* stream);
int gn_fill_normal(float* out, size_t n, float mean, float std, uint64_t seed, uint64_t offset, void* stream);
int gn_gaussian_noise_fwd(const float* x, float* y, size_t n, float stddev, uint64_t seed, uint64_t offset, void* stream);
int gn_gaussian_dropout_apply(const float* x, float* y, size_t n, float sd, uint64_t seed, uint64_t offset, void* stream);
int gn_alpha_dropout_fwd(const float* x, float* y, size_t n, float rate, float a, float b, float alpha_p, uint64_t seed, uint64_t offset, void* stream);
int gn_alpha_dropout_bwd(const float* dy, float* dx, size_t n, float rate, float a, uint64_t seed, uint64_t offset, void* stream);
int gn_gather_rows(const float* src, const int64_t* idx, float* out, int rows, int width, void* stream);
int gn_axpy(float* y, const float* x, float a, size_t n, void* stream);

size_t gn_bn_stats_workspace(size_t rows, int C);
int gn_bn_stats(const float* x, size_t rows, int C, double* sums, void* ws, size_t ws_bytes, void* stream);
int gn_bn_finalize(const double* sums, double count, const float* gamma, const float* beta, float eps, float momentum,
                   float* moving_mean, float* moving_var, float* scale, float* shift,
                   float* save_mean, float* save_invstd, int C, void* stream);
int gn_bn_finalize_zero_debias(const double* sums, double count, const float* gamma, const float* beta, float eps, float momentum,
                               float* moving_mean, float* moving_var, float* biased_mean, float* biased_var, int local_step,
                               float* scale, float* shift, float* save_mean, float* save_invstd, int C, void* stream);
int gn_bn_infer_coeffs(const float* gamma, const float* beta, const float* moving_mean, const float* moving_var,
                       float eps, float* scale, float* shift, int C, void* stream);
int gn_bn_apply(const float* x, const float* scale, const float* shift, const uint8_t* mask, float* y,
                size_t rows, int C, int act, float act_param, float rate, void* stream);
int gn_bn_bwd_stats(const float* dy, const float* y, const float* x, const uint8_t* mask,
                    const float* save_mean, const float* save_invstd, double* dsums, void* ws, size_t ws_bytes,
                    size_t rows, int C, int act, float act_param, float rate, const float* scale, const float* shift, void* stream);
int gn_bn_bwd_apply(const float* dy, const float* y, const float* x, const uint8_t* mask,
                    const float* gamma, const float* save_mean, const float* save_invstd,
                    const double* dsums_global, double count, const double* dsums_local, float* dx, float* dgamma, float* dbeta,
                    size_t rows, int C, int act, float act_param, float rate, const float* scale, const float* shift, void* stream);

int gn_bn_bwd_stats_conv1(const float* g, const float* w, int L, int Lout, int k, int pad_left, const float* x, const uint8_t* mask,
                          const float* save_mean, const float* save_invstd, double* dsums, void* ws, size_t ws_bytes, size_t rows, int C,
                          int act, float act_param, float rate, const float* scale, const float* shift, void* stream);
int gn_bn_bwd_apply_conv1(const float* g, const float* w, int L, int Lout, int k, int pad_left, const float* x, const uint8_t* mask,
                          const float* gamma, const float* save_mean, const float* save_invstd, const double* dsums_global, double count,
                          const double* dsums_local, float* dx, float* dgamma, float* dbeta, size_t rows, int C, int act, float act_param,
                          float rate, const float* scale, const float* shift, void* stream);

int gn_bce_loss(const float* p, const float* y, float* dp, float* out, int B, int Bglobal, void* stream);
int gn_mse_loss(const float* p, const float* y, float* dp, float* out, int B, int Bglobal, void* stream);

enum gn_loss {
  GN_LOSS_BINARY_CROSSENTROPY = 0, GN_LOSS_MEAN_SQUARED_ERROR = 1, GN_LOSS_MEAN_ABSOLUTE_ERROR = 2, GN_LOSS_MEAN_ABSOLUTE_PERCENTAGE_ERROR = 3,
  GN_LOSS_MEAN_SQUARED_LOGARITHMIC_ERROR = 4, GN_LOSS_HINGE = 5, GN_LOSS_SQUARED_HINGE = 6, GN_LOSS_LOGCOSH = 7, GN_LOSS_POISSON = 8,
  GN_LOSS_KULLBACK_LEIBLER_DIVERGENCE = 9, GN_LOSS_CATEGORICAL_CROSSENTROPY = 10, GN_LOSS_COSINE_PROXIMITY = 11,
  GN_LOSS_CATEGORICAL_ACCURACY = 12, GN_LOSS_KINDS = 13
};
size_t gn_loss_pass_workspace(long long rows, int cols);
int gn_loss_pass(int kind, const float* p, const float* y, float* dp, float* out, long long rows, int cols, double denom,
                 void* ws, size_t ws_bytes, void* stream);

size_t gn_weight_count_workspace(long long rows);
int gn_weight_count(const float* w, long long rows, double* count, void* ws, size_t ws_bytes, void* stream);
size_t gn_loss_pass_weighted_workspace(long long rows, int cols);
int gn_loss_pass_weighted(int kind, const float* p, const float* y, const float* w, const double* count, float* dp, float* out,
                          long long rows, int cols, void* ws, size_t ws_bytes, void* stream);

int gn_adam_step(float* p, const float* g, float* m, float* v, size_t n, float lr_t, float b1, float b2, float eps, void* stream);

enum gn_optim_rule { GN_OPT_SGD = 0, GN_OPT_RMSPROP = 1, GN_OPT_ADAGRAD = 2, GN_OPT_ADADELTA = 3, GN_OPT_ADAMAX = 4, GN_OPT_ADAM = 5, GN_OPT_AMSGRAD = 6 };
int gn_optim_step(int rule, float* p, const float* g, float* s0, float* s1, float* s2, size_t n, float lr, const float* lr_dev, float h0, float h1,
                  float eps, int nesterov, const float* clip_scale, float clipvalue, void* stream);
size_t gn_optim_sumsq_slots(size_t n);
int gn_optim_sumsq(const float* g, size_t n, double* partials, void* stream);
int gn_optim_clip_factor(const double* partials, size_t count, float clipnorm, float* factor, void* stream);

int gn_set_rng_base(const uint64_t* base_dev);
int gn_adam_step_dyn(float* p, const float* g, float* m, float* v, size_t n, const float* lr_t_dev, float b1, float b2, float eps, void* stream);
int gn_fill_normal_dyn(float* out, size_t n, float mean, const float* sd_dev, uint64_t seed, uint64_t offset, void* stream);
int gn_bn_finalize_zero_debias_dyn(const double* sums, double count, const float* gamma, const float* beta, float eps, float momentum,
                                   float* moving_mean, float* moving_var, float* biased_mean, float* biased_var, const int32_t* local_step_dev,
                                   float* scale, float* shift, float* save_mean, float* save_invstd, int C, void* stream);

int gn_prof_enable(int on);
int gn_prof_reset(void);
int gn_prof_collect(int kind, double* out4_host);

int gn_chirp_fd_whitened(const double* m1, const double* m2, const double* scale, double* out_hp, double* out_hc,
                         int nb, int Nf, double df, double f_low, double dist_mpc, double iota, double phi0, void* stream);
int gn_irfft_f64(const double* X, double* out, const double* twiddle, int nb, int N, void* stream);
int gn_rfft_f64(const double* x, double* X, const double* twiddle, int nb, int N, void* stream);
int gn_align_crop(const double* hp, const double* hc, const int32_t* idx, double* out, int32_t* ref_out,
                  int nb, int N, int roll, int crop0, int crop_len, int peak_off, double Fp, double Fc, double g, void* stream);
int gn_synth_templates(const double* m1, const double* m2, const int32_t* idx, const double* scale, const double* twiddle,
                       double* out_f64, float* out_f32, int32_t* ref_idx, int nb, int N, int roll, int crop0, int crop_len,
                       int peak_off, double df, double f_low, double dist_mpc, double iota, double phi0, double Fp, double Fc, double g,
                       void* stream);
int gn_synth_templates_prior(const double* scale, const double* twiddle, double* out_f64, float* out_f32, float* labels, double* m_out,
                             int32_t* idx_out, int32_t* ref_idx, int nb, int N, int roll, int crop0, int crop_len, int peak_off,
                             double df, double f_low, double dist_mpc, double iota, double phi0, double Fp, double Fc, double g,
                             uint64_t seed, uint64_t counter, int idx_lo, int idx_hi, double m_min, double M_max, void* stream);
int gn_noise_whitened(const double* amp, const double* wscale, const double* window, const double* twiddle, const double* normals_in,
                      double* normals_out, const double* add_f64, double* out_f64, float* out_f32, int nb, int N, int crop0, int crop_len,
                      double df, uint64_t seed, uint64_t counter, void* stream);
int gn_synth_templates_noise(const double* m1, const double* m2, const int32_t* idx, const double* scale, const double* twiddle,
                             const double* noise_amp, const double* window, double* out_f64, float* out_f32, float* labels, double* m_out,
                             int32_t* idx_out, int32_t* ref_idx, int nb, int N, int roll, int crop0, int crop_len, int peak_off, double df,
                             double f_low, double dist_mpc, double iota, double phi0, double Fp, double Fc, double g, uint64_t seed,
                             uint64_t counter, int idx_lo, int idx_hi, double m_min, double M_max, uint64_t noise_seed,
                             uint64_t noise_counter, double* normals_out, void* stream);
int gn_noise_fd(const double* amp, double* X, int nb, int Nf, uint64_t seed, uint64_t offset, void* stream);
int gn_scale_f64(double* x, double s, size_t n, void* stream);
int gn_mul_f64(double* x, const double* w, size_t n, size_t period, int complex_x, void* stream);
int gn_f64_to_f32(const double* x, float* y, double s, size_t n, void* stream);

int gn_kde2d_pdf(const double* data, int n, const double* pts, int m, double inv00, double inv01, double inv11, double norm,
                 double* out, void* stream);

#ifdef __cplusplus
}
#endif
#endif
```

Measured before the change: 1949.

## Restructure Winograd wgrad kernels for three blocks per CU with compile-time stages

Result: no change. 1967 (median of 6 runs) (+0.9%).

```diff
diff --git a/gennet_amd/_lib.py b/gennet_amd/_lib.py
--- a/gennet_amd/_lib.py
+++ b/gennet_amd/_lib.py
@@ -123,6 +123,11 @@
 }
 
 
+_COUNTS = {
+    'gn_kernel_blocks_per_cu': [i32],
+}
+
+
 class GennetHipError(RuntimeError):
     pass
 
@@ -139,7 +144,7 @@
                                      '(hipcc --offload-arch=gfx950); gennet_amd has no CPU fallback' % (LIB_PATH, e))
         import torch
         L = C.CDLL(LIB_PATH)
-        for table, restype in ((_SIGS, i32), (_SIZE_FNS, sz), (_PREDICATES, i32)):
+        for table, restype in ((_SIGS, i32), (_SIZE_FNS, sz), (_PREDICATES, i32), (_COUNTS, i32)):
             for name, args in table.items():
                 try:
                     fn = getattr(L, name)
@@ -154,7 +159,7 @@
 
 
 def exported_symbols():
-    return sorted(list(_SIGS) + list(_SIZE_FNS) + list(_PREDICATES) + ['gn_last_error', 'gn_version'])
+    return sorted(list(_SIGS) + list(_SIZE_FNS) + list(_PREDICATES) + list(_COUNTS) + ['gn_last_error', 'gn_version'])
 
 
 def call(name, *args):
@@ -179,3 +184,15 @@
     except AttributeError:
         raise GennetHipError('%s is not exported by %s (stale build?)' % (name, LIB_PATH))
     return bool(fn(*args))
+
+
+def count(name, *args):
+    L = lib()
+    try:
+        fn = getattr(L, name)
+    except AttributeError:
+        raise GennetHipError('%s is not exported by %s (stale build?)' % (name, LIB_PATH))
+    n = fn(*args)
+    if n < 0:
+        raise GennetHipError('%s failed (%d): %s' % (name, n, L.gn_last_error().decode()))
+    return int(n)
diff --git a/gennet_amd/csrc/capi.hip b/gennet_amd/csrc/capi.hip
--- a/gennet_amd/csrc/capi.hip
+++ b/gennet_amd/csrc/capi.hip
@@ -267,6 +267,19 @@
 
 const char* gn_last_error(void) { return g_err; }
 int gn_version(void) { return 100; }
+
+int gn_kernel_blocks_per_cu(int kind) {
+  int n;
+  switch (kind) {
+    case 5: n = conv_wino_blocks_per_cu(); break;
+    case 6: n = wgrad_wino_blocks_per_cu(); break;
+    case 7: n = conv_wino_s2_blocks_per_cu(); break;
+    case 8: n = wgrad_wino_s2_blocks_per_cu(); break;
+    default: set_error("gn_kernel_blocks_per_cu: kind %d is not one of the transform-domain kernels (5 .. 8)", kind); return -1;
+  }
+  if (n < 0) set_error("gn_kernel_blocks_per_cu: the occupancy query of kind %d failed", kind);
+  return n;
+}
 
 int gn_prof_enable(int on) {
   g_prof_on = on != 0;
diff --git a/gennet_amd/csrc/common.h b/gennet_amd/csrc/common.h
--- a/gennet_amd/csrc/common.h
+++ b/gennet_amd/csrc/common.h
@@ -123,16 +123,20 @@
 size_t conv_wino_workspace_bytes(int Cin, int Cout);
 bool conv_wino_supported(const ConvArgs& a);
 int conv_wino_run(const ConvArgs& a, void* ws, size_t ws_bytes, hipStream_t s);
+int conv_wino_blocks_per_cu();
 size_t conv_wino_s2_workspace_bytes(int Cin, int Cout);
 int conv_wino_s2_kind(const ConvArgs& a);
 int conv_wino_s2_run(const ConvArgs& a, void* ws, size_t ws_bytes, hipStream_t s);
+int conv_wino_s2_blocks_per_cu();
 void wgrad_split_plan(int B, int M, int Cin, int Cout, int TC, int TN, int* splits, int* chunks_per_split);
 bool wgrad_wino_supported(const WgradArgs& a);
 size_t wgrad_wino_workspace_bytes(int B, int M, int Cin, int Cout);
 int wgrad_wino_run(WgradArgs& a, float* dw, hipStream_t s);
+int wgrad_wino_blocks_per_cu();
 bool wgrad_wino_s2_supported(const WgradArgs& a);
 size_t wgrad_wino_s2_workspace_bytes(int B, int M, int Cin, int Cout);
 int wgrad_wino_s2_run(WgradArgs& a, float* dw, hipStream_t s);
+int wgrad_wino_s2_blocks_per_cu();
 size_t wgrad_bf16x3_workspace_bytes(int B, int M, int Cin, int Cout, int in_stride);
 bool wgrad_bf16x3_supported(const WgradArgs& a);
 int wgrad_bf16x3_run(const WgradArgs& a, int splits, void* ws, size_t ws_bytes, hipStream_t s);
diff --git a/gennet_amd/csrc/conv_wino.hip b/gennet_amd/csrc/conv_wino.hip
--- a/gennet_amd/csrc/conv_wino.hip
+++ b/gennet_amd/csrc/conv_wino.hip
@@ -262,10 +262,15 @@
 #endif
 }
 
+template <int WAVES_M>
+constexpr size_t conv_wino_lds_bytes() {
+  return 3 * sizeof(float) * ((size_t)2 * (WAVES_M * 16 + 2) * 8 + (size_t)6 * 8 * 64);
+}
+
 template <int WAVES_M, int ABL = 0>
 static int launch_conv_wino(const ConvArgs& a, const float* U, int off0, hipStream_t s) {
   constexpr int TT = WAVES_M * 16, TN = 64;
-  constexpr size_t lds = 3 * sizeof(float) * ((size_t)2 * (TT + 2) * 8 + (size_t)6 * 8 * TN);
+  constexpr size_t lds = conv_wino_lds_bytes<WAVES_M>();
   static_assert(lds <= 160 * 1024, "stages too large");
   if (lds > 64 * 1024) {
     static unsigned long long lds_done = 0;
@@ -289,6 +294,12 @@
 }
 
 size_t conv_wino_workspace_bytes(int Cin, int Cout) { return (size_t)6 * Cin * Cout * sizeof(float); }
+
+int conv_wino_blocks_per_cu() {
+  int n = 0;
+  if (hipOccupancyMaxActiveBlocksPerMultiprocessor(&n, (const void*)conv_wino_kernel<4, 0>, 256, conv_wino_lds_bytes<4>()) != hipSuccess) return -1;
+  return n;
+}
 
 bool conv_wino_supported(const ConvArgs& a) {
   if (a.t.ntaps != 5 || a.t.in_stride != 1 || a.t.out_stride != 1 || a.t.out_off != 0) return false;
diff --git a/gennet_amd/csrc/conv_wino_s2.hip b/gennet_amd/csrc/conv_wino_s2.hip
--- a/gennet_amd/csrc/conv_wino_s2.hip
+++ b/gennet_amd/csrc/conv_wino_s2.hip
@@ -304,10 +304,15 @@
 #endif
 }
 
+template <int KIND>
+constexpr size_t conv_wino_s2_lds_bytes() {
+  return 3 * sizeof(float) * ((size_t)(KIND == 1 ? 4 : 2) * (64 + 1) * 8 + (size_t)7 * 8 * 64);
+}
+
 template <int KIND, int SB>
 static int launch_s2(const ConvArgs& a, const float* U, int off0, int offA, int offB, hipStream_t s) {
-  constexpr int TT = 64, TN = 64, TS = KIND == 1 ? 4 : 2;
-  constexpr size_t lds = 3 * sizeof(float) * ((size_t)TS * (TT + 1) * 8 + (size_t)7 * 8 * TN);
+  constexpr int TT = 64, TN = 64;
+  constexpr size_t lds = conv_wino_s2_lds_bytes<KIND>();
   static_assert(lds <= 160 * 1024, "stages too large");
   if (lds > 64 * 1024) {
     static unsigned long long lds_done = 0;
@@ -331,6 +336,19 @@
 }
 
 size_t conv_wino_s2_workspace_bytes(int Cin, int Cout) { return (size_t)7 * Cin * Cout * sizeof(float); }
+
+template <int KIND, int SB>
+static int s2_blocks_per_cu() {
+  constexpr size_t lds = conv_wino_s2_lds_bytes<KIND>();
+  if (lds > 64 * 1024) {
+    static unsigned long long lds_done = 0;
+    allow_big_lds((const void*)conv_wino_s2_kernel<KIND, SB>, &lds_done);
+  }
+  int n = 0;
+  if (hipOccupancyMaxActiveBlocksPerMultiprocessor(&n, (const void*)conv_wino_s2_kernel<KIND, SB>, 256, lds) != hipSuccess) return -1;
+  return n;
+}
+int conv_wino_s2_blocks_per_cu() { return std::min(s2_blocks_per_cu<1, 0>(), std::min(s2_blocks_per_cu<2, 0>(), s2_blocks_per_cu<2, 1>())); }
 
 int conv_wino_s2_kind(const ConvArgs& a) {
   if (a.t.ntaps != 5 || a.Cin % 8 || a.Cout % 64 || a.Cin < 32) return 0;
diff --git a/gennet_amd/csrc/wgrad_wino.hip b/gennet_amd/csrc/wgrad_wino.hip
--- a/gennet_amd/csrc/wgrad_wino.hip
+++ b/gennet_amd/csrc/wgrad_wino.hip
@@ -5,6 +5,16 @@
 #include "wino_common.h"
 
 namespace gn {
+
+constexpr int kWgXSubRows = 38, kWgXPlaneRows = 20;
+constexpr int kWgXS = 4 * kWgXSubRows * 16;
+constexpr int kWgYS = 4 * 2 * 16 * 16;
+constexpr int kWgStageBytes = (kWgXS + kWgYS) * 4;
+constexpr int kWgStageUnits = kWgStageBytes / 256;
+constexpr size_t kWgLdsBytes = 3 * (size_t)kWgStageBytes;
+static_assert(kWgStageBytes % 256 == 0 && 2 * kWgStageUnits + 31 <= 255, "stage offsets must fit the 8-bit read2st64 offsets");
+static_assert(kWgXPlaneRows % 4 == 0 && kWgXPlaneRows >= 18 && kWgXSubRows >= kWgXPlaneRows + 18, "x planes: 18 rows each, 256-byte units apart");
+static_assert(3 * kWgLdsBytes <= 160 * 1024, "three blocks per CU");
 
 template <int O>
 __device__ __forceinline__ void wg_slot_e(f32x4& c, float a, float b, f32x2& e0, f32x2& e1, unsigned addr_b) {
@@ -29,8 +39,8 @@
       "ds_read2st64_b32 %8, %14 offset0:%21 offset1:%22\n\t"
       "v_mfma_f32_16x16x4_f32 %0, %9, %10, %0"
       : "+v"(c), "=&v"(e0), "=&v"(e1), "=&v"(d[0]), "=&v"(d[1]), "=&v"(d[2]), "=&v"(d[3]), "=&v"(d[4]), "=&v"(d[5])
-      : "v"(a), "v"(b), "v"(addr_b), "v"(addr_a[0]), "v"(addr_a[1]), "v"(addr_a[2]), "i"(O), "i"(O + 1), "i"(O + 4), "i"(O + 5), "i"(OA), "i"(OA + 1), "i"(OA + 5),
-        "i"(OA + 6)
+      : "v"(a), "v"(b), "v"(addr_b), "v"(addr_a[0]), "v"(addr_a[1]), "v"(addr_a[2]), "i"(O), "i"(O + 1), "i"(O + 4), "i"(O + 5), "i"(OA), "i"(OA + 1),
+        "i"(OA + kWgXPlaneRows / 4), "i"(OA + kWgXPlaneRows / 4 + 1)
       : "memory");
 }
 template <int O>
@@ -47,24 +57,24 @@
 
 template <int H, int ABL = 0>
 struct WgPair {
-  template <int NP0, int NP1, int I = 0, class DMA>
-  static __device__ __forceinline__ void run(f32x4 (&acc)[6][4], const f32x2 (&v)[6], f32x2 (&vn)[6], f32x2 (&d)[6], WinoT& t, f32x2 (&D)[2][6], unsigned addr_b,
-                                             unsigned addr_b_next, const unsigned (&addr_a)[3], const unsigned (&addr_a_next)[3], unsigned long long k15,
-                                             unsigned long long km15, DMA& dma) {
+  template <int ST, int NP0, int NP1, int I = 0, class DMA>
+  static __device__ __forceinline__ void run(f32x4 (&acc)[6][4], const f32x2 (&v)[6], f32x2 (&vn)[6], f32x2 (&d)[6], WinoT& t, f32x2 (&D)[2][6], unsigned base_b,
+                                             const unsigned (&base_a)[3], unsigned long long k15, unsigned long long km15, DMA& dma) {
     if constexpr (I < 48) {
       constexpr int CT = I / 12, G = I % 12, S = G / 6, P = G % 6;
+      constexpr int SU = ST * kWgStageUnits, SU1 = (ST == 2 ? 0 : ST + 1) * kWgStageUnits;
       f32x2(&dc)[6] = D[CT & 1];
       f32x2(&dn)[6] = D[(CT + 1) & 1];
       const float av = v[P][S], bv = dc[P][S];
       constexpr int OE = (CT < 3) ? (CT + 1) * 8 + 2 * H : (H == 0 ? 2 : 0);
       if constexpr ((ABL & 8) != 0) wino_slot(acc[P][CT], av, bv);
       else if constexpr (I == 0) {
-        if constexpr (H == 0) wg_slot_ea<OE, 2>(acc[P][CT], av, bv, dn[0], dn[5], addr_b, d, addr_a);
-        else wg_slot_ea<OE, 0>(acc[P][CT], av, bv, dn[0], dn[5], addr_b, d, addr_a_next);
-      } else if constexpr (I == 12) wg_slot_e_wd<OE>(acc[P][CT], av, bv, dn[0], dn[5], addr_b, d);
+        if constexpr (H == 0) wg_slot_ea<SU + OE, SU + 2>(acc[P][CT], av, bv, dn[0], dn[5], base_b, d, base_a);
+        else wg_slot_ea<SU + OE, SU1>(acc[P][CT], av, bv, dn[0], dn[5], base_b, d, base_a);
+      } else if constexpr (I == 12) wg_slot_e_wd<SU + OE>(acc[P][CT], av, bv, dn[0], dn[5], base_b, d);
       else if constexpr (G == 0) {
-        if constexpr (CT == 3 && H == 1) wg_slot_e<OE>(acc[P][CT], av, bv, dn[0], dn[5], addr_b_next);
-        else wg_slot_e<OE>(acc[P][CT], av, bv, dn[0], dn[5], addr_b);
+        if constexpr (CT == 3 && H == 1) wg_slot_e<SU1 + OE>(acc[P][CT], av, bv, dn[0], dn[5], base_b);
+        else wg_slot_e<SU + OE>(acc[P][CT], av, bv, dn[0], dn[5], base_b);
       } else if constexpr (G == 4) wino_slot_w<(I == 4 ? 6 : 0)>(acc[P][CT], av, bv, dn[0], dn[5]);
       else wino_slot(acc[P][CT], av, bv);
       if constexpr (G == 4) {
@@ -80,19 +90,17 @@
         if constexpr (CT == 2 && G == 9) wino_run<5, 10>(d, vn, t, k15, km15);
         if constexpr (CT == 3 && G == 9) wino_run<10, kWinoPieces>(d, vn, t, k15, km15);
       }
-      run<NP0, NP1, I + 1>(acc, v, vn, d, t, D, addr_b, addr_b_next, addr_a, addr_a_next, k15, km15, dma);
+      run<ST, NP0, NP1, I + 1>(acc, v, vn, d, t, D, base_b, base_a, k15, km15, dma);
     }
   }
 };
 
 template <int ABL = 0>
-__global__ __launch_bounds__(256, 2) void wgrad_wino_kernel(WgradArgs a, int off0, int cpb) {
+__global__ __launch_bounds__(256, 3) void wgrad_wino_kernel(WgradArgs a, int off0, int cpb) {
 #if defined(__HIP_DEVICE_COMPILE__)
   constexpr int NT = 256;
-  constexpr int XS = 4 * 2 * 20 * 16;
-  constexpr int YS = 4 * 2 * 16 * 16;
-  constexpr int BUF = XS + YS;
-  constexpr int STAGE_BYTES = BUF * 4;
+  constexpr int XS = kWgXS, BUF = kWgXS + kWgYS;
+  constexpr int SUBG = kWgXSubRows * 4, PLANEG = kWgXPlaneRows * 4;
   extern __shared__ __attribute__((aligned(16))) float smem[];
   typedef __attribute__((address_space(3))) void* lptr_t;
 
@@ -110,58 +118,59 @@
 #pragma unroll
       for (int r = 0; r < 4; ++r) acc[p][ct][r] = 0.f;
 
-  constexpr int X_ITEMS = 3, Y_ITEMS = 2;
-  int xoff[X_ITEMS], yoff[Y_ITEMS];
+  constexpr int X_ITEMS = 3;
+  int xoff[X_ITEMS], yoff;
 #pragma unroll
   for (int it = 0; it < X_ITEMS; ++it) {
-    const int g = tid + it * NT;
-    const int sub = g / 160, rem = g % 160, plane = rem / 80, prow = (rem % 80) >> 2, c4 = rem & 3;
+    const int g = it < 2 ? tid + it * NT : 2 * NT + (tid >> 6) * 32 + lane;
+    const int sub = g / SUBG, rem = g % SUBG, plane = rem / PLANEG, prow = (rem % PLANEG) >> 2, c4 = rem & 3;
     xoff[it] = ((2 * prow + plane + off0) * a.Cin + ci0 + sub * 16 + 4 * c4) * 4;
   }
-#pragma unroll
-  for (int it = 0; it < Y_ITEMS; ++it) {
-    const int g = tid + it * NT;
-    const int ct = g >> 7, rem = g & 127, plane = rem >> 6, tile = (rem & 63) >> 2, c4 = rem & 3;
-    yoff[it] = ((2 * tile + plane) * a.Cout + co0 + ct * 16 + 4 * c4) * 4;
+  {
+    const int ct = tid >> 7, rem = tid & 127, plane = rem >> 6, tile = (rem & 63) >> 2, c4 = rem & 3;
+    yoff = ((2 * tile + plane) * a.Cout + co0 + ct * 16 + 4 * c4) * 4;
   }
   const int xbytes = __builtin_amdgcn_readfirstlane(a.Lin * a.Cin * 4), ybytes = __builtin_amdgcn_readfirstlane(a.M * a.Cout * 4);
-  int q_next = 0, st_next = 0;
   bool in_loop = false;
   const int wv64 = __builtin_amdgcn_readfirstlane(tid & ~63);
-  auto dma_piece = [&](auto kc) {
-    constexpr int k = decltype(kc)::value;
+  auto dma_piece = [&](auto kc, auto stc, int q_next) __attribute__((always_inline)) {
+    constexpr int k = decltype(kc)::value, ST = decltype(stc)::value;
     if ((ABL & 1) && in_loop) return;
     const int b = __builtin_amdgcn_readfirstlane(q_next / cpb), cb = __builtin_amdgcn_readfirstlane(q_next % cpb);
-    float* stg = smem + st_next * BUF;
+    float* stg = smem + ST * BUF;
     if constexpr (k < X_ITEMS) {
       if (k < 2 || wv64 < 128) {
         const uintptr_t p = (uintptr_t)(a.x + (size_t)b * a.Lin * a.Cin);
         const __amdgpu_buffer_rsrc_t srd = __builtin_amdgcn_make_buffer_rsrc((void*)p, 0, xbytes, 0x00020000);
-        gn_buffer_load_lds(srd, (lptr_t)(stg + (k * NT + wv64) * 4), 16, xoff[k] + cb * 32 * a.Cin * 4, 0, 0, 0);
+        gn_buffer_load_lds(srd, (lptr_t)(stg + (k * NT + (k < 2 ? wv64 : wv64 >> 1)) * 4), 16, xoff[k] + cb * 32 * a.Cin * 4, 0, 0, 0);
       }
     } else {
       constexpr int it = k - X_ITEMS;
-      const int cbo = cb * 32 * a.Cout * 4;
+      const int cbo = cb * 32 * a.Cout * 4 + it * 128;
       const uintptr_t p = (uintptr_t)(a.dy + (size_t)b * a.M * a.Cout) + (uintptr_t)(unsigned)cbo;
       const __amdgpu_buffer_rsrc_t srd = __builtin_amdgcn_make_buffer_rsrc((void*)p, 0, ybytes - cbo, 0x00020000);
-      gn_buffer_load_lds(srd, (lptr_t)(stg + XS + (it * NT + wv64) * 4), 16, yoff[it], 0, 0, 0);
+      gn_buffer_load_lds(srd, (lptr_t)(stg + XS + (it * NT + wv64) * 4), 16, yoff, 0, 0, 0);
     }
   };
-  auto dma_all = [&]() {
-    dma_piece(std::integral_constant<int, 0>{}); dma_piece(std::integral_constant<int, 1>{}); dma_piece(std::integral_constant<int, 2>{});
-    dma_piece(std::integral_constant<int, 3>{}); dma_piece(std::integral_constant<int, 4>{});
+  auto dma_all = [&](auto stc, int q_next) __attribute__((always_inline)) {
+    dma_piece(std::integral_constant<int, 0>{}, stc, q_next); dma_piece(std::integral_constant<int, 1>{}, stc, q_next);
+    dma_piece(std::integral_constant<int, 2>{}, stc, q_next); dma_piece(std::integral_constant<int, 3>{}, stc, q_next);
+    dma_piece(std::integral_constant<int, 4>{}, stc, q_next);
   };
 
   const unsigned lds0 = (unsigned)(uintptr_t)smem;
   unsigned base_a[3];
 #pragma unroll
-  for (int j2 = 0; j2 < 3; ++j2) base_a[j2] = lds0 + wave * 2560 + ((kq + j2) * 16 + n16) * 4;
+  for (int j2 = 0; j2 < 3; ++j2) base_a[j2] = lds0 + wave * (kWgXSubRows * 64) + ((kq + j2) * 16 + n16) * 4;
   const unsigned base_b = lds0 + XS * 4 + (kq * 16 + n16) * 4;
   const unsigned long long k15 = 0x3fc000003fc00000ull, km15 = 0xbfc00000bfc00000ull;
 
   if (q_begin < q_end) {
-    q_next = q_begin; st_next = 0; dma_all();
-    q_next = min(q_begin + 1, q_end - 1); st_next = 1; dma_all();
+    constexpr std::integral_constant<int, 0> s0{};
+    constexpr std::integral_constant<int, 1> s1{};
+    constexpr std::integral_constant<int, 2> s2{};
+    dma_all(s0, q_begin);
+    dma_all(s1, min(q_begin + 1, q_end - 1));
     __syncthreads();
 
     f32x2 V0[6], V1[6], d[6], D[2][6];
@@ -170,7 +179,7 @@
       const char* sb = reinterpret_cast<const char*>(smem);
 #pragma unroll
       for (int j = 0; j < 6; ++j) {
-        const float* pp = reinterpret_cast<const float*>(sb + (base_a[j >> 1] - lds0) + (j & 1) * 1280);
+        const float* pp = reinterpret_cast<const float*>(sb + (base_a[j >> 1] - lds0) + (j & 1) * (kWgXPlaneRows * 64));
         d[j][0] = pp[0]; d[j][1] = pp[64];
       }
       wino_run<0, kWinoPieces>(d, V0, tt, k15, km15);
@@ -179,28 +188,41 @@
       wino_a_piece<0>(D[0][0], D[0][5], D[0][1], D[0][2], D[0][3], D[0][4]); wino_a_piece<1>(D[0][0], D[0][5], D[0][1], D[0][2], D[0][3], D[0][4]);
       wino_a_piece<2>(D[0][0], D[0][5], D[0][1], D[0][2], D[0][3], D[0][4]); wino_a_piece<3>(D[0][0], D[0][5], D[0][1], D[0][2], D[0][3], D[0][4]);
     }
-    int st = 0;
     in_loop = true;
-    for (int q = q_begin; q < q_end; ++q) {
-      const int st1 = st == 2 ? 0 : st + 1, st2 = st1 == 2 ? 0 : st1 + 1;
-      q_next = min(q + 2, q_end - 1);
-      st_next = st2;
-      unsigned addr_a[3], addr_a_next[3];
-#pragma unroll
-      for (int j2 = 0; j2 < 3; ++j2) { addr_a[j2] = base_a[j2] + st * STAGE_BYTES; addr_a_next[j2] = base_a[j2] + st1 * STAGE_BYTES; }
-      const unsigned addr_b = base_b + st * STAGE_BYTES, addr_b_next = base_b + st1 * STAGE_BYTES;
-      WgPair<0, ABL>::template run<3, 2>(acc, V0, V1, d, tt, D, addr_b, addr_b_next, addr_a, addr_a_next, k15, km15, dma_piece);
-      WgPair<1, ABL>::template run<3, 2>(acc, V1, V0, d, tt, D, addr_b, addr_b_next, addr_a, addr_a_next, k15, km15, dma_piece);
+    auto chunk = [&](auto stc, int q) __attribute__((always_inline)) {
+      constexpr int ST = decltype(stc)::value;
+      const int q_next = min(q + 2, q_end - 1);
+      auto dma = [&](auto kc) __attribute__((always_inline)) { dma_piece(kc, std::integral_constant<int, (ST + 2) % 3>{}, q_next); };
+      WgPair<0, ABL>::template run<ST, 3, 2>(acc, V0, V1, d, tt, D, base_b, base_a, k15, km15, dma);
+      WgPair<1, ABL>::template run<ST, 3, 2>(acc, V1, V0, d, tt, D, base_b, base_a, k15, km15, dma);
       if constexpr (!(ABL & 4)) __syncthreads();
-      st = st1;
+    };
+    int q = q_begin;
+    for (; q + 6 <= q_end; q += 6) {
+      chunk(s0, q); chunk(s1, q + 1); chunk(s2, q + 2); chunk(s0, q + 3); chunk(s1, q + 4); chunk(s2, q + 5);
+    }
+    if (q < q_end) {
+      chunk(s0, q);
+      if (q + 1 < q_end) {
+        chunk(s1, q + 1);
+        if (q + 2 < q_end) {
+          chunk(s2, q + 2);
+          if (q + 3 < q_end) {
+            chunk(s0, q + 3);
+            if (q + 4 < q_end) chunk(s1, q + 4);
+          }
+        }
+      }
     }
     asm volatile("s_nop 15\n\ts_nop 7" : "+v"(acc[5][0]), "+v"(acc[5][1]), "+v"(acc[5][2]), "+v"(acc[5][3]));
   }
 
   const size_t cc = (size_t)a.Cin * a.Cout;
+  const int lane_e = __builtin_amdgcn_mbcnt_hi(~0u, __builtin_amdgcn_mbcnt_lo(~0u, 0u));
+  const int row_e = ci0 + (wv64 >> 2) + 4 * (lane_e >> 4), col_e = co0 + (lane_e & 15);
 #pragma unroll
   for (int p = 0; p < 6; ++p) {
-    float* dst = a.part + ((size_t)split * 6 + p) * cc + (size_t)(ci0 + wave * 16 + 4 * kq) * a.Cout + co0 + n16;
+    float* dst = a.part + ((size_t)split * 6 + p) * cc + (size_t)row_e * a.Cout + col_e;
 #pragma unroll
     for (int ct = 0; ct < 4; ++ct)
 #pragma unroll
@@ -232,6 +254,12 @@
   return (size_t)a.Lin * a.Cin * 4 < 0x40000000ull && (size_t)a.M * a.Cout * 4 < 0x40000000ull;
 }
 
+int wgrad_wino_blocks_per_cu() {
+  int n = 0;
+  if (hipOccupancyMaxActiveBlocksPerMultiprocessor(&n, (const void*)wgrad_wino_kernel<0>, 256, kWgLdsBytes) != hipSuccess) return -1;
+  return n;
+}
+
 size_t wgrad_wino_workspace_bytes(int B, int M, int Cin, int Cout) {
   int s, cps;
   wgrad_split_plan(B, M, Cin, Cout, 64, 64, &s, &cps);
@@ -246,7 +274,7 @@
   int splits;
   wgrad_split_plan(a.B, a.M, a.Cin, a.Cout, 64, 64, &splits, &a.chunks_per_split);
   const int cpb = (a.M + 31) / 32;
-  constexpr size_t lds = 3 * sizeof(float) * (4 * 2 * 20 * 16 + 4 * 2 * 16 * 16);
+  constexpr size_t lds = kWgLdsBytes;
   dim3 grid(a.Cin / 64, a.Cout / 64, splits);
   prof_begin(s);
 #ifdef GN_ABLATION
diff --git a/gennet_amd/csrc/wgrad_wino_s2.hip b/gennet_amd/csrc/wgrad_wino_s2.hip
--- a/gennet_amd/csrc/wgrad_wino_s2.hip
+++ b/gennet_amd/csrc/wgrad_wino_s2.hip
@@ -5,6 +5,14 @@
 #include "wino_common.h"
 
 namespace gn {
+
+constexpr int kWg2XS = 4 * 4 * 12 * 16;
+constexpr int kWg2YS = 4 * 2 * 8 * 16;
+constexpr int kWg2StageBytes = (kWg2XS + kWg2YS) * 4;
+constexpr int kWg2StageUnits = kWg2StageBytes / 256;
+constexpr size_t kWg2LdsBytes = 3 * (size_t)kWg2StageBytes;
+static_assert(kWg2StageBytes % 256 == 0 && 2 * kWg2StageUnits + 15 <= 255, "stage offsets must fit the 8-bit read2st64 offsets");
+static_assert(3 * kWg2LdsBytes <= 160 * 1024, "three blocks per CU");
 
 template <int O>
 __device__ __forceinline__ void wg2_slot_e(f32x4& c, float a, float b, f32x2& e0, f32x2& e1, unsigned addr_b) {
@@ -16,25 +24,26 @@
       : "v"(a), "v"(b), "v"(addr_b), "i"(O), "i"(O + 1), "i"(O + 2), "i"(O + 3)
       : "memory");
 }
-template <int O>
-__device__ __forceinline__ void wg2_slot_ea(f32x4& c, float a, float b, f32x2& e0, f32x2& e1, unsigned addr_b, f32x2 (&d)[7], const unsigned (&addr_a)[2]) {
+template <int O, int OA>
+__device__ __forceinline__ void wg2_slot_ea(f32x4& c, float a, float b, f32x2& e0, f32x2& e1, unsigned addr_b, f32x2 (&d)[8], const unsigned (&addr_a)[2]) {
   asm volatile(
       "ds_read2st64_b32 %1, %12 offset0:%15 offset1:%16\n\t"
       "ds_read2st64_b32 %2, %12 offset0:%17 offset1:%18\n\t"
-      "ds_read2st64_b32 %3, %13 offset0:0 offset1:1\n\t"
-      "ds_read2st64_b32 %4, %13 offset0:3 offset1:4\n\t"
-      "ds_read2st64_b32 %5, %13 offset0:6 offset1:7\n\t"
-      "ds_read2st64_b32 %6, %13 offset0:9 offset1:10\n\t"
-      "ds_read2st64_b32 %7, %14 offset0:0 offset1:1\n\t"
-      "ds_read2st64_b32 %8, %14 offset0:3 offset1:4\n\t"
-      "ds_read2st64_b32 %9, %14 offset0:6 offset1:7\n\t"
+      "ds_read2st64_b32 %3, %13 offset0:%19 offset1:%20\n\t"
+      "ds_read2st64_b32 %4, %13 offset0:%21 offset1:%22\n\t"
+      "ds_read2st64_b32 %5, %13 offset0:%23 offset1:%24\n\t"
+      "ds_read2st64_b32 %6, %13 offset0:%25 offset1:%26\n\t"
+      "ds_read2st64_b32 %7, %14 offset0:%19 offset1:%20\n\t"
+      "ds_read2st64_b32 %8, %14 offset0:%21 offset1:%22\n\t"
+      "ds_read2st64_b32 %9, %14 offset0:%23 offset1:%24\n\t"
       "v_mfma_f32_16x16x4_f32 %0, %10, %11, %0"
       : "+v"(c), "=&v"(e0), "=&v"(e1), "=&v"(d[0]), "=&v"(d[1]), "=&v"(d[2]), "=&v"(d[3]), "=&v"(d[4]), "=&v"(d[5]), "=&v"(d[6])
-      : "v"(a), "v"(b), "v"(addr_b), "v"(addr_a[0]), "v"(addr_a[1]), "i"(O), "i"(O + 1), "i"(O + 2), "i"(O + 3)
+      : "v"(a), "v"(b), "v"(addr_b), "v"(addr_a[0]), "v"(addr_a[1]), "i"(O), "i"(O + 1), "i"(O + 2), "i"(O + 3), "i"(OA), "i"(OA + 4), "i"(OA + 1),
+        "i"(OA + 5), "i"(OA + 2), "i"(OA + 6), "i"(OA + 3), "i"(OA + 7)
       : "memory");
 }
 template <int O>
-__device__ __forceinline__ void wg2_slot_e_wd(f32x4& c, float a, float b, f32x2& e0, f32x2& e1, unsigned addr_b, f32x2 (&d)[7]) {
+__device__ __forceinline__ void wg2_slot_e_wd(f32x4& c, float a, float b, f32x2& e0, f32x2& e1, unsigned addr_b, f32x2 (&d)[8]) {
   asm volatile(
       "ds_read2st64_b32 %1, %12 offset0:%13 offset1:%14\n\t"
       "ds_read2st64_b32 %2, %12 offset0:%15 offset1:%16\n\t"
@@ -45,43 +54,61 @@
       : "memory");
 }
 
+__device__ constexpr int kWg2Pos[7] = {0, 7, 4, 6, 1, 3, 5};
+#define GN_PK_RSUB_SELF(o, x) asm volatile("v_pk_add_f32 %0, %1, %0 neg_lo:[0,1] neg_hi:[0,1]" : "+v"(o) : "v"(x))
+#define GN_PK_COPY_SELF(o) asm volatile("v_pk_mul_f32 %0, %0, 1.0 op_sel_hi:[1,0]" : "+v"(o))
+template <int K>
+__device__ __forceinline__ void wg2_x_piece(f32x2 (&w)[8]) {
+  if constexpr (K == 0) GN_PK_SUB_SELF(w[0], w[4]);
+  else if constexpr (K == 1) GN_PK_ADD(w[7], w[2], w[4]);
+  else if constexpr (K == 2) GN_PK_SUB_SELF(w[4], w[2]);
+  else if constexpr (K == 3) GN_PK_RSUB_SELF(w[6], w[2]);
+  else if constexpr (K == 4) GN_PK_SUB_SELF(w[1], w[3]);
+  else if constexpr (K == 5) GN_PK_SUB_SELF(w[5], w[3]);
+  else GN_PK_COPY_SELF(w[3]);
+}
+template <int K0, int K1>
+__device__ __forceinline__ void wg2_x_run(f32x2 (&w)[8]) {
+  if constexpr (K0 < K1) {
+    wg2_x_piece<K0>(w);
+    wg2_x_run<K0 + 1, K1>(w);
+  }
+}
+
 struct Wg2Chunk {
-  template <int NPIECES, int I = 0, class DMA>
-  static __device__ __forceinline__ void run(f32x4 (&acc)[7][4], const f32x2 (&v)[7], f32x2 (&vn)[7], f32x2 (&d)[7], f32x2 (&D)[2][4], unsigned addr_b,
-                                             unsigned addr_b_next, const unsigned (&addr_a_next)[2], DMA& dma) {
+  template <int ST, int NPIECES, int I = 0, class DMA>
+  static __device__ __forceinline__ void run(f32x4 (&acc)[7][4], const f32x2 (&v)[8], f32x2 (&vn)[8], f32x2 (&D)[2][4], unsigned base_b,
+                                             const unsigned (&base_a)[2], DMA& dma) {
     if constexpr (I < 56) {
       constexpr int CT = I / 14, G = I % 14, S = G / 7, P = G % 7;
+      constexpr int SU = ST * kWg2StageUnits, SU1 = (ST == 2 ? 0 : ST + 1) * kWg2StageUnits;
       constexpr int BI = (P == 0 || P == 4) ? 0 : ((P == 1 || P == 5) ? 2 : (P == 2 ? 3 : 1));
       f32x2(&dc)[4] = D[CT & 1];
       f32x2(&dn)[4] = D[(CT + 1) & 1];
-      const float av = v[P][S], bv = dc[BI][S];
+      const float av = v[kWg2Pos[P]][S], bv = dc[BI][S];
       constexpr int OE = (CT < 3) ? (CT + 1) * 4 : 0;
-      if constexpr (I == 0) wg2_slot_ea<OE>(acc[P][CT], av, bv, dn[0], dn[1], addr_b, d, addr_a_next);
-      else if constexpr (I == 14) wg2_slot_e_wd<OE>(acc[P][CT], av, bv, dn[0], dn[1], addr_b, d);
+      if constexpr (I == 0) wg2_slot_ea<SU + OE, SU1>(acc[P][CT], av, bv, dn[0], dn[1], base_b, vn, base_a);
+      else if constexpr (I == 14) wg2_slot_e_wd<SU + OE>(acc[P][CT], av, bv, dn[0], dn[1], base_b, vn);
       else if constexpr (G == 0) {
-        if constexpr (CT == 3) wg2_slot_e<OE>(acc[P][CT], av, bv, dn[0], dn[1], addr_b_next);
-        else wg2_slot_e<OE>(acc[P][CT], av, bv, dn[0], dn[1], addr_b);
+        if constexpr (CT == 3) wg2_slot_e<SU1 + OE>(acc[P][CT], av, bv, dn[0], dn[1], base_b);
+        else wg2_slot_e<SU + OE>(acc[P][CT], av, bv, dn[0], dn[1], base_b);
       } else if constexpr (G == 4) wino_slot_w<(I == 4 ? 7 : 0)>(acc[P][CT], av, bv, dn[0], dn[1]);
       else wino_slot(acc[P][CT], av, bv);
       if constexpr (G == 4 && CT < NPIECES) dma(std::integral_constant<int, CT>{});
-      if constexpr (G == 5) {
+      if constexpr (G == 12) {
         GN_PK_ADD(dn[2], dn[0], dn[1]);
         GN_PK_SUB(dn[3], dn[0], dn[1]);
       }
-      if constexpr (CT == 1 && G == 9) s2_run<1, 0, 7, 0, 4>(d, vn);
-      if constexpr (CT == 2 && G == 9) s2_run<1, 0, 7, 4, 7>(d, vn);
-      run<NPIECES, I + 1>(acc, v, vn, d, D, addr_b, addr_b_next, addr_a_next, dma);
+      if constexpr (CT == 1 && G == 9) wg2_x_run<0, 4>(vn);
+      if constexpr (CT == 2 && G == 9) wg2_x_run<4, 7>(vn);
+      run<ST, NPIECES, I + 1>(acc, v, vn, D, base_b, base_a, dma);
     }
   }
 };
 
-__global__ __launch_bounds__(256, 2) void wgrad_wino_s2_kernel(WgradArgs a, int off0, int cpb) {
+__global__ __launch_bounds__(256, 3) void wgrad_wino_s2_kernel(WgradArgs a, int off0, int cpb) {
 #if defined(__HIP_DEVICE_COMPILE__)
-  constexpr int NT = 256;
-  constexpr int XS = 4 * 4 * 12 * 16;
-  constexpr int YS = 4 * 2 * 8 * 16;
-  constexpr int BUF = XS + YS;
-  constexpr int STAGE_BYTES = BUF * 4;
+  constexpr int XS = kWg2XS, BUF = kWg2XS + kWg2YS;
   extern __shared__ __attribute__((aligned(16))) float smem[];
   typedef __attribute__((address_space(3))) void* lptr_t;
 
@@ -100,12 +127,10 @@
       for (int r = 0; r < 4; ++r) acc[p][ct][r] = 0.f;
 
   constexpr int X_ITEMS = 3;
-  int xoff[X_ITEMS], yoff;
-#pragma unroll
-  for (int it = 0; it < X_ITEMS; ++it) {
-    const int g = tid + it * NT;
-    const int sub = g / 192, rem = g % 192, plane = rem / 48, prow = (rem % 48) >> 2, c4 = rem & 3;
-    xoff[it] = ((4 * prow + plane + off0) * a.Cin + ci0 + sub * 16 + 4 * c4) * 4;
+  int xoff, yoff;
+  {
+    const int plane = lane >> 4, prow = (lane >> 2) & 3, c4 = lane & 3;
+    xoff = ((4 * prow + plane + off0) * a.Cin + ci0 + 4 * c4) * 4;
   }
   {
     const int g = tid;
@@ -113,16 +138,15 @@
     yoff = ((2 * tile + plane) * a.Cout + co0 + ct * 16 + 4 * c4) * 4;
   }
   const int xbytes = __builtin_amdgcn_readfirstlane(a.Lin * a.Cin * 4), ybytes = __builtin_amdgcn_readfirstlane(a.M * a.Cout * 4);
-  int q_next = 0, st_next = 0;
   const int wv64 = __builtin_amdgcn_readfirstlane(tid & ~63);
-  auto dma_piece = [&](auto kc) {
-    constexpr int k = decltype(kc)::value;
+  auto dma_piece = [&](auto kc, auto stc, int q_next) __attribute__((always_inline)) {
+    constexpr int k = decltype(kc)::value, ST = decltype(stc)::value;
     const int b = __builtin_amdgcn_readfirstlane(q_next / cpb), cb = __builtin_amdgcn_readfirstlane(q_next % cpb);
-    float* stg = smem + st_next * BUF;
+    float* stg = smem + ST * BUF;
     if constexpr (k < X_ITEMS) {
       const uintptr_t p = (uintptr_t)(a.x + (size_t)b * a.Lin * a.Cin);
       const __amdgpu_buffer_rsrc_t srd = __builtin_amdgcn_make_buffer_rsrc((void*)p, 0, xbytes, 0x00020000);
-      gn_buffer_load_lds(srd, (lptr_t)(stg + (k * NT + wv64) * 4), 16, xoff[k] + cb * 32 * a.Cin * 4, 0, 0, 0);
+      gn_buffer_load_lds(srd, (lptr_t)(stg + (3 * wv64 + k * 64) * 4), 16, xoff + ((cb * 32 + k * 16) * a.Cin * 4 + wv64), 0, 0, 0);
     } else {
       const int cbo = cb * 16 * a.Cout * 4;
       const uintptr_t p = (uintptr_t)(a.dy + (size_t)b * a.M * a.Cout) + (uintptr_t)(unsigned)cbo;
@@ -130,61 +154,73 @@
       gn_buffer_load_lds(srd, (lptr_t)(stg + XS + wv64 * 4), 16, yoff, 0, 0, 0);
     }
   };
-  auto dma_all = [&]() {
-    dma_piece(std::integral_constant<int, 0>{}); dma_piece(std::integral_constant<int, 1>{}); dma_piece(std::integral_constant<int, 2>{});
-    dma_piece(std::integral_constant<int, 3>{});
+  auto dma_all = [&](auto stc, int q_next) __attribute__((always_inline)) {
+    dma_piece(std::integral_constant<int, 0>{}, stc, q_next); dma_piece(std::integral_constant<int, 1>{}, stc, q_next);
+    dma_piece(std::integral_constant<int, 2>{}, stc, q_next); dma_piece(std::integral_constant<int, 3>{}, stc, q_next);
   };
 
   const unsigned lds0 = (unsigned)(uintptr_t)smem;
   unsigned base_a[2];
 #pragma unroll
-  for (int j4 = 0; j4 < 2; ++j4) base_a[j4] = lds0 + wave * 3072 + ((kq + j4) * 16 + n16) * 4;
+  for (int j4 = 0; j4 < 2; ++j4) base_a[j4] = lds0 + wave * 3072 + ((kq + j4) >> 2) * 1024 + (((kq + j4) & 3) * 16 + n16) * 4;
   const unsigned base_b = lds0 + XS * 4 + (kq * 16 + n16) * 4;
 
   if (q_begin < q_end) {
-    q_next = q_begin; st_next = 0; dma_all();
-    q_next = min(q_begin + 1, q_end - 1); st_next = 1; dma_all();
+    constexpr std::integral_constant<int, 0> s0{};
+    constexpr std::integral_constant<int, 1> s1{};
+    constexpr std::integral_constant<int, 2> s2{};
+    dma_all(s0, q_begin);
+    dma_all(s1, min(q_begin + 1, q_end - 1));
     __syncthreads();
 
-    f32x2 V0[7], V1[7], d[7], D[2][4];
+    f32x2 V0[8], V1[8], D[2][4];
     {
       const char* sb = reinterpret_cast<const char*>(smem);
 #pragma unroll
       for (int j = 0; j < 7; ++j) {
-        const float* pp = reinterpret_cast<const float*>(sb + (base_a[j >> 2] - lds0) + (j & 3) * 768);
-        d[j][0] = pp[0]; d[j][1] = pp[64];
+        const float* pp = reinterpret_cast<const float*>(sb + (base_a[j >> 2] - lds0) + (j & 3) * 256);
+        V0[j][0] = pp[0]; V0[j][1] = pp[256];
       }
-      s2_run<1, 0, 7, 0, 7>(d, V0);
+      wg2_x_run<0, 7>(V0);
       const float* pb = reinterpret_cast<const float*>(sb + (base_b - lds0));
       D[0][0][0] = pb[0]; D[0][0][1] = pb[64]; D[0][1][0] = pb[128]; D[0][1][1] = pb[192];
       GN_PK_ADD(D[0][2], D[0][0], D[0][1]);
       GN_PK_SUB(D[0][3], D[0][0], D[0][1]);
     }
-    int st = 0;
-    for (int q = q_begin; q < q_end; q += 2) {
-#pragma unroll
-      for (int half = 0; half < 2; ++half) {
-        if (half == 1 && q + 1 >= q_end) break;
-        const int st1 = st == 2 ? 0 : st + 1, st2 = st1 == 2 ? 0 : st1 + 1;
-        q_next = min(q + half + 2, q_end - 1);
-        st_next = st2;
-        unsigned addr_a_next[2];
-#pragma unroll
-        for (int j4 = 0; j4 < 2; ++j4) addr_a_next[j4] = base_a[j4] + st1 * STAGE_BYTES;
-        const unsigned addr_b = base_b + st * STAGE_BYTES, addr_b_next = base_b + st1 * STAGE_BYTES;
-        if (half == 0) Wg2Chunk::run<4>(acc, V0, V1, d, D, addr_b, addr_b_next, addr_a_next, dma_piece);
-        else Wg2Chunk::run<4>(acc, V1, V0, d, D, addr_b, addr_b_next, addr_a_next, dma_piece);
-        __syncthreads();
-        st = st1;
+    auto chunk = [&](auto stc, int q, const f32x2 (&v)[8], f32x2 (&vn)[8]) __attribute__((always_inline)) {
+      constexpr int ST = decltype(stc)::value;
+      const int q_next = min(q + 2, q_end - 1);
+      auto dma = [&](auto kc) __attribute__((always_inline)) { dma_piece(kc, std::integral_constant<int, (ST + 2) % 3>{}, q_next); };
+      Wg2Chunk::run<ST, 4>(acc, v, vn, D, base_b, base_a, dma);
+      __syncthreads();
+    };
+    int q = q_begin;
+    for (; q + 6 <= q_end; q += 6) {
+      chunk(s0, q, V0, V1); chunk(s1, q + 1, V1, V0); chunk(s2, q + 2, V0, V1);
+      chunk(s0, q + 3, V1, V0); chunk(s1, q + 4, V0, V1); chunk(s2, q + 5, V1, V0);
+    }
+    if (q < q_end) {
+      chunk(s0, q, V0, V1);
+      if (q + 1 < q_end) {
+        chunk(s1, q + 1, V1, V0);
+        if (q + 2 < q_end) {
+          chunk(s2, q + 2, V0, V1);
+          if (q + 3 < q_end) {
+            chunk(s0, q + 3, V1, V0);
+            if (q + 4 < q_end) chunk(s1, q + 4, V0, V1);
+          }
+        }
       }
     }
     asm volatile("s_nop 15\n\ts_nop 7" : "+v"(acc[6][0]), "+v"(acc[6][1]), "+v"(acc[6][2]), "+v"(acc[6][3]));
   }
 
   const size_t cc = (size_t)a.Cin * a.Cout;
+  const int lane_e = __builtin_amdgcn_mbcnt_hi(~0u, __builtin_amdgcn_mbcnt_lo(~0u, 0u));
+  const int row_e = ci0 + (wv64 >> 2) + 4 * (lane_e >> 4), col_e = co0 + (lane_e & 15);
 #pragma unroll
   for (int p = 0; p < 7; ++p) {
-    float* dst = a.part + ((size_t)split * 7 + p) * cc + (size_t)(ci0 + wave * 16 + 4 * kq) * a.Cout + co0 + n16;
+    float* dst = a.part + ((size_t)split * 7 + p) * cc + (size_t)row_e * a.Cout + col_e;
 #pragma unroll
     for (int ct = 0; ct < 4; ++ct)
 #pragma unroll
@@ -226,6 +262,12 @@
   return (size_t)a.Lin * a.Cin * 4 < 0x40000000ull && (size_t)a.M * a.Cout * 4 < 0x40000000ull;
 }
 
+int wgrad_wino_s2_blocks_per_cu() {
+  int n = 0;
+  if (hipOccupancyMaxActiveBlocksPerMultiprocessor(&n, (const void*)wgrad_wino_s2_kernel, 256, kWg2LdsBytes) != hipSuccess) return -1;
+  return n;
+}
+
 size_t wgrad_wino_s2_workspace_bytes(int B, int M, int Cin, int Cout) {
   int s, cps, cpb;
   s2_plan(B, M, Cin, Cout, &s, &cps, &cpb);
@@ -239,7 +281,7 @@
   }
   int splits, cpb;
   s2_plan(a.B, a.M, a.Cin, a.Cout, &splits, &a.chunks_per_split, &cpb);
-  constexpr size_t lds = 3 * sizeof(float) * (4 * 4 * 12 * 16 + 4 * 2 * 8 * 16);
+  constexpr size_t lds = kWg2LdsBytes;
   dim3 grid(a.Cin / 64, a.Cout / 64, splits);
   prof_begin(s);
   hipLaunchKernelGGL(wgrad_wino_s2_kernel, grid, dim3(256), lds, s, a, a.off[0], cpb);
diff --git a/gennet_amd/ops.py b/gennet_amd/ops.py
--- a/gennet_amd/ops.py
+++ b/gennet_amd/ops.py
@@ -771,6 +771,10 @@
     _lib.call('gn_prof_reset')
 
 
+def kernel_blocks_per_cu(kind):
+    return _lib.count('gn_kernel_blocks_per_cu', int(kind))
+
+
 def prof_collect(kind=-1):
     import ctypes
     out = (ctypes.c_double * 4)()
diff --git a/include/gennet_hip.h b/include/gennet_hip.h
--- a/include/gennet_hip.h
+++ b/include/gennet_hip.h
@@ -180,6 +180,7 @@
 int gn_prof_enable(int on);
 int gn_prof_reset(void);
 int gn_prof_collect(int kind, double* out4_host);
+int gn_kernel_blocks_per_cu(int kind);
 
 int gn_chirp_fd_whitened(const double* m1, const double* m2, const double* scale, double* out_hp, double* out_hc,
                          int nb, int Nf, double df, double f_low, double dist_mpc, double iota, double phi0, void* stream);
```
